# fabioiuri/DRecPy

Hardware: AMD Instinct MI355X
Metric: training samples/sec (user-item pairs) (higher is better)
Workload: dtype f32; 1 GPU; CDAE hidden_factors=128 sampled-output sparse-Adagrad on synth-10m-shaped synthetic (10000000 users x 1000000 items, 199573906 positives), corruption 0.2, neg_ratio 5; batch_per_gpu=65536, global_batch=65536, touch_list=prepared ahead on a side stream, batches=fresh device-sampled batch every step (sampler running ahead on the side stream)

## Files before the change

drecpy_amd/_lib.py:

```python
import ctypes as C
import os

_HERE = os.path.dirname(os.path.abspath(__file__))
LIB_PATH = os.path.join(_HERE, 'libdrx.so')

LOSS_BCE, LOSS_MSE = 0, 1
TARGETS_REFERENCE, TARGETS_PER_ROW = 0, 1
OPT_ADAM, OPT_ADAGRAD, OPT_ROWWISE_ADAGRAD = 0, 1, 2
DENSE_AUX_CLEAN = 0x100
KEY_NONE = 0xFFFFFFFF
SHARD_SELF_BYPASS = 1
BATCH_SHARE_USERS = 1


class DrxError(RuntimeError):
    pass


DRX_REC_SIGMOID_BIAS, DRX_REC_BIAS, DRX_REC_CLIP = 0, 1, 2

KNN_METRICS = {'cosine': 0, 'adjusted_cosine': 1, 'cosine_cf': 2, 'jaccard': 3, 'msd': 4, 'pearson': 5}
KNN_USER, KNN_ITEM = 0, 1
KNN_AGGREGATIONS = {'mean': 0, 'weighted_mean': 1}

# ... 116 lines not shown
    _fields_ = [(n, C.c_void_p) for n in ('K0u', 'm_u', 'v_u', 'K0i', 'm_i', 'v_i')] + [('n_items', C.c_int32), ('n_users', C.c_int32)] + \
               [(n, C.c_float) for n in ('alpha_u', 'alpha_i', 'l2_coef', 'beta1', 'beta2', 'eps')] + [('row_order', C.c_void_p), ('n_long', C.c_int32), ('opt_kind', C.c_int32)]


class Optim(C.Structure):
    _fields_ = [('kind', C.c_int32), ('lr', C.c_float), ('reg_rate', C.c_float), ('beta1', C.c_float),
                ('beta2', C.c_float), ('eps', C.c_float), ('alpha', C.c_float * 5),
                ('s1', C.c_void_p * 5), ('s2', C.c_void_p * 5)]


_lib = None

SIGNATURES = {
    'drx_version': (C.c_int, []),
    'drx_strerror': (C.c_char_p, [C.c_int]),
    'drx_hash_u32': (C.c_uint32, [C.c_uint64, C.c_uint32, C.c_uint32]),
    'drx_event_create': (C.c_void_p, []),
    'drx_event_destroy': (None, [C.c_void_p]),
    'drx_event_record': (C.c_int, [C.c_void_p, C.c_void_p]),
    'drx_stream_wait_event': (C.c_int, [C.c_void_p, C.c_void_p]),
    'drx_event_synchronize': (C.c_int, [C.c_void_p]),
    'drx_stream_create_cu_slice': (C.c_void_p, [C.c_int32]),
    'drx_stream_destroy': (None, [C.c_void_p]),
    'drx_cdae_forward': (C.c_int, [C.POINTER(CdaeParams), C.POINTER(History), C.POINTER(Batch), C.c_void_p,
                                   C.c_void_p, C.c_void_p]),
    'drx_cdae_scratch_bytes': (C.c_size_t, [C.POINTER(CdaeParams), C.c_int32, C.c_int32, C.c_int32]),
    'drx_cdae_step_dense': (C.c_int, [C.POINTER(CdaeParams), C.POINTER(Optim), C.POINTER(History), C.POINTER(Batch),
                                      C.c_int32, C.c_int32, C.c_void_p, C.c_size_t, C.c_void_p, C.c_void_p]),
    'drx_cdae_step_sparse': (C.c_int, [C.POINTER(CdaeParams), C.POINTER(Optim), C.POINTER(History), C.POINTER(Batch),
                                       C.c_int32, C.c_void_p, C.c_size_t, C.c_void_p, C.c_void_p]),
    'drx_cdae_step_sparse_timed': (C.c_int, [C.POINTER(CdaeParams), C.POINTER(Optim), C.POINTER(History),
                                             C.POINTER(Batch), C.c_int32, C.c_void_p, C.c_size_t, C.c_void_p,
                                             C.POINTER(C.c_void_p), C.c_void_p]),
    'drx_cdae_prep_bytes': (C.c_size_t, [C.POINTER(CdaeParams), C.c_int32, C.c_int32]),
    'drx_cdae_sparse_prepare': (C.c_int, [C.POINTER(CdaeParams), C.POINTER(History), C.POINTER(Batch), C.c_void_p,
                                          C.c_size_t, C.c_void_p]),
    'drx_cdae_step_sparse_prepared': (C.c_int, [C.POINTER(CdaeParams), C.POINTER(Optim), C.POINTER(History),
                                                C.POINTER(Batch), C.c_int32, C.c_void_p, C.c_size_t, C.c_void_p,
                                                C.c_size_t, C.c_void_p, C.POINTER(C.c_void_p), C.c_void_p]),
    'drx_cdae_prep_bytes_hot': (C.c_size_t, [C.POINTER(CdaeParams), C.c_int32, C.c_int32, C.c_int32]),
    'drx_cdae_scratch_bytes_hot': (C.c_size_t, [C.POINTER(CdaeParams), C.c_int32, C.c_int32, C.c_int32]),
    'drx_cdae_sparse_prepare_hot': (C.c_int, [C.POINTER(CdaeParams), C.POINTER(History), C.POINTER(Batch), C.POINTER(HotHead),
                                              C.c_void_p, C.c_size_t, C.c_void_p]),
    'drx_debug_prep_counts': (C.c_int, [C.POINTER(CdaeParams), C.POINTER(History), C.POINTER(Batch), C.POINTER(HotHead), C.c_void_p,
                                        C.c_int32, C.c_int32, C.c_int32, C.c_void_p, C.c_size_t, C.c_void_p, C.c_void_p, C.c_void_p,
                                        C.c_void_p, C.c_void_p, C.POINTER(C.c_int32), C.c_void_p]),
    'drx_debug_prep_result': (C.c_int, [C.POINTER(CdaeParams), C.c_int32, C.c_int32, C.c_int32, C.c_void_p, C.c_size_t, C.c_void_p,
                                        C.c_void_p, C.c_void_p, C.c_void_p, C.c_void_p, C.c_void_p]),
    'drx_debug_cdae_reduce': (C.c_int, [C.POINTER(CdaeParams), C.POINTER(Optim), C.POINTER(History), C.POINTER(Batch), C.POINTER(HotHead),
                                        C.c_void_p, C.c_size_t, C.c_void_p, C.c_void_p, C.c_void_p, C.c_int32, C.c_void_p, C.c_size_t,
                                        C.c_void_p]),
    'drx_debug_span_plan': (C.c_int, [C.POINTER(CdaeParams), C.c_int32, C.c_int32, C.c_int32, C.c_void_p, C.c_size_t, C.c_void_p,
                                      C.c_void_p, C.c_void_p, C.c_void_p]),
    'drx_cdae_step_sparse_hot': (C.c_int, [C.POINTER(CdaeParams), C.POINTER(Optim), C.POINTER(History), C.POINTER(Batch),
                                           C.POINTER(HotHead), C.c_int32, C.c_void_p, C.c_size_t, C.c_void_p, C.c_size_t,
                                           C.c_void_p, C.POINTER(C.c_void_p), C.c_void_p]),
    'drx_cdae_hot_rows_for': (C.c_int32, [C.POINTER(CdaeParams), C.c_int32, C.c_int32, C.c_int32, C.c_int32]),
    'drx_cdae_prep_forget': (None, [C.c_void_p]),
    'drx_point_sample_scratch_bytes': (C.c_size_t, [C.c_int32]),
    'drx_list_sample_device': (C.c_int, [C.POINTER(ListGroups), C.c_int32, C.c_int32, C.c_int32, C.c_int32, C.c_uint64, C.c_void_p, C.c_void_p,
                                         C.c_void_p, C.c_void_p]),
    'drx_point_sample': (C.c_int, [C.POINTER(History), C.c_int32, C.c_int32, C.c_int32, C.c_int32, C.c_uint64,
                                   C.c_void_p, C.c_void_p, C.c_void_p, C.c_void_p, C.c_void_p, C.c_size_t, C.c_void_p, C.c_uint32,
                                   C.c_void_p]),
    'drx_point_sample_recorded': (C.c_int, [C.POINTER(History), C.POINTER(History), C.c_int32, C.c_int32, C.c_int32, C.c_int32, C.c_uint64,
                                   C.c_void_p, C.c_void_p, C.c_void_p, C.c_void_p, C.c_void_p, C.c_size_t, C.c_void_p, C.c_uint32,
                                   C.c_void_p]),
    'drx_point_sample_by_user_scratch_bytes': (C.c_size_t, [C.c_int32, C.c_int32]),
    'drx_point_sample_by_user': (C.c_int, [C.POINTER(History), C.POINTER(History), C.c_int32, C.c_int32, C.c_int32, C.c_int32, C.c_uint64,
                                           C.c_void_p, C.c_void_p, C.c_void_p, C.c_void_p, C.c_void_p, C.c_size_t, C.c_void_p, C.c_uint32,
                                           C.c_void_p]),
    'drx_point_sample_valued': (C.c_int, [C.POINTER(History), C.POINTER(History), C.c_void_p, C.c_float, C.c_float, C.c_int32, C.c_int32,
                                          C.c_int32, C.c_int32, C.c_uint64, C.c_void_p, C.c_void_p, C.c_void_p, C.c_void_p]),
    'drx_dmf_distinct_scratch_bytes': (C.c_size_t, [C.c_int32, C.c_int32, C.c_int32]),
    'drx_dmf_batch_distinct_device': (C.c_int, [C.c_void_p, C.c_void_p, C.c_void_p, C.c_int32, C.c_int32, C.c_int32] + [C.c_void_p] * 10 +
                                      [C.c_void_p, C.c_size_t, C.c_void_p]),
    'drx_shard_prep_bytes': (C.c_size_t, [C.POINTER(CdaeParams), C.POINTER(Shard), C.c_int32, C.c_int32]),
    'drx_shard_work_bytes': (C.c_size_t, [C.POINTER(Shard)]),
    'drx_shard_prep_layout': (C.c_int, [C.POINTER(CdaeParams), C.POINTER(Shard), C.c_int32, C.c_int32, C.POINTER(C.c_size_t)]),
    'drx_shard_prepare': (C.c_int, [C.POINTER(CdaeParams), C.POINTER(Shard), C.POINTER(History), C.POINTER(Batch), C.c_void_p,
                                    C.c_size_t, C.c_void_p, C.c_size_t, C.c_void_p]),
    'drx_shard_owner_table_bytes': (C.c_size_t, [C.POINTER(Shard), C.c_int32]),
    'drx_shard_chunks': (C.c_int32, [C.POINTER(Shard)]),
    'drx_shard_unit_shift': (C.c_int32, [C.POINTER(Shard)]),
    'drx_shard_owner_index': (C.c_int, [C.POINTER(Shard), C.c_void_p, C.c_int32, C.POINTER(C.c_int32), C.c_int32, C.c_int32, C.c_void_p,
                                        C.c_size_t, C.c_void_p]),
    'drx_shard_gather_rows': (C.c_int, [C.POINTER(CdaeParams), C.POINTER(Shard), C.c_void_p, C.c_int32, C.POINTER(C.c_int32),
                                        C.c_int32, C.c_void_p, C.c_void_p]),
    'drx_shard_step_scratch_bytes': (C.c_size_t, [C.POINTER(CdaeParams), C.c_int32, C.c_int32]),
    'drx_shard_step_local': (C.c_int, [C.POINTER(CdaeParams), C.POINTER(Optim), C.POINTER(Shard), C.POINTER(History), C.POINTER(Batch),
                                       C.c_void_p, C.c_size_t, C.c_void_p, C.c_void_p, C.c_int32, C.c_int32, C.c_void_p, C.c_size_t,
                                       C.POINTER(C.c_void_p), C.c_void_p]),
    'drx_shard_apply': (C.c_int, [C.POINTER(CdaeParams), C.POINTER(Optim), C.POINTER(Shard), C.c_int32, C.c_void_p, C.c_void_p,
                                  C.c_int32, C.POINTER(C.c_int32), C.c_int32, C.c_int32, C.c_void_p, C.POINTER(C.c_void_p), C.POINTER(C.c_int64),
                                  C.c_void_p, C.c_void_p]),
    'drx_shard_exchange_sizes': (C.c_int, [C.POINTER(CdaeParams), C.POINTER(Shard), C.c_void_p, C.c_void_p, C.POINTER(C.c_int64)]),
    'drx_shard_phase_layout': (C.c_int, [C.POINTER(CdaeParams), C.POINTER(Shard), C.c_void_p, C.c_void_p, C.c_int32, C.POINTER(C.c_int64)]),
    'drx_shard_phase_keys': (C.c_int, [C.POINTER(Shard), C.c_void_p, C.POINTER(ShardExchange), C.c_void_p]),
    'drx_shard_phase_rows': (C.c_int, [C.POINTER(CdaeParams), C.POINTER(Shard), C.c_void_p, C.POINTER(ShardExchange), C.c_int32, C.c_void_p]),
    'drx_shard_phase_local': (C.c_int, [C.POINTER(CdaeParams), C.POINTER(Optim), C.POINTER(Shard), C.POINTER(History), C.POINTER(Batch),
                                        C.c_void_p, C.POINTER(ShardExchange), C.c_void_p, C.c_size_t, C.c_int32, C.c_int32, C.c_void_p,
                                        C.c_size_t, C.POINTER(C.c_void_p), C.c_void_p]),
    'drx_shard_phase_tail': (C.c_int, [C.POINTER(CdaeParams), C.POINTER(Optim), C.POINTER(Shard), C.c_void_p, C.POINTER(ShardExchange),
                                       C.POINTER(ShardExchange), C.c_int32, C.c_void_p, C.c_void_p]),
    'drx_copy_f4': (C.c_int, [C.c_void_p, C.c_void_p, C.c_size_t, C.c_void_p]),
    'drx_copy_f4_variant': (C.c_int, [C.c_void_p, C.c_void_p, C.c_size_t, C.c_int32, C.c_void_p]),
# ... 277 lines not shown
```

drecpy_amd/csrc/drx_cdae.hip:

```cpp
#include "drx_common.hpp"
#include "drx_rows.hpp"
#include "drx_segreduce.hpp"
#include <cstring>
#include "drx_scan.hpp"
#include "drx_prep.hpp"
#include "drx_segstream.hpp"
#include "drx_cdae_host.hpp"
#include <type_traits>
#include <mutex>
#include <unordered_map>

#ifdef DRX_STAMPS
static unsigned long long *h_stamps = nullptr;
extern "C" int drx_debug_set_stamps(unsigned long long *buf, unsigned int) { h_stamps = buf; return 0; }
#endif

namespace drx {

struct SparseBufs {
  float *dz1;
  float *g2;
  float *dz2;
  float *lossb;
  float *phead, *ptail;
  float *phs, *pts;
  float *pblock, *pbs;
  float *bpart;
  const uint8_t *solo_v, *solo_o;
  unsigned long long *stamps;
  const int32_t *order;
  const int32_t *usamp, *worder, *n_items;
  const WorkItem *witem;
  int T, n_chunks, n_bpart;
};

template <int G, int J, int KIND = -1>
__device__ __forceinline__ void sparse_apply(const DrxCdaeParams &P, const DrxOptim &opt, int B, uint32_t key, int lane,
                                             const float4 (&g)[J], float gs) {
  const uint32_t N = (uint32_t)P.n_items;
  float *const tW = P.W, *const tO = P.W2T, *const tV = P.V;
  float *const a0 = opt.s1[0], *const a1 = opt.s1[1], *const a2 = opt.s1[2];
  float *const c0 = opt.s2[0], *const c1 = opt.s2[1], *const c2 = opt.s2[2];
  const int var = key < N ? 0 : (key < 2 * N ? 1 : 2);
  const size_t row = key - (uint32_t)var * N;
  float *const tab = var == 0 ? tW : (var == 1 ? tO : tV);
  float *const s1 = var == 0 ? a0 : (var == 1 ? a1 : a2);
  float *const s2 = var == 0 ? c0 : (var == 1 ? c1 : c2);
  OptScalars o = opt_for(opt, 0, B);
  o.inv_k = 1.0f / (float)P.k;
  float4 w[J];
  load_row<G, J>(tab, row, P.ld, lane, w);
  row_update<G, J, KIND>(o, tab, s1, s2, row, P.ld, lane, w, g);
  if (var == 1 && lane == 0) {
    const int kind = KIND >= 0 ? KIND : o.kind;
    float pb = P.b2[row], m = opt.s1[4][row], v = kind == DRX_OPT_ADAM ? opt.s2[4][row] : 0.f;
    o.rb = 0.f;
    opt_update1<KIND>(o, gs, pb, m, v);
    P.b2[row] = pb; opt.s1[4][row] = m;
    if (kind == DRX_OPT_ADAM) opt.s2[4][row] = v;
  }
}

template <int G, int J>
// ... 283 lines not shown
  if (r != 0) return;
#pragma unroll
  for (int j = 0; j < J; ++j) acc[j] = f4_zero();
#pragma unroll 8
  for (int rr = 0; rr < R; ++rr) {
    float4 v[J];
    load_row<G, J>(lds, (size_t)rr, P.ld, lane, v);
#pragma unroll
    for (int j = 0; j < J; ++j) f4_add(acc[j], v[j]);
  }
  sampled_finish<G, J>(P, opt, H, bt, scale, qthr, loss_kind, S, b, lane, acc);
}

template <int KIND>
struct DirectPolicyT {
  DrxCdaeParams P;
  DrxOptim opt;
  int B;
  float scale;
  const float *dz1;
  long long g2_off;
  const float *dz2;
  template <int G, int J>
  __device__ __forceinline__ void load(uint32_t key, uint32_t bv, int lane, float4 (&row)[J], float &sc, float &coef) const {
    const uint32_t N = (uint32_t)P.n_items;
    const bool is_out = key >= N && key < 2 * N;
    const uint32_t b = bv & 0x7FFFFFFFu;
    load_row<G, J>(dz1 + (is_out ? g2_off : 0ll), (size_t)b, P.ld, lane, row);
    if (is_out) sc = dz2[b];
    coef = key < N ? ((bv >> 31) ? -scale : scale) : 1.0f;
  }
  template <int G, int J>
  __device__ __forceinline__ void finish(uint32_t key, int, int lane, const float4 (&g)[J], float gs) const {
    sparse_apply<G, J, KIND>(P, opt, B, key, lane, g, gs);
  }
  static constexpr bool kStreamParks = false;
  __device__ __forceinline__ StreamArrays stream_arrays() const {
    const uint32_t N = (uint32_t)P.n_items;
    return StreamArrays{{0u, N, 2u * N}, {dz1, dz1 + g2_off, dz1}, {P.W, P.W2T, P.V}, {opt.s1[0], opt.s1[1], opt.s1[2]},
                        {scale, 1.0f, 1.0f}, {nullptr, dz2, nullptr}, {nullptr, P.b2, nullptr}, {nullptr, opt.s1[4], nullptr}};
  }
  __device__ __forceinline__ float stream_decay() const { return opt.reg_rate / (float)B; }
  __device__ __forceinline__ void stream_update(float g, float &p, float &a) const {
    static_assert(KIND == DRX_OPT_ADAGRAD || KIND < 0, "one slot per element");
    OptScalars o = opt_for(opt, 0, B);
    float unused = 0.f;
    opt_update1<DRX_OPT_ADAGRAD>(o, g, p, a, unused);
  }
  __device__ __forceinline__ void stream_update_scalar(float g, float &p, float &a) const { stream_update(g, p, a); }
};
using DirectPolicy = DirectPolicyT<-1>;
using DirectPolicyAdagrad = DirectPolicyT<DRX_OPT_ADAGRAD>;

template <int G, int J, int NT>
__device__ __forceinline__ void bias_final_body(const DrxCdaeParams &P, const DrxOptim &opt, const BiasArgs &A,
                                                float *lds , float *red) {
  constexpr int R = NT / G;
  const int lane = threadIdx.x % G, r = threadIdx.x / G;
  float4 acc[J];
#pragma unroll
  for (int j = 0; j < J; ++j) acc[j] = f4_zero();
  constexpr int NB = J == 1 ? 8 : 2;
  for (int i = r; i < A.n_part; i += NB * R) {
    float4 v[NB][J];
#pragma unroll
    for (int q = 0; q < NB; ++q) {
#pragma unroll
      for (int j = 0; j < J; ++j) v[q][j] = f4_zero();
      if (i + q * R < A.n_part) load_row<G, J>(A.part, (size_t)(i + q * R), P.ld, lane, v[q]);
    }
#pragma unroll
    for (int q = 0; q < NB; ++q)
#pragma unroll
      for (int j = 0; j < J; ++j) f4_add(acc[j], v[q][j]);
  }
  store_row<G, J>(lds, (size_t)r, P.ld, lane, acc);
  __syncthreads();
  if (r == 0) {
    float4 g[J], w[J];
#pragma unroll
    for (int j = 0; j < J; ++j) g[j] = f4_zero();
#pragma unroll 8
    for (int rr = 0; rr < R; ++rr) {
      float4 v[J];
      load_row<G, J>(lds, (size_t)rr, P.ld, lane, v);
#pragma unroll
      for (int j = 0; j < J; ++j) f4_add(g[j], v[j]);
    }
    load_row<G, J>(P.b, 0, P.ld, lane, w);
    OptScalars o = opt_for(opt, 0, A.B);
    if (o.kind == DRX_OPT_ROWWISE_ADAGRAD) o.kind = DRX_OPT_ADAGRAD;
    o.rb = 0.f;
    row_update<G, J>(o, P.b, opt.s1[3], opt.s2[3], 0, P.ld, lane, w, g);
  }
  if (A.loss_out) {
    const float *lp = A.part + (size_t)A.n_part * P.ld;
    float a = 0.f;
    for (int b = threadIdx.x; b < A.n_part; b += NT) a += lp[b];
    float t = block_sum(a, red);
    if (threadIdx.x == 0) { A.loss_out[0] = t / (float)A.B; A.loss_out[1] = 0.f; }
  }
}

template <int G, int J>
struct BiasFinalExtra {
  DrxCdaeParams P;
  DrxOptim opt;
  BiasArgs A;
  __device__ __forceinline__ void operator()(float *lds) const {
    __shared__ float red[kFixBlock / 64];
    bias_final_body<G, J, kFixBlock>(P, opt, A, lds, red);
  }
};

constexpr int kHotSlice = 512;
constexpr int kHotGroup = 64;

struct HotArgs {
  const float *dz1;
  const uint32_t *mask;
  float *part;
  uint32_t *any;
  const int32_t *item;
  float scale;
  int B, H, Bw, S, first;
  float *bpart;
  const float *lossb;
};

static inline int hot_slices(int B) { return (B + kHotSlice - 1) / kHotSlice; }
static inline int hot_groups(int H) { return (H + kHotGroup - 1) / kHotGroup; }

typedef __bf16 hot_bf16x8 __attribute__((ext_vector_type(8)));
typedef float hot_f32x4 __attribute__((ext_vector_type(4)));
typedef uint32_t hot_u32x4 __attribute__((ext_vector_type(4)));

template <int LD, int NT>
struct HotPartialExtra {
  HotArgs A;
  __device__ __forceinline__ void operator()(float *) const {
    constexpr int CS = LD / 16, NW = NT / 64;
    const int lane = threadIdx.x & 63, wv = __builtin_amdgcn_readfirstlane((int)(threadIdx.x >> 6));
    const int ngr = (A.H + kHotGroup - 1) / kHotGroup;
    const int task = ((int)blockIdx.x - A.first) * NW + wv;
    if (task >= A.S * ngr * CS) return;
    const int cs = task % CS, rg = (task / CS) % ngr, s = task / (CS * ngr);
    const int c = lane & 15, kq = lane >> 4;
    const int nt = min(kHotGroup, A.H - rg * kHotGroup) / 16;
    const int b_begin = s * kHotSlice, b_end = min(A.B, b_begin + kHotSlice);
    const uint32_t *const mgrp = A.mask + (size_t)rg * kHotGroup * A.Bw;
    const float *const slice = A.dz1 + (size_t)b_begin * LD + cs * 16;
    const uint32_t mlane = (uint32_t)c * (uint32_t)A.Bw, xlane = (uint32_t)(8 * kq * LD + c);
    hot_f32x4 acc[4];
#pragma unroll
    for (int t = 0; t < 4; ++t) acc[t] = hot_f32x4{0.f, 0.f, 0.f, 0.f};
    uint32_t seen = 0u;
    float bsum = 0.f;
    for (int b0 = b_begin; b0 < b_end; b0 += 32) {
      float x[8];
      uint32_t w[4];
      {
        const float *const rows = slice + (size_t)(b0 - b_begin) * LD;
        const uint32_t *const words = mgrp + (b0 >> 5);
        const int left = A.B - b0 - 8 * kq;
// ... 18 lines not shown
          hv[e] = __float_as_uint(v) & 0xFFFF0000u;
          const float r1 = v - __uint_as_float(hv[e]);
          mv[e] = __float_as_uint(r1) & 0xFFFF0000u;
          lv[e] = __float_as_uint(r1 - __uint_as_float(mv[e])) & 0xFFFF0000u;
        }
        bh[i] = (hv[0] >> 16) | hv[1];
        bm[i] = (mv[0] >> 16) | mv[1];
        bl[i] = (lv[0] >> 16) | lv[1];
      }
#pragma unroll
      for (int t = 0; t < 4; ++t) {
        seen |= (w[t] != 0u ? 1u : 0u) << t;
        const uint32_t bits = (w[t] >> (8 * kq)) & 0xFFu;
        hot_u32x4 a;
#pragma unroll
        for (int i = 0; i < 4; ++i) a[i] = ((bits >> (2 * i)) & 1u) * 0x3F80u | ((bits >> (2 * i + 1)) & 1u) * 0x3F800000u;
        const hot_bf16x8 av = __builtin_bit_cast(hot_bf16x8, a);
        acc[t] = __builtin_amdgcn_mfma_f32_16x16x32_bf16(av, __builtin_bit_cast(hot_bf16x8, bh), acc[t], 0, 0, 0);
        acc[t] = __builtin_amdgcn_mfma_f32_16x16x32_bf16(av, __builtin_bit_cast(hot_bf16x8, bm), acc[t], 0, 0, 0);
        acc[t] = __builtin_amdgcn_mfma_f32_16x16x32_bf16(av, __builtin_bit_cast(hot_bf16x8, bl), acc[t], 0, 0, 0);
      }
    }
    float *const out = A.part + ((size_t)s * A.H + rg * kHotGroup) * LD + cs * 16 + c;
#pragma unroll
    for (int t = 0; t < 4; ++t)
      if (t < nt) {
#pragma unroll
        for (int i = 0; i < 4; ++i) out[(size_t)(16 * t + 4 * kq + i) * LD] = acc[t][i];
      }
    if (cs == 0) {
      uint32_t rows[4];
#pragma unroll
      for (int t = 0; t < 4; ++t) rows[t] = (uint32_t)__ballot((seen >> t) & 1u) & 0xFFFFu;
      if (lane == 0) {
        uint32_t *const any = A.any + (size_t)s * (A.H / 32) + rg * (kHotGroup / 32);
        any[0] = rows[0] | (rows[1] << 16);
        if (nt > 2) any[1] = rows[2] | (rows[3] << 16);
      }
    }
    if (rg == 0) {
      const float g1 = __shfl(bsum, c + 16, 64), g2 = __shfl(bsum, c + 32, 64), g3 = __shfl(bsum, c + 48, 64);
      if (kq == 0) A.bpart[(size_t)s * LD + cs * 16 + c] = ((bsum + g1) + g2) + g3;
      if (cs == 0 && A.lossb) {
        float l = 0.f;
        for (int b = b_begin + lane; b < b_end; b += 64) l += A.lossb[b];
#pragma unroll
        for (int o = 32; o > 0; o >>= 1) l += __shfl_xor(l, o, 64);
        if (lane == 0) A.bpart[(size_t)A.S * LD + s] = l;
      }
    }
  }
};

template <int LD, class Policy>
struct HotFinishExtra {
  HotArgs A;
  Policy pol;
  __device__ __forceinline__ void operator()(float *lds) const {
    constexpr int NT = kFixBlock, NQ = NT / LD;
    static_assert(NQ >= 1 && NT % LD == 0, "a row per workgroup");
    const int h = (int)blockIdx.x - A.first;
    if (h >= A.H) return;
    const uint32_t bit = 1u << (h & 31);
    bool touched = false;
    for (int s = (int)threadIdx.x; s < A.S; s += NT) touched |= (A.any[(size_t)s * (A.H / 32) + (h >> 5)] & bit) != 0u;
    if (!__syncthreads_or(touched)) return;
    const int c = (int)threadIdx.x % LD, q = (int)threadIdx.x / LD;
    const int per = (A.S + NQ - 1) / NQ, s0 = q * per, s1 = min(A.S, s0 + per);
    float sum = 0.f;
#pragma unroll 8
    for (int s = s0; s < s1; ++s) sum += A.part[((size_t)s * A.H + h) * LD + c];
    lds[q * LD + c] = sum;
    __syncthreads();
    if (q == 0) {
      float t = lds[c];
#pragma unroll
      for (int k = 1; k < NQ; ++k) t += lds[k * LD + c];
      const StreamArrays SA = pol.stream_arrays();
      const size_t off = (size_t)A.item[h] * LD + c;
      float pv = SA.table[0][off], av = SA.slot[0][off];
      pol.stream_update(fmaf(pol.stream_decay(), pv, A.scale * t), pv, av);
      SA.table[0][off] = pv;
      SA.slot[0][off] = av;
    }
  }
};

template <class E1, class E2>
struct ExtraPair {
  E1 e1;
  int n1;
  E2 e2;
  __device__ __forceinline__ void operator()(float *lds) const {
    if ((int)blockIdx.x < n1) e1(lds);
    else e2(lds);
  }
};

static SparseBufs sparse_layout(Carver &cv, const DrxCdaeParams &P, int B, int n_touch_slots) {
  SparseBufs S{};
  S.T = n_touch_slots + 2 * B;
  const int chunk = seg_chunk(long_segments(S.T, P));
  S.n_chunks = (S.T + chunk - 1) / chunk;
  S.n_bpart = 1024;
  S.dz1 = cv.take<float>((size_t)2 * B * P.ld);
  S.g2 = cv.take<float>((size_t)B * P.ld);
  S.dz2 = cv.take<float>(B);
  S.lossb = cv.take<float>(B);
  S.phead = cv.take<float>((size_t)S.n_chunks * P.ld);
  S.ptail = cv.take<float>((size_t)S.n_chunks * P.ld);
  S.phs = cv.take<float>(S.n_chunks);
  S.pts = cv.take<float>(S.n_chunks);
  {
    const int cpb = kSegBlock / pick_geom(P.ld).G;
    const int n_blocks = (S.n_chunks + cpb - 1) / cpb;
    S.pblock = cv.take<float>((size_t)n_blocks * P.ld);
    S.pbs = cv.take<float>(n_blocks);
  }
  S.bpart = cv.take<float>((size_t)S.n_bpart * (P.ld + 1));
  return S;
}

static std::mutex g_hot_mu;
static std::unordered_map<const void *, int> g_hot_of;
static void hot_record(const void *prepared, int H) {
  std::lock_guard<std::mutex> lk(g_hot_mu);
  if (H > 0) g_hot_of[prepared] = H;
  else g_hot_of.erase(prepared);
}
static int hot_recorded(const void *prepared) {
  std::lock_guard<std::mutex> lk(g_hot_mu);
  const auto it = g_hot_of.find(prepared);
  return it == g_hot_of.end() ? 0 : it->second;
}

struct HotBufs { float *part; uint32_t *any; float *bpart; };
static HotBufs hot_layout(Carver &cv, const DrxCdaeParams &P, int B, int H) {
  HotBufs HB{nullptr, nullptr, nullptr};
  if (H <= 0) return HB;
  HB.part = cv.take<float>((size_t)hot_slices(B) * H * P.ld);
  HB.any = cv.take<uint32_t>((size_t)hot_slices(B) * (H / 32));
  HB.bpart = cv.take<float>((size_t)hot_slices(B) * (P.ld + 1));
  return HB;
}

template <int G, int J>
static void launch_forward(ForwardForm form, const DrxCdaeParams &P, const DrxOptim &opt, const DrxHistory &hist, const DrxBatch &bt,
                           float scale, uint32_t qthr, int32_t loss_kind, const SparseBufs &S, const float *ks_h, const float *ks_dot,
                           hipStream_t st) {
  constexpr int gpb = kBlock / G;
  const dim3 groups((bt.B + gpb - 1) / gpb);
  const bool adagrad = opt.kind == DRX_OPT_ADAGRAD;
  switch (form) {
  case ForwardForm::ColumnShard:
    hipLaunchKernelGGL((k_kshard_rest<G, J>), groups, dim3(kBlock), 0, st, P, opt, hist, bt, scale, qthr, loss_kind, S, ks_h, ks_dot);
    break;
  case ForwardForm::SharedUsers:
    if constexpr (G >= 16 && J <= 2) {
      const long long wmax = (long long)(P.n_users < bt.B ? P.n_users : bt.B) + bt.B / share_item_triples(P.ld) + 1;
      hipLaunchKernelGGL((adagrad ? k_items_fwd_bwd<G, J, DRX_OPT_ADAGRAD> : k_items_fwd_bwd<G, J>), dim3((unsigned)(wmax < bt.B ? wmax : bt.B)),
                         dim3(kItemThreads), share_item_lds_bytes(P.ld), st, P, opt, hist, bt, scale, qthr, loss_kind, S);
    }
    break;
  case ForwardForm::PerWorkgroup:
    hipLaunchKernelGGL((k_sampled_fwd_bwd_wg<G, J>), dim3(bt.B), dim3(kBlock), (size_t)gpb * P.ld * 4, st, P, opt, hist, bt, scale, qthr,
                       loss_kind, S);
    break;
  case ForwardForm::PerGroup:
    hipLaunchKernelGGL((adagrad ? k_sampled_fwd_bwd<G, J, DRX_OPT_ADAGRAD> : k_sampled_fwd_bwd<G, J>), groups, dim3(kBlock), 0, st, P, opt, hist,
                       bt, scale, qthr, loss_kind, S);
    break;
  }
}

template <int G, int J, class Policy>
static int reduce_and_finish(ReduceForm form, const DrxCdaeParams &P, const DrxOptim &opt, const SparseBufs &S, const SegBufs &SB,
                             const PlanBufs &PB, const SpanPlan &plan, const BiasArgs &BA, const HotArgs &HA, void *const *events,
                             hipStream_t st) {
  const Policy pol{P, opt, BA.B, HA.scale, S.dz1, (long long)(S.g2 - S.dz1), S.dz2};
  const BiasFinalExtra<G, J> bias{P, opt, BA};
  int rc = DRX_EINVAL;
  if (HA.H == 0) rc = launch_reduce<G, J>(form, SB, PB, plan, pol, BA, st);
  else if constexpr (kHotBuilt<G, J, Policy>) {
    constexpr int NT = kStreamThreads<G>;
    HotArgs part = HA;
    part.first = 0;
    const int n_hot = (HA.S * hot_groups(HA.H) * (G / 4) + NT / 64 - 1) / (NT / 64);
    rc = launch_reduce_streamed<G, J>(SB, PB, plan, pol, n_hot, HotPartialExtra<4 * G, NT>{part}, st);
  }
  if (rc) return rc;
  DRX_HIP(phase_event(events, 3, st));
  rc = DRX_EINVAL;
  if (HA.H == 0) rc = launch_spans<G, J>(SB, PB, plan, pol, 1, bias, st);
  else if constexpr (kHotBuilt<G, J, Policy>) {
    HotArgs fin = HA;
    fin.first = kSpanBlocks + 1;
    using Finish = ExtraPair<BiasFinalExtra<G, J>, HotFinishExtra<4 * G, Policy>>;
    rc = launch_spans<G, J>(SB, PB, plan, pol, 1 + HA.H, Finish{bias, fin.first, {fin, pol}}, st);
  }
  if (rc) return rc;
  DRX_HIP(phase_event(events, 4, st));
  DRX_HIP(phase_event(events, 5, st));
  return DRX_OK;
}

}

using namespace drx;

extern "C" {

size_t drx_cdae_scratch_bytes(const DrxCdaeParams *p, int32_t B, int32_t n_touch_slots, int32_t dense_mode) {
  if (!p || B < 1 || n_touch_slots < 0) return 0;
  Carver c(nullptr, 0);
  if (dense_mode) {
    c.off = dense_layout_bytes(*p, B);
  } else {
    (void)sparse_layout(c, *p, B, n_touch_slots);
    (void)prep_layout(c, *p, B, n_touch_slots);
  }
  return align_up(c.off, 256) + 256;
}

struct GivenGradients { const float *dz1, *g2, *dz2; int32_t form; };

static int step_sparse_impl(const DrxCdaeParams *p, const DrxOptim *opt, const DrxHistory *hist, const DrxBatch *bt,
                            int32_t loss_kind, const void *prepared, size_t prepared_bytes, void *scratch, size_t scratch_bytes,
                            float *loss_out, void *const *events, void *stream, const float *ks_h = nullptr,
                            const float *ks_dot = nullptr, const DrxHotHead *hot = nullptr, const GivenGradients *given = nullptr) {
  int rc = check_params(p);
  if (rc) return rc;
  rc = check_batch(hist, bt);
  if (rc || !opt || !scratch || !bt->iid || (!bt->y && !given) || !bt->keep_off) return DRX_EINVAL;
  if (opt->kind != DRX_OPT_ADAM && opt->kind != DRX_OPT_ADAGRAD && opt->kind != DRX_OPT_ROWWISE_ADAGRAD) return DRX_EINVAL;
  for (int i = 0; i < 5; ++i)
    if (!opt->s1[i] || (opt->kind == DRX_OPT_ADAM && !opt->s2[i])) return DRX_EINVAL;
  if ((uint64_t)2 * p->n_items + p->n_users + 1 >= 0xFFFFFFFFull) return DRX_EINVAL;
  hipStream_t st = (hipStream_t)stream;
  const int H = hot ? hot->H : 0;
  if (prepared && hot_recorded(prepared) != H) return DRX_EINVAL;
  Carver cv(scratch, scratch_bytes);
  SparseBufs S = sparse_layout(cv, *p, bt->B, bt->n_touch_slots);
  const HotBufs HB = hot_layout(cv, *p, bt->B, H);
  PrepBufs R{};
  if (prepared) {
    Carver cp(const_cast<void *>(prepared), prepared_bytes);
    R = prep_layout(cp, *p, bt->B, bt->n_touch_slots, H);
    if (!cp.ok()) return DRX_ESCRATCH;
  } else {
    R = prep_layout(cv, *p, bt->B, bt->n_touch_slots, H);
  }
  if (!cv.ok()) return DRX_ESCRATCH;
  const float scale = 1.0f / (1.0f - bt->q);
  const uint32_t qthr = q_threshold(bt->q);
  const int rows_per_block = (bt->B + S.n_bpart - 1) / S.n_bpart;
  const int n_bpart = (bt->B + rows_per_block - 1) / rows_per_block;
  S.solo_v = prepared ? R.solo_v : nullptr;
  S.solo_o = prepared ? R.solo_o : nullptr;
  S.order = prepared ? R.order : nullptr;
  SegBufs SB{R.keys_s, R.vals_s, S.phead, S.ptail, S.phs, S.pts, nullptr, nullptr, nullptr, nullptr, S.T, S.n_chunks, p->ld, nullptr};
#ifdef DRX_STAMPS
  S.stamps = SB.stamps = h_stamps;
#endif
  PlanBufs PB{S.pblock, S.pbs};
  if (prepared && ks_h && share_users(p, hist, bt, R)) return DRX_EINVAL;
  const bool share = prepared && !ks_h && share_users(p, hist, bt, R);
  S.usamp = share ? R.usamp : nullptr;
  S.witem = share ? R.witem : nullptr;
  S.worder = share ? R.worder : nullptr;
  S.n_items = share ? R.n_du : nullptr;
  ReduceForm form = reduce_form(opt->kind, bt->B, S.T, *p);
  const ForwardForm fwd = forward_form(ks_h != nullptr, share, bt->B, bt->n_touch_slots);
  if (H > 0 && !hot_head_fits(form, p->ld, share, ks_h != nullptr)) return DRX_EINVAL;
  if (given) {
    if (share || (given->form == 1 && (H > 0 || form == ReduceForm::PlannedLong))) return DRX_EINVAL;
    if (given->form == 1) form = ReduceForm::PlannedShort;
  }
  const HotArgs HA{S.dz1, R.hmask, HB.part, HB.any, hot ? hot->item : nullptr, scale, bt->B, H, R.Bw, hot_slices(bt->B), 0, HB.bpart,
                   loss_out ? S.lossb : nullptr};
  const BiasArgs BA = H > 0 ? BiasArgs{S.dz1, HB.bpart, S.lossb, loss_out, bt->B, hot_slices(bt->B), kHotSlice}
                            : BiasArgs{S.dz1, S.bpart, S.lossb, loss_out, bt->B, n_bpart, rows_per_block};
  DRX_HIP(phase_event(events, 0, st));
  if (given) {
    const size_t row_bytes = (size_t)bt->B * p->ld * sizeof(float);
    DRX_HIP(hipMemcpyAsync(S.dz1, given->dz1, row_bytes, hipMemcpyDeviceToDevice, st));
    DRX_HIP(hipMemcpyAsync(S.g2, given->g2, row_bytes, hipMemcpyDeviceToDevice, st));
    DRX_HIP(hipMemcpyAsync(S.dz2, given->dz2, (size_t)bt->B * sizeof(float), hipMemcpyDeviceToDevice, st));
    DRX_HIP(hipMemsetAsync(S.lossb, 0, (size_t)bt->B * sizeof(float), st));
  } else {
    (void)dispatch_geom(p->ld, [&](auto g) -> int {
      launch_forward<decltype(g)::G, decltype(g)::J>(fwd, *p, *opt, *hist, *bt, scale, qthr, loss_kind, S, ks_h, ks_dot, st);
      return DRX_OK;
    });
  }
  DRX_HIP(phase_event(events, 1, st));
  if (!prepared) {
    rc = prepare_impl(p, hist, bt, R, st, false, TouchPresence{nullptr, WireGeo{1, 0, 1}}, hot ? hot->slot : nullptr,
                      hot ? hot->item : nullptr);
    if (rc) return rc;
  }
  DRX_HIP(phase_event(events, 2, st));
  rc = dispatch_geom(p->ld, [&](auto g) -> int {
    constexpr int G = decltype(g)::G, J = decltype(g)::J;
    return opt->kind == DRX_OPT_ADAGRAD
        ? reduce_and_finish<G, J, DirectPolicyAdagrad>(form, *p, *opt, S, SB, PB, R.plan, BA, HA, events, st)
        : reduce_and_finish<G, J, DirectPolicy>(form, *p, *opt, S, SB, PB, R.plan, BA, HA, events, st);
  });
  if (rc) return rc;
  DRX_LAUNCH_CHECK();
  return DRX_OK;
}

size_t drx_cdae_prep_bytes(const DrxCdaeParams *p, int32_t B, int32_t n_touch_slots) {
  if (!p || B < 1 || n_touch_slots < 0) return 0;
  Carver c(nullptr, 0);
  (void)prep_layout(c, *p, B, n_touch_slots);
  return align_up(c.off, 256) + 256;
}

int drx_cdae_sparse_prepare(const DrxCdaeParams *p, const DrxHistory *hist, const DrxBatch *bt, void *prepared,
                            size_t prepared_bytes, void *stream) {
  int rc = check_params(p);
  if (rc) return rc;
  rc = check_batch(hist, bt);
  if (rc || !prepared || !bt->iid || !bt->keep_off) return DRX_EINVAL;
  Carver cp(prepared, prepared_bytes);
  PrepBufs R = prep_layout(cp, *p, bt->B, bt->n_touch_slots);
  if (!cp.ok()) return DRX_ESCRATCH;
  hot_record(prepared, 0);
  rc = prepare_impl(p, hist, bt, R, (hipStream_t)stream, true);
  if (rc) return rc;
  if (p->ld <= 16) order_by_degree(bt, R, (hipStream_t)stream, true);
  DRX_LAUNCH_CHECK();
  return DRX_OK;
}

size_t drx_cdae_prep_result_bytes(const DrxCdaeParams *p, int32_t B, int32_t n_touch_slots) {
  if (!p || B < 1 || n_touch_slots < 0) return 0;
  Carver c(nullptr, 0);
  return prep_layout(c, *p, B, n_touch_slots).result_bytes;
}

int drx_cdae_step_sparse_prepared(const DrxCdaeParams *p, const DrxOptim *opt, const DrxHistory *hist, const DrxBatch *bt,
                                  int32_t loss_kind, const void *prepared, size_t prepared_bytes, void *scratch,
                                  size_t scratch_bytes, float *loss_out, void *const *events, void *stream) {
  if (!prepared) return DRX_EINVAL;
  return step_sparse_impl(p, opt, hist, bt, loss_kind, prepared, prepared_bytes, scratch, scratch_bytes, loss_out, events, stream);
}

int drx_cdae_kshard_forward(const DrxCdaeParams *p, const DrxHistory *hist, const DrxBatch *bt, float *h_out, float *dot_partial,
                            void *stream) {
  return drx_cdae_kshard_forward_prepared(p, hist, bt, nullptr, 0, h_out, dot_partial, stream);
}

int drx_cdae_kshard_forward_prepared(const DrxCdaeParams *p, const DrxHistory *hist, const DrxBatch *bt, const void *prepared,
                                     size_t prepared_bytes, float *h_out, float *dot_partial, void *stream) {
  int rc = check_params(p);
  if (rc) return rc;
  rc = check_batch(hist, bt);
  if (rc || !bt->iid || !bt->keep_off || !h_out || !dot_partial) return DRX_EINVAL;
  const int32_t *order = nullptr;
  if (prepared) {
    Carver cp(const_cast<void *>(prepared), prepared_bytes);
    const PrepBufs R = prep_layout(cp, *p, bt->B, bt->n_touch_slots);
    if (!cp.ok()) return DRX_ESCRATCH;
    order = R.order;
  }
  hipStream_t st = (hipStream_t)stream;
  const float scale = 1.0f / (1.0f - bt->q);
  const uint32_t qthr = q_threshold(bt->q);
  const bool per_wg = forward_per_workgroup(bt->B, bt->n_touch_slots);
  return dispatch_geom(p->ld, [&](auto g) -> int {
    constexpr int G = decltype(g)::G, J = decltype(g)::J;
    constexpr int gpb = kBlock / G;
    if (per_wg)
      hipLaunchKernelGGL((k_kshard_fwd_wg<G, J>), dim3(bt->B), dim3(kBlock), (size_t)gpb * p->ld * 4, st, *p, *hist, *bt, scale, qthr,
                         h_out, dot_partial);
    else
      hipLaunchKernelGGL((k_kshard_fwd<G, J>), dim3((bt->B + gpb - 1) / gpb), dim3(kBlock), 0, st, *p, *hist, *bt, scale, qthr, h_out,
                         dot_partial, order);
    DRX_LAUNCH_CHECK();
    return DRX_OK;
  });
// ... 5 lines not shown
  if (!h || !dot_total) return DRX_EINVAL;
  if (opt && opt->kind == DRX_OPT_ROWWISE_ADAGRAD) return DRX_EINVAL;
  return step_sparse_impl(p, opt, hist, bt, loss_kind, prepared, prepared_bytes, scratch, scratch_bytes, loss_out, events, stream,
                          h, dot_total);
}

int drx_cdae_step_sparse(const DrxCdaeParams *p, const DrxOptim *opt, const DrxHistory *hist, const DrxBatch *bt,
                         int32_t loss_kind, void *scratch, size_t scratch_bytes, float *loss_out, void *stream) {
  return step_sparse_impl(p, opt, hist, bt, loss_kind, nullptr, 0, scratch, scratch_bytes, loss_out, nullptr, stream);
}

int drx_cdae_step_sparse_timed(const DrxCdaeParams *p, const DrxOptim *opt, const DrxHistory *hist, const DrxBatch *bt,
                               int32_t loss_kind, void *scratch, size_t scratch_bytes, float *loss_out, void *const *events,
                               void *stream) {
  if (!events) return DRX_EINVAL;
  return step_sparse_impl(p, opt, hist, bt, loss_kind, nullptr, 0, scratch, scratch_bytes, loss_out, events, stream);
}

static int hot_rows(const DrxCdaeParams *p, int32_t H) {
  if (!p || H < 0 || H > DRX_MAX_HOT || H % 32 || H > p->n_items) return -1;
  return H;
}

static bool hot_ok(const DrxCdaeParams *p, const DrxHotHead *hot) {
  return hot && hot_rows(p, hot->H) >= 0 && (hot->H == 0 || (hot->slot && hot->item && p->ld <= 4 * kHotMaxG));
}

size_t drx_cdae_prep_bytes_hot(const DrxCdaeParams *p, int32_t B, int32_t n_touch_slots, int32_t H) {
  if (!p || B < 1 || n_touch_slots < 0 || hot_rows(p, H) < 0) return 0;
  Carver c(nullptr, 0);
  (void)prep_layout(c, *p, B, n_touch_slots, H);
  return align_up(c.off, 256) + 256;
}

size_t drx_cdae_scratch_bytes_hot(const DrxCdaeParams *p, int32_t B, int32_t n_touch_slots, int32_t H) {
  if (!p || B < 1 || n_touch_slots < 0 || hot_rows(p, H) < 0) return 0;
  Carver c(nullptr, 0);
  (void)sparse_layout(c, *p, B, n_touch_slots);
  (void)hot_layout(c, *p, B, H);
  (void)prep_layout(c, *p, B, n_touch_slots, H);
  return align_up(c.off, 256) + 256;
}

int drx_cdae_sparse_prepare_hot(const DrxCdaeParams *p, const DrxHistory *hist, const DrxBatch *bt, const DrxHotHead *hot,
                                void *prepared, size_t prepared_bytes, void *stream) {
  int rc = check_params(p);
  if (rc) return rc;
  rc = check_batch(hist, bt);
  if (rc || !prepared || !bt->iid || !bt->keep_off || !hot_ok(p, hot)) return DRX_EINVAL;
  Carver cp(prepared, prepared_bytes);
  PrepBufs R = prep_layout(cp, *p, bt->B, bt->n_touch_slots, hot->H);
  if (!cp.ok()) return DRX_ESCRATCH;
  hot_record(prepared, 0);
  rc = prepare_impl(p, hist, bt, R, (hipStream_t)stream, true, TouchPresence{nullptr, WireGeo{1, 0, 1}}, hot->slot, hot->item);
  if (rc) return rc;
  hot_record(prepared, hot->H);
  if (p->ld <= 16) order_by_degree(bt, R, (hipStream_t)stream, true);
  DRX_LAUNCH_CHECK();
  return DRX_OK;
}

int drx_debug_prep_counts(const DrxCdaeParams *p, const DrxHistory *hist, const DrxBatch *bt, const DrxHotHead *hot, uint8_t *present,
                          int32_t ipr, int32_t cshift, int32_t world, void *prepared, size_t prepared_bytes, uint32_t *hist_out,
                          uint32_t *buckets_out, uint32_t *keys_out, uint32_t *vals_out, uint32_t *mask_out, int32_t *info_out,
                          void *stream) {
  int rc = check_params(p);
  if (rc) return rc;
  rc = check_batch(hist, bt);
  if (rc || !prepared || !bt->iid || !bt->keep_off || !hist_out || !buckets_out || !keys_out || !vals_out || !info_out) return DRX_EINVAL;
  if ((uint64_t)2 * p->n_items + p->n_users + 1 >= 0xFFFFFFFFull) return DRX_EINVAL;
  if (hot && !hot_ok(p, hot)) return DRX_EINVAL;
  if (present && (ipr < 1 || cshift < 0 || cshift > 30 || world < 1)) return DRX_EINVAL;
  const int H = hot ? hot->H : 0;
  if (H > 0 && !mask_out) return DRX_EINVAL;
  Carver cp(prepared, prepared_bytes);
  const PrepBufs R = prep_layout(cp, *p, bt->B, bt->n_touch_slots, H);
  if (!cp.ok()) return DRX_ESCRATCH;
  if (H > 0 && !hot_list_fits(R.T, *p, present != nullptr)) return DRX_EINVAL;
  hipStream_t st = (hipStream_t)stream;
  hot_record(prepared, 0);
  launch_touches(p, hist, bt, R, st, TouchPresence{present, WireGeo{present ? ipr : 1, present ? cshift : 0, present ? world : 1}},
                 H > 0 ? hot->slot : nullptr, H > 0 ? hot->item : nullptr);
  const SortRider rider{bt->keep_off, bt->B, R.order_work, R.partials, R.partial_rows};
  const uint32_t *h = nullptr;
  rc = sort_first_counts(R.sort_temp, R.sort_bytes, R.keys, (size_t)R.T, R.bits, true, st, rider, &h);
  if (rc) return rc;
  const int dbits = sort_first_digit_bits(R.bits);
  DRX_HIP(hipMemcpyAsync(hist_out, h, sizeof(uint32_t) << dbits, hipMemcpyDeviceToDevice, st));
  DRX_HIP(hipMemcpyAsync(buckets_out, R.order_work, 256 * sizeof(uint32_t), hipMemcpyDeviceToDevice, st));
  DRX_HIP(hipMemcpyAsync(keys_out, R.keys, (size_t)R.T * sizeof(uint32_t), hipMemcpyDeviceToDevice, st));
  DRX_HIP(hipMemcpyAsync(vals_out, R.vals, (size_t)R.T * sizeof(uint32_t), hipMemcpyDeviceToDevice, st));
  if (H > 0) DRX_HIP(hipMemcpyAsync(mask_out, R.hmask, (size_t)H * R.Bw * sizeof(uint32_t), hipMemcpyDeviceToDevice, st));
  info_out[0] = dbits;
  info_out[1] = R.partials ? R.partial_rows : 0;
  info_out[2] = R.T;
  info_out[3] = DRX_PREP_ROUNDS ? touch_grid(bt->B) : (bt->B + 15) / 16;
  DRX_LAUNCH_CHECK();
  return DRX_OK;
}

int drx_debug_prep_result(const DrxCdaeParams *p, int32_t B, int32_t n_touch_slots, int32_t H, const void *prepared, size_t prepared_bytes,
                          uint32_t *keys_s_out, uint32_t *vals_s_out, uint8_t *solo_v_out, uint8_t *solo_o_out, int32_t *order_out,
                          void *stream) {
  int rc = check_params(p);
  if (rc) return rc;
  if (B < 1 || n_touch_slots < 0 || hot_rows(p, H) < 0 || !prepared || !keys_s_out || !vals_s_out || !solo_v_out || !solo_o_out || !order_out)
    return DRX_EINVAL;
  Carver cp(const_cast<void *>(prepared), prepared_bytes);
  const PrepBufs R = prep_layout(cp, *p, B, n_touch_slots, H);
  if (!cp.ok()) return DRX_ESCRATCH;
  hipStream_t st = (hipStream_t)stream;
  DRX_HIP(hipMemcpyAsync(keys_s_out, R.keys_s, (size_t)R.T * sizeof(uint32_t), hipMemcpyDeviceToDevice, st));
  DRX_HIP(hipMemcpyAsync(vals_s_out, R.vals_s, (size_t)R.T * sizeof(uint32_t), hipMemcpyDeviceToDevice, st));
  DRX_HIP(hipMemcpyAsync(solo_v_out, R.solo_v, (size_t)B, hipMemcpyDeviceToDevice, st));
  DRX_HIP(hipMemcpyAsync(solo_o_out, R.solo_o, (size_t)B, hipMemcpyDeviceToDevice, st));
  DRX_HIP(hipMemcpyAsync(order_out, R.order, (size_t)B * sizeof(int32_t), hipMemcpyDeviceToDevice, st));
  return DRX_OK;
}

int drx_debug_cdae_reduce(const DrxCdaeParams *p, const DrxOptim *opt, const DrxHistory *hist, const DrxBatch *bt, const DrxHotHead *hot,
                          const void *prepared, size_t prepared_bytes, const float *dz1_in, const float *g2_in, const float *dz2_in,
                          int32_t form, void *scratch, size_t scratch_bytes, void *stream) {
  if (!dz1_in || !g2_in || !dz2_in || (form != 0 && form != 1) || (hot && !hot_ok(p, hot))) return DRX_EINVAL;
  const GivenGradients given{dz1_in, g2_in, dz2_in, form};
  return step_sparse_impl(p, opt, hist, bt, DRX_LOSS_BCE, prepared, prepared_bytes, scratch, scratch_bytes, nullptr, nullptr, stream,
                          nullptr, nullptr, hot && hot->H > 0 ? hot : nullptr, &given);
}

int drx_debug_span_plan(const DrxCdaeParams *p, int32_t B, int32_t n_touch_slots, int32_t H, const void *prepared, size_t prepared_bytes,
                        uint8_t *ext_out, uint32_t *desc_out, uint32_t *cnt_out, void *stream) {
  int rc = check_params(p);
  if (rc) return rc;
  if (B < 1 || n_touch_slots < 0 || hot_rows(p, H) < 0 || !prepared || !ext_out || !desc_out || !cnt_out) return DRX_EINVAL;
  Carver cp(const_cast<void *>(prepared), prepared_bytes);
  const PrepBufs R = prep_layout(cp, *p, B, n_touch_slots, H);
  if (!cp.ok()) return DRX_ESCRATCH;
  hipStream_t st = (hipStream_t)stream;
  DRX_HIP(hipMemcpyAsync(ext_out, R.plan.ext, (size_t)R.n_chunks, hipMemcpyDeviceToDevice, st));
  DRX_HIP(hipMemcpyAsync(desc_out, R.plan.desc, (size_t)R.n_chunks * sizeof(uint2), hipMemcpyDeviceToDevice, st));
  DRX_HIP(hipMemcpyAsync(cnt_out, R.plan.cnt, 2 * sizeof(uint32_t), hipMemcpyDeviceToDevice, st));
  return DRX_OK;
}

int drx_cdae_step_sparse_hot(const DrxCdaeParams *p, const DrxOptim *opt, const DrxHistory *hist, const DrxBatch *bt,
                             const DrxHotHead *hot, int32_t loss_kind, const void *prepared, size_t prepared_bytes, void *scratch,
                             size_t scratch_bytes, float *loss_out, void *const *events, void *stream) {
  if (!hot_ok(p, hot)) return DRX_EINVAL;
  return step_sparse_impl(p, opt, hist, bt, loss_kind, prepared, prepared_bytes, scratch, scratch_bytes, loss_out, events, stream,
                          nullptr, nullptr, hot);
}

int32_t drx_cdae_hot_rows_for(const DrxCdaeParams *p, int32_t opt_kind, int32_t B, int32_t n_touch_slots, int32_t H) {
  if (B < 1 || n_touch_slots < 0 || hot_rows(p, H) <= 0) return 0;
  return hot_head_fits(reduce_form(opt_kind, B, n_touch_slots + 2 * B, *p), p->ld, false, false) ? H : 0;
}

void drx_cdae_prep_forget(const void *prepared) {
  if (prepared) hot_record(prepared, 0);
}

}
```

drecpy_amd/csrc/drx_common.hpp:

```cpp
#pragma once
#include <cstring>
#include <hip/hip_runtime.h>
#include <stdint.h>
#include "drx.h"

#define DRX_HIP(expr)                                  \
  do {                                                 \
    hipError_t e_ = (expr);                            \
    if (e_ != hipSuccess) return (int)e_;              \
  } while (0)

#define DRX_LAUNCH_CHECK()                             \
  do {                                                 \
    hipError_t e_ = hipGetLastError();                 \
    if (e_ != hipSuccess) return (int)e_;              \
  } while (0)

namespace drx {

constexpr int kWave = 64;
constexpr int kBlock = 256;

__host__ __device__ inline uint32_t hash_u32(uint64_t seed, uint32_t a, uint32_t b) {
  uint64_t x = seed + (uint64_t)a * 0x9E3779B97F4A7C15ull + (uint64_t)b * 0xD1B54A32D192ED03ull;
// ... 96 lines not shown
  bool ok() const { return off <= cap; }
};

size_t sort_pairs_temp_bytes(size_t n, int end_bit);
int sort_pairs(void *temp, size_t temp_bytes, const uint32_t *kin, uint32_t *kout, const uint32_t *vin,
               uint32_t *vout, size_t n, int end_bit, hipStream_t stream);
__device__ __forceinline__ int degree_bucket(const int32_t *keep_off, int b) {
  const int d = (keep_off[b + 1] - keep_off[b]) >> 2;
  return 255 - (d > 255 ? 255 : d);
}

__device__ __forceinline__ unsigned long long same_bucket_lanes(bool valid, int d) {
  unsigned long long m = __ballot(valid);
#pragma unroll
  for (int bit = 0; bit < 8; ++bit) {
    const bool one = (d >> bit) & 1;
    const unsigned long long bl = __ballot(one);
    m &= one ? bl : ~bl;
  }
  return m;
}

template <int NT>
__device__ __forceinline__ void degree_counts_body(const int32_t *__restrict__ keep_off, int B, unsigned int *__restrict__ work, int block_id,
                                                   unsigned int *cnt ) {
  for (int i = threadIdx.x; i < 256; i += NT) cnt[i] = 0;
  __syncthreads();
  const int b = block_id * NT + (int)threadIdx.x, lane = threadIdx.x & 63;
  const bool valid = b < B;
  const int d = valid ? degree_bucket(keep_off, b) : 0;
  const unsigned long long m = same_bucket_lanes(valid, d);
  if (valid && lane == __ffsll((long long)m) - 1) atomicAdd(&cnt[d], (unsigned int)__popcll(m));
  __syncthreads();
  for (int i = threadIdx.x; i < 256; i += NT)
    if (cnt[i]) atomicAdd(&work[i], cnt[i]);
}

struct SortRider {
  const int32_t *keep_off;
  int B;
  unsigned int *counts;
  const uint32_t *partials = nullptr;
  int partial_rows = 0;
};
constexpr int kPartialWords = 512;
int sort_first_digit_bits(int end_bit);

int sort_pairs_ex(void *temp, size_t temp_bytes, const uint32_t *kin, uint32_t *kout, const uint32_t *vin, uint32_t *vout, size_t n, int end_bit,
                  bool drop_none, hipStream_t stream, bool pre_zeroed = false, SortRider rider = SortRider{nullptr, 0, nullptr});
void sort_pairs_zero_region(void *temp, size_t n, int end_bit, uint32_t **words, size_t *n_words);
int sort_first_counts(void *temp, size_t temp_bytes, const uint32_t *kin, size_t n, int end_bit, bool drop_none, hipStream_t stream,
                      SortRider rider, const uint32_t **hist);

inline int bits_for(uint64_t max_key_exclusive) {
  int b = 1;
  while (b < 32 && (1ull << b) < max_key_exclusive) ++b;
  return b;
}

}
```

drecpy_amd/csrc/drx_prep.hpp:

```cpp
#pragma once
#include <algorithm>
#include "drx_common.hpp"
#include "drx_rows.hpp"
#include "drx_segreduce.hpp"
#include "drx_scan.hpp"

namespace drx {

struct WireGeo {
  int ipr, cshift, world;
  __host__ __device__ __forceinline__ uint32_t wire(int item, int is_out) const {
    const int o = item / ipr;
    const uint32_t l = 2u * (uint32_t)(item - o * ipr) + (uint32_t)(is_out ? 1 : 0);
    return (((l >> cshift) * (uint32_t)world + (uint32_t)o) << cshift) | (l & ((1u << cshift) - 1u));
  }
  __host__ __device__ __forceinline__ uint32_t local(uint32_t w) const {
    return (((w >> cshift) / (uint32_t)world) << cshift) | (w & ((1u << cshift) - 1u));
  }
  __host__ __device__ __forceinline__ uint32_t unit(uint32_t w) const { return w >> cshift; }
};

struct TouchPresence {
  uint8_t *present;
  WireGeo G;
  __device__ __forceinline__ uint32_t wire(int item, int is_out) const { return G.wire(item, is_out); }
};

#ifndef DRX_HOT_LDS_LOOKUP
#define DRX_HOT_LDS_LOOKUP 1
#endif
struct HotMark {
  const int16_t *slot;
  uint32_t *mask;
  int H, Bw;
  const int32_t *item;
  int tbits;
};
static inline int hot_table_bits(int H) {
  int b = 0;
  while ((1 << b) < 4 * H) ++b;
  return b;
}
static inline size_t hot_table_lds_bytes(int H) { return H > 0 && DRX_HOT_LDS_LOOKUP ? ((size_t)6 << hot_table_bits(H)) : 0; }
__device__ __forceinline__ uint32_t hot_table_home(int item, int tbits) { return ((uint32_t)item * 2654435761u) >> (32 - tbits); }

static __global__ __launch_bounds__(kBlock) void k_sparse_touches(int n_items, DrxHistory H, DrxBatch bt, uint32_t qthr, uint32_t *keys,
                                                           uint32_t *vals, int T, uint8_t *solo, uint32_t *zero_a,
                                                           int n_zero_a, uint32_t *zero_b, int n_zero_b, uint32_t *zero_c, int n_zero_c,
                                                           TouchPresence pres, HotMark hot) {
  constexpr int G = 16;
  const int lane = threadIdx.x % G;
  const int b = blockIdx.x * (kBlock / G) + threadIdx.x / G;
  for (int w = blockIdx.x * kBlock + threadIdx.x; w < n_zero_a; w += gridDim.x * kBlock) zero_a[w] = 0u;
  for (int w = blockIdx.x * kBlock + threadIdx.x; w < n_zero_b; w += gridDim.x * kBlock) zero_b[w] = 0u;
// ... 213 lines not shown
}

template <int NT>
__device__ __forceinline__ void degree_scatter_body(const int32_t *__restrict__ keep_off, int B, unsigned int *__restrict__ work,
                                                    int32_t *__restrict__ order, int block_id, unsigned int *lds ) {
  unsigned int *start = lds, *cnt = lds + 256, *base = lds + 512;
  for (int i = threadIdx.x; i < 256; i += NT) cnt[i] = 0;
  if (threadIdx.x < 64) {
    unsigned int c[4], sum = 0;
#pragma unroll
    for (int q = 0; q < 4; ++q) { c[q] = work[threadIdx.x * 4 + q]; sum += c[q]; }
    unsigned int inc = sum;
#pragma unroll
    for (int o = 1; o < 64; o <<= 1) { const unsigned int t = __shfl_up(inc, o); if ((int)threadIdx.x >= o) inc += t; }
    unsigned int run = inc - sum;
#pragma unroll
    for (int q = 0; q < 4; ++q) { start[threadIdx.x * 4 + q] = run; run += c[q]; }
  }
  __syncthreads();
  const int b = block_id * NT + (int)threadIdx.x, lane = threadIdx.x & 63;
  const bool valid = b < B;
  const int d = valid ? degree_bucket(keep_off, b) : 0;
  const unsigned long long m = same_bucket_lanes(valid, d);
  const int leader = valid ? __ffsll((long long)m) - 1 : lane;
  unsigned int at = 0;
  if (valid && lane == leader) at = atomicAdd(&cnt[d], (unsigned int)__popcll(m));
  at = __shfl(at, leader);
  __syncthreads();
  for (int i = threadIdx.x; i < 256; i += NT) base[i] = cnt[i] ? atomicAdd(&work[256 + i], cnt[i]) : 0u;
  __syncthreads();
  if (valid) order[start[d] + base[d] + at + __popcll(m & ((1ull << lane) - 1ull))] = b;
}

static __global__ __launch_bounds__(1024) void k_degree_scatter(const int32_t *__restrict__ keep_off, int B, unsigned int *__restrict__ work,
                                                         int32_t *__restrict__ order) {
  __shared__ unsigned int lds[768];
  degree_scatter_body<1024>(keep_off, B, work, order, (int)blockIdx.x, lds);
}

static __global__ void k_mark_solo(uint32_t *keys_s, const uint32_t *__restrict__ vals_s, int T, uint32_t n_items, int B, uint8_t *solo_v,
                            uint8_t *solo_o) {
  for (int j = blockIdx.x * blockDim.x + threadIdx.x; j < T; j += gridDim.x * blockDim.x) {
    const uint32_t k = keys_s[j];
    if (k == DRX_KEY_NONE || k < n_items) continue;
    const uint32_t prev = j > 0 ? keys_s[j - 1] : DRX_KEY_NONE, next = j + 1 < T ? keys_s[j + 1] : DRX_KEY_NONE;
    if (k == prev || k == next) continue;
    const uint32_t b = vals_s[j];
    if (k < 2 * n_items) solo_o[b] = 1;
    else solo_v[b] = 1;
    keys_s[j] = DRX_KEY_NONE;
  }
}

static __global__ __launch_bounds__(256) void k_plan_and_mark(uint32_t *keys_s, const uint32_t *__restrict__ vals_s, int T, int n_chunks, int cpb,
                                                       SpanPlan P, uint32_t n_items, int B, uint8_t *solo_v, uint8_t *solo_o,
                                                       int order_blocks, const int32_t *keep_off, unsigned int *order_work,
                                                       int32_t *order) {
  const int plan_blocks = (int)gridDim.x - order_blocks;
  if ((int)blockIdx.x >= plan_blocks) {
    __shared__ unsigned int lds[768];
    degree_scatter_body<256>(keep_off, B, order_work, order, (int)blockIdx.x - plan_blocks, lds);
    return;
  }
  const int tid = blockIdx.x * blockDim.x + threadIdx.x;
  const int real = P.xrank ? (int)P.cnt[20] : 0;
  if (tid < n_chunks && (real == 0 || (long long)tid * P.chunk < (long long)real)) plan_chunk(keys_s, T, n_chunks, cpb, P, tid);
  const int nb = (n_chunks + cpb - 1) / cpb;
  if (P.xrank && (tid & ~63) < nb) place_block(keys_s, vals_s, T, cpb, B, P, tid, tid < nb);
  const int j_lo = real != 0 ? max(0, real - 2 * B) : 0, j_hi = real != 0 ? min(T, real) : T;
  for (int j = j_lo + tid; j < j_hi; j += plan_blocks * blockDim.x) {
    const uint32_t k = keys_s[j];
    if (k == DRX_KEY_NONE || k < n_items) continue;
    const uint32_t prev = j > 0 ? keys_s[j - 1] : DRX_KEY_NONE, next = j + 1 < T ? keys_s[j + 1] : DRX_KEY_NONE;
    if (k == prev || k == next) continue;
    const uint32_t b = vals_s[j];
    if (k < 2 * n_items) solo_o[b] = 1;
    else solo_v[b] = 1;
    keys_s[j] = DRX_KEY_NONE;
  }
}

struct BiasArgs {
  const float *dz1;
  float *part;
  const float *lossb;
  float *loss_out;
  int B, n_part, rows_per_block;
};

template <int G, int J, int NT>
__device__ __forceinline__ void bias_partial_body(int ld, const BiasArgs &A, int block_id, float *lds , float *red) {
  constexpr int R = (NT < kSegBlock ? NT : kSegBlock) / G;
  const int lane = threadIdx.x % G, r = threadIdx.x / G;
  const int b0 = block_id * A.rows_per_block, b1 = r < R ? min(A.B, b0 + A.rows_per_block) : 0;
  float4 acc[J];
#pragma unroll
  for (int j = 0; j < J; ++j) acc[j] = f4_zero();
  constexpr int NB = J == 1 ? 8 : 2;
  for (int b = b0 + r; b < b1; b += NB * R) {
    float4 v[NB][J];
#pragma unroll
    for (int q = 0; q < NB; ++q) {
#pragma unroll
      for (int j = 0; j < J; ++j) v[q][j] = f4_zero();
      if (b + q * R < b1) load_row<G, J>(A.dz1, (size_t)(b + q * R), ld, lane, v[q]);
    }
#pragma unroll
    for (int q = 0; q < NB; ++q)
#pragma unroll
      for (int j = 0; j < J; ++j) f4_add(acc[j], v[q][j]);
  }
  if (r < R) store_row<G, J>(lds, (size_t)r, ld, lane, acc);
  __syncthreads();
  if (r == 0) {
    float4 t[J];
#pragma unroll
    for (int j = 0; j < J; ++j) t[j] = f4_zero();
#pragma unroll 8
    for (int rr = 0; rr < R; ++rr) {
      float4 v[J];
      load_row<G, J>(lds, (size_t)rr, ld, lane, v);
#pragma unroll
      for (int j = 0; j < J; ++j) f4_add(t[j], v[j]);
    }
    store_row<G, J>(A.part, (size_t)block_id, ld, lane, t);
  }
  if (A.loss_out) {
    const int b1 = min(A.B, b0 + A.rows_per_block);
    float a = 0.f;
    for (int b = b0 + (int)threadIdx.x; b < b1; b += NT) a += A.lossb[b];
    const float tl = block_sum(a, red);
// ... 18 lines not shown
struct PrepBufs {
  uint32_t *keys_s, *vals_s, *keys, *vals;
  void *sort_temp;
  size_t sort_bytes;
  uint8_t *solo_v, *solo_o;
  SpanPlan plan;
  int32_t *order;
  int32_t *usamp;
  int32_t *pitem;
  WorkItem *witem;
  int32_t *worder;
  int32_t *n_du;
  unsigned int *order_work;
  int n_chunks;
  size_t result_bytes;
  int T, bits;
  uint32_t *hmask;
  int H, Bw;
  uint32_t *partials;
  int partial_rows;
};

static inline bool long_segments(int T, const DrxCdaeParams &P) { return (int64_t)T > 8 * ((int64_t)2 * P.n_items + P.n_users); }

#ifndef DRX_STREAM_DEPTH
#define DRX_STREAM_DEPTH 4
#endif
constexpr int kStreamDepth = DRX_STREAM_DEPTH;
constexpr int kStreamIndexBits = 28;
constexpr int kHotMaxG = 32;

enum class ReduceForm { Streamed, PlannedLong, PlannedShort };

template <class Policy> struct PolicyKind;
template <template <int> class PolicyT, int KIND> struct PolicyKind<PolicyT<KIND>> { static constexpr int value = KIND; };
template <int G, int J, class Policy>
constexpr bool kStreamBuilt = kStreamDepth > 0 && J == 1 && G >= 16 && PolicyKind<Policy>::value == DRX_OPT_ADAGRAD;
template <int G, int J, class Policy>
constexpr bool kHotBuilt = kStreamBuilt<G, J, Policy> && G <= kHotMaxG;

static inline ReduceForm reduce_form(int opt_kind, int B, int T, const DrxCdaeParams &K) {
  if (long_segments(T, K)) return ReduceForm::PlannedLong;
  const Geom gm = pick_geom(K.ld);
  const bool streamed = kStreamDepth > 0 && gm.J == 1 && gm.G >= 16 && K.ld == 4 * gm.G && opt_kind == DRX_OPT_ADAGRAD &&
                        B < (1 << kStreamIndexBits) && K.n_items < (1 << kStreamIndexBits) && K.n_users < (1 << kStreamIndexBits);
  return streamed ? ReduceForm::Streamed : ReduceForm::PlannedShort;
}

static inline bool hot_list_fits(int T, const DrxCdaeParams &K, bool presence) { return !presence && !long_segments(T, K); }
static inline bool hot_head_fits(ReduceForm form, int ld, bool share, bool kshard) {
  return form == ReduceForm::Streamed && pick_geom(ld).G <= kHotMaxG && !share && !kshard;
}

static inline bool forward_per_workgroup(int B, int n_touch_slots) {
  const long long mean_hist = n_touch_slots / (long long)B;
  return mean_hist > 64 || (B <= 8192 && mean_hist > 16);
}
enum class ForwardForm { ColumnShard, SharedUsers, PerWorkgroup, PerGroup };
static inline ForwardForm forward_form(bool kshard, bool share, int B, int n_touch_slots) {
  if (kshard) return ForwardForm::ColumnShard;
  if (share) return ForwardForm::SharedUsers;
  return forward_per_workgroup(B, n_touch_slots) ? ForwardForm::PerWorkgroup : ForwardForm::PerGroup;
}

static inline hipError_t phase_event(void *const *events, int i, hipStream_t st) {
  return events ? hipEventRecord((hipEvent_t)events[i], st) : hipSuccess;
}

static PrepBufs prep_layout(Carver &cv, const DrxCdaeParams &P, int B, int n_touch_slots, int H = 0) {
  PrepBufs R{};
  R.T = n_touch_slots + 2 * B;
  R.bits = bits_for((uint64_t)2 * P.n_items + P.n_users + 1);
  R.keys_s = cv.take<uint32_t>(R.T);
  R.vals_s = cv.take<uint32_t>(R.T);
  R.solo_v = cv.take<uint8_t>((size_t)2 * B);
  R.solo_o = R.solo_v ? R.solo_v + B : nullptr;
  R.plan.chunk = seg_chunk(long_segments(R.T, P));
  R.n_chunks = (R.T + R.plan.chunk - 1) / R.plan.chunk;
  R.plan.desc = cv.take<uint2>(R.n_chunks);
  R.plan.cnt = cv.take<uint32_t>(128);
  R.plan.ext = cv.take<uint8_t>(R.n_chunks);
  {
    R.plan.xstride = (R.n_chunks + 1) / 2;
    const bool placed = long_segments(R.T, P);
    const bool placed_any = placed || DRX_STREAM_PLACED != 0;
    R.plan.xrank = placed_any ? cv.take<uint32_t>((size_t)R.plan.xstride) : nullptr;
    R.plan.xperm = placed_any ? cv.take<uint32_t>((size_t)R.plan.xstride) : nullptr;
    R.usamp = placed ? cv.take<int32_t>(B) : nullptr;
    R.pitem = placed ? cv.take<int32_t>(B) : nullptr;
    R.witem = placed ? cv.take<WorkItem>((size_t)B) : nullptr;
    R.worder = placed ? cv.take<int32_t>(B) : nullptr;
    R.n_du = placed ? cv.take<int32_t>(128) : nullptr;
  }
  R.order = cv.take<int32_t>(B);
  R.result_bytes = align_up(cv.off, 256);
  R.keys = cv.take<uint32_t>(R.T);
  R.vals = cv.take<uint32_t>(R.T);
  R.sort_bytes = sort_pairs_temp_bytes(R.T, R.bits);
  R.sort_temp = cv.take<char>(R.sort_bytes);
  R.order_work = cv.take<unsigned int>(512);
  R.H = H;
  R.Bw = (B + 31) / 32;
  R.hmask = H > 0 ? cv.take<uint32_t>((size_t)H * R.Bw) : nullptr;
  R.partial_rows = DRX_PREP_ROUNDS && sort_first_digit_bits(R.bits) == 8 ? touch_grid(B) : 0;
  R.partials = R.partial_rows > 0 ? cv.take<uint32_t>((size_t)R.partial_rows * kPartialWords) : nullptr;
  return R;
}

static int plan_zero_words(const PrepBufs &R) { return (int)(((const char *)R.plan.ext + R.n_chunks - (const char *)R.plan.cnt + 3) / 4); }

static int plan_spans(const DrxCdaeParams *p, const DrxBatch *bt, const PrepBufs &R0, hipStream_t st, bool cleared) {
  const PrepBufs &R = R0;
  if (!cleared) DRX_HIP(hipMemsetAsync(R.plan.cnt, 0, (size_t)plan_zero_words(R) * 4, st));
  hipLaunchKernelGGL(k_plan_spans<0>, dim3((R.n_chunks + 255) / 256), dim3(256), 0, st, R.keys_s, R.vals_s, R.T, R.n_chunks,
                     kSegBlock / pick_geom(p->ld).G, bt->B, R.plan);
  if (R.plan.xrank) hipLaunchKernelGGL(k_place_blocks, dim3(256), dim3(256), 0, st, R.plan, R.n_chunks);
  return DRX_OK;
}

static void order_by_degree(const DrxBatch *bt, const PrepBufs &R, hipStream_t st, bool cleared) {
  if (!cleared) (void)hipMemsetAsync(R.order_work, 0, 512 * sizeof(unsigned int), st);
  const int blocks = (bt->B + 1023) / 1024;
  hipLaunchKernelGGL(k_degree_counts, dim3(blocks), dim3(1024), 0, st, bt->keep_off, bt->B, R.order_work);
  hipLaunchKernelGGL(k_degree_scatter, dim3(blocks), dim3(1024), 0, st, bt->keep_off, bt->B, R.order_work, R.order);
}

constexpr int kTpFallback = 0x7fff0001;

static __global__ __launch_bounds__(256) void k_tp_begin(DrxBatch bt, int n_users, uint32_t *__restrict__ k2, uint32_t *__restrict__ v2,
                                                         int32_t *__restrict__ se, int n_se, uint8_t *solo, uint32_t *zero_a, int n_zero_a,
                                                         uint32_t *zero_b, int n_zero_b) {
  const int tid = blockIdx.x * blockDim.x + threadIdx.x, nt = gridDim.x * blockDim.x;
  for (int j = tid; j < 2 * bt.B; j += nt) {
    k2[j] = j < bt.B ? (uint32_t)bt.uid[j] : (uint32_t)n_users + (uint32_t)bt.iid[j - bt.B];
    v2[j] = (uint32_t)j;
  }
  for (int j = tid; j < n_se; j += nt) se[j] = 0;
  for (int j = tid; j < 2 * bt.B; j += nt) solo[j] = 0;
  for (int j = tid; j < n_zero_a; j += nt) zero_a[j] = 0u;
  for (int j = tid; j < n_zero_b; j += nt) zero_b[j] = 0u;
// ... 218 lines not shown
  const uint32_t qthr = q_threshold(bt->q);
  hipLaunchKernelGGL(k_tp_begin, dim3(512), dim3(256), 0, st, *bt, U, k2, v2, start, 2 * (U + N), R.solo_v, R.plan.cnt, plan_zero_words(R),
                     R.order_work, 512);
  int rc = sort_pairs(stemp, sb, k2, ks, v2, vs, (size_t)2 * B, bits2, st);
  if (rc) return rc;
  hipLaunchKernelGGL(k_tp_runs, dim3((2 * B + 255) / 256 < 1024 ? (2 * B + 255) / 256 : 1024), dim3(256), 0, st, ks, 2 * B, start, end);
  const int egrid = U < (1 << 20) ? U : (1 << 20);
  const int wgrid = (int)((nnz + 255) / 256 < 16384 ? (nnz + 255) / 256 : 16384);
  const int rt = share_item_triples(p->ld);
  if (share) {
    const int ig = (B + 255) / 256;
    hipLaunchKernelGGL(k_tp_item_flags, dim3(ig), dim3(256), 0, st, ks, B, rt, start, R.pitem, R.n_du);
    rc = scan_i32(sctemp2, scb2, R.pitem, R.pitem, (size_t)B, true, st);
    if (rc) return rc;
    hipLaunchKernelGGL(k_tp_item_finish, dim3(ig), dim3(256), 0, st, ks, vs, B, rt, start, end, hist->indptr, R.usamp, R.pitem, R.witem,
                       R.n_du, R.plan.cnt);
    hipLaunchKernelGGL(k_tp_item_order, dim3(ig), dim3(256), 0, st, ks, B, rt, start, hist->indptr, R.pitem, R.worder, R.n_du);
    hipLaunchKernelGGL((k_tp_count<true>), dim3(egrid), dim3(256), 0, st, *hist, *bt, qthr, U, start, end, vs, cnt, km, rt);
  } else
    hipLaunchKernelGGL((k_tp_count<false>), dim3(egrid), dim3(256), 0, st, *hist, *bt, qthr, U, start, end, vs, cnt, km, rt);
  int *cnt_last = (int *)R.vals;
  DRX_HIP(hipMemcpyAsync(cnt_last, cnt + (nnz - 1), sizeof(int), hipMemcpyDeviceToDevice, st));
  rc = scan_i32(sctemp, scb, cnt, cnt, (size_t)nnz, false, st);
  if (rc) return rc;
  if (share)
    hipLaunchKernelGGL((k_tp_write<true>), dim3(wgrid), dim3(256), 0, st, *hist, *bt, qthr, start, end, vs, cnt, km, R.keys_s, R.vals_s, R.pitem, rt, row_end);
  else
    hipLaunchKernelGGL((k_tp_write<false>), dim3(wgrid), dim3(256), 0, st, *hist, *bt, qthr, start, end, vs, cnt, km, R.keys_s, R.vals_s, R.pitem, rt, row_end);
  hipLaunchKernelGGL(k_tp_tail, dim3(2048), dim3(256), 0, st, ks, vs, B, U, N, cnt + (nnz - 1), cnt_last, R.T, R.keys_s, R.vals_s, R.plan.cnt);
  return DRX_OK;
}

static void launch_touches(const DrxCdaeParams *p, const DrxHistory *hist, const DrxBatch *bt, const PrepBufs &R, hipStream_t st,
                           TouchPresence pres, const int16_t *hot_slot, const int32_t *hot_item) {
  const int gpb = kBlock / 16;
  (void)gpb;
  uint32_t *sort_zero = nullptr;
  size_t sort_zero_words = 0;
  sort_pairs_zero_region(R.sort_temp, (size_t)R.T, R.bits, &sort_zero, &sort_zero_words);
  const HotMark hm{R.H > 0 ? hot_slot : nullptr, R.hmask, R.H, R.Bw, hot_item, hot_table_bits(R.H)};
#if DRX_PREP_ROUNDS
  hipLaunchKernelGGL(k_sparse_touches_rounds, dim3(touch_grid(bt->B)), dim3(kBlock), hot_table_lds_bytes(R.H), st, p->n_items, *hist, *bt,
                     q_threshold(bt->q), R.keys, R.vals, R.T, R.solo_v, R.plan.cnt, plan_zero_words(R), R.order_work, 512,
                     sort_zero, (int)sort_zero_words, pres, hm, R.partials);
#else
  hipLaunchKernelGGL(k_sparse_touches, dim3((bt->B + gpb - 1) / gpb), dim3(kBlock), hot_table_lds_bytes(R.H), st, p->n_items, *hist, *bt,
                     q_threshold(bt->q), R.keys, R.vals, R.T, R.solo_v, R.plan.cnt, plan_zero_words(R), R.order_work, 512,
                     sort_zero, (int)sort_zero_words, pres, hm);
#endif
}

static int prepare_impl(const DrxCdaeParams *p, const DrxHistory *hist, const DrxBatch *bt, const PrepBufs &R, hipStream_t st,
                        bool with_marks = false, TouchPresence pres = TouchPresence{nullptr, WireGeo{1, 0, 1}},
                        const int16_t *hot_slot = nullptr, const int32_t *hot_item = nullptr) {
  if (R.H > 0 && (!hot_slot || !hot_item || !hot_list_fits(R.T, *p, pres.present != nullptr))) return DRX_EINVAL;
  if (hist->t_rank && hist->t_users && hist->t_pos && hist->t_items && !pres.present && long_segments(R.T, *p)) {
    const int32_t *row_end = nullptr;
    const int rc = prepare_transposed(p, hist, bt, R, st, with_marks, &row_end);
    if (rc == DRX_OK) {
      PrepBufs Rb = R;
      Rb.plan.row_end = row_end;
      Rb.plan.row_end_keys = (uint32_t)p->n_items;
      if (with_marks && p->ld > 16) {
        if (!share_users(p, hist, bt, R)) order_by_degree(bt, R, st, true);
        const int blocks = std::max(2048, (R.n_chunks + 255) / 256);
        hipLaunchKernelGGL(k_plan_and_mark, dim3(blocks), dim3(256), 0, st, R.keys_s, R.vals_s, R.T, R.n_chunks,
                           kSegBlock / pick_geom(p->ld).G, Rb.plan, (uint32_t)p->n_items, bt->B, R.solo_v, R.solo_o, 0, bt->keep_off,
                           R.order_work, R.order);
        if (R.plan.xrank) hipLaunchKernelGGL(k_place_blocks, dim3(256), dim3(256), 0, st, Rb.plan, R.n_chunks);
        return DRX_OK;
      }
      return plan_spans(p, bt, Rb, st, true);
    }
    if (rc != kTpFallback) return rc;
  }
  launch_touches(p, hist, bt, R, st, pres, hot_slot, hot_item);
  const bool fused_order = with_marks && p->ld > 16;
  const SortRider rider{fused_order ? bt->keep_off : nullptr, bt->B, R.order_work, R.partials, R.partial_rows};
  const int rc = sort_pairs_ex(R.sort_temp, R.sort_bytes, R.keys, R.keys_s, R.vals, R.vals_s, (size_t)R.T, R.bits, true, st, true, rider);
  if (rc) return rc;
  if (with_marks && p->ld > 16) {
    const int blocks = std::max(2048, (R.n_chunks + 255) / 256);
    const int order_blocks = (bt->B + 255) / 256;
    hipLaunchKernelGGL(k_plan_and_mark, dim3(blocks + order_blocks), dim3(256), 0, st, R.keys_s, R.vals_s, R.T, R.n_chunks,
                       kSegBlock / pick_geom(p->ld).G, R.plan, (uint32_t)p->n_items, bt->B, R.solo_v, R.solo_o,
                       order_blocks, bt->keep_off, R.order_work, R.order);
    if (R.plan.xrank) hipLaunchKernelGGL(k_place_blocks, dim3(256), dim3(256), 0, st, R.plan, R.n_chunks);
    return DRX_OK;
  }
  return plan_spans(p, bt, R, st, true);
}

static int mark_solo(const DrxCdaeParams *p, const DrxBatch *bt, const PrepBufs &R, hipStream_t st, bool cleared) {
  if (!cleared) {
    DRX_HIP(hipMemsetAsync(R.solo_v, 0, (size_t)bt->B * 2, st));
  }
  if (p->ld <= 16) return DRX_OK;
  hipLaunchKernelGGL(k_mark_solo, dim3(2048), dim3(256), 0, st, R.keys_s, R.vals_s, R.T, (uint32_t)p->n_items, bt->B, R.solo_v,
                     R.solo_o);
  return DRX_OK;
}


}
```

drecpy_amd/csrc/drx_segreduce.hpp:

```cpp
#pragma once
#include "drx_rows.hpp"

namespace drx {

#ifndef DRX_CHUNK
#define DRX_CHUNK 32
#endif
constexpr int kChunk = DRX_CHUNK;
constexpr int kChunkLong = 64;
static inline int seg_chunk(bool long_segments) { return long_segments ? kChunkLong : kChunk; }
#ifdef DRX_SEG_WAVE_PER_CHUNK
#define SEG_GPB(G) (drx::kBlock / 64)
#else
#define SEG_GPB(G) (drx::kBlock / (G))
#endif
constexpr int kShortSpan = 64;
#ifndef DRX_SEG_BLOCK
#define DRX_SEG_BLOCK 128
#endif
constexpr int kSegBlock = DRX_SEG_BLOCK;
constexpr int kPlanShort = 16;
constexpr int kFixBlock = 512;

struct SegBufs {
// ... 67 lines not shown
    uint32_t k8[LB];
    float s8[LB], c8[LB];
    float4 rows[LB][J];
#pragma unroll
    for (int u = 0; u < LB; ++u) {
      const int t = t0 + u;
      k8[u] = t < n ? bcast(kreg, t) : DRX_KEY_NONE;
      const uint32_t b = bcast(vreg, t < n ? t : 0);
      s8[u] = 0.f;
      c8[u] = 1.f;
#pragma unroll
      for (int jx = 0; jx < J; ++jx) rows[u][jx] = f4_zero();
      if (k8[u] != DRX_KEY_NONE) pol.template load<G, J>(k8[u], b, lane, rows[u], s8[u], c8[u]);
    }
#pragma unroll
    for (int u = 0; u < LB; ++u) {
      const uint32_t key = k8[u];
      if (key != DRX_KEY_NONE) {
        if (key != cur) {
          flush(false);
          cur = key;
          cur_from_start = (t0 + u == 0);
#pragma unroll
          for (int jx = 0; jx < J; ++jx) acc[jx] = f4_zero();
          accs = 0.f;
        }
#pragma unroll
        for (int jx = 0; jx < J; ++jx) f4_fma(acc[jx], c8[u], rows[u][jx]);
        accs += s8[u];
        cur_pos = start + t0 + u;
      }
    }
  }
  const bool ran_to_end = n > 0 && bcast(kreg, n - 1) != DRX_KEY_NONE;
  flush(ran_to_end);
  if (lane == 0) {
    const uint32_t first = n > 0 ? S.keys_s[start] : DRX_KEY_NONE, last = n > 0 ? S.keys_s[end - 1] : DRX_KEY_NONE;
    const bool cont = first != DRX_KEY_NONE && first == prev_key;
    const bool middle = cont && last == first && next_key == first;
    S.cflag[g] = middle ? 2 : (cont ? 1 : 0);
  }
}

struct SpanPlan {
  uint2 *desc;
  uint32_t *cnt;
  uint8_t *ext;
  uint32_t *xrank;
  uint32_t *xperm;
  int xstride;
  int chunk;
  const int32_t *row_end;
  uint32_t row_end_keys;
};
#ifndef DRX_STREAM_PLACED
#define DRX_STREAM_PLACED 0
#endif
#ifndef DRX_XBINS
#define DRX_XBINS 8
#endif
constexpr int kXBase = 32, kXBins = DRX_XBINS;

__device__ __forceinline__ void place_block(const uint32_t *__restrict__ keys_s, const uint32_t *__restrict__ vals_s, int T, int cpb, int B,
                                            const SpanPlan &P, int blk, bool on) {
  int x = blk & (kXBins - 1);
  if (on && P.cnt[20] != 0u && (long long)blk * cpb * P.chunk >= (long long)P.cnt[20]) on = false;
  bool banded = true;
  if (on && P.chunk == kChunk) {
    const long long first = (long long)blk * cpb * P.chunk, last = first + (long long)cpb * P.chunk - 1;
    banded = first > 0 && last < T && keys_s[first] != DRX_KEY_NONE && keys_s[first - 1] == keys_s[first] && keys_s[last] == keys_s[first];
  }
  if (on && banded) {
    const int at = blk * cpb * P.chunk;
    if (at < T && keys_s[at] != DRX_KEY_NONE) {
      uint32_t b = vals_s[at];
      if (b & 0x80000000u) b &= 0x7FFFFFFFu;
      else if (b >= (uint32_t)B) b = (uint32_t)(((unsigned long long)(b - (uint32_t)B) * (unsigned long long)B) / (unsigned long long)max(1u, P.cnt[21]));
      x = (int)min((uint32_t)(kXBins - 1), (uint32_t)(((unsigned long long)b * (unsigned long long)kXBins) / (unsigned long long)(B > 0 ? B : 1)));
    }
  }
  const int lane = threadIdx.x & 63;
  unsigned long long mine = 0ull, of_lane = 0ull;
#pragma unroll
  for (int r = 0; r < kXBins; ++r) {
    const unsigned long long m = __ballot(on && x == r);
    if (x == r) mine = m;
    if (lane == r) of_lane = m;
  }
  uint32_t base = 0;
  if (lane < kXBins && of_lane) base = atomicAdd(&P.cnt[kXBase + lane], (uint32_t)__popcll(of_lane));
  base = (uint32_t)__shfl((int)base, x);
  if (on) P.xrank[blk] = ((uint32_t)x << 24) | (base + (uint32_t)__popcll(mine & ((1ull << lane) - 1ull)));
  if (on && blk == 0) { P.cnt[16] = 1u; P.cnt[17] = (uint32_t)cpb; }
}

static __global__ __launch_bounds__(256) void k_place_blocks(SpanPlan P, int n_chunks) {
  __shared__ uint32_t pre[kXBins];
  if (threadIdx.x < kXBins) {
    uint32_t run = 0;
    for (int t = 0; t < (int)threadIdx.x; ++t) run += P.cnt[kXBase + t];
    pre[threadIdx.x] = run;
  }
  __syncthreads();
  const int cpb = (int)P.cnt[17];
  const int nb = cpb > 0 ? (n_chunks + cpb - 1) / cpb : 0;
  for (int blk = blockIdx.x * blockDim.x + threadIdx.x; blk < nb; blk += gridDim.x * blockDim.x) {
    if (P.cnt[20] != 0u && (long long)blk * cpb * P.chunk >= (long long)P.cnt[20]) continue;
// ... 287 lines not shown
            for (int jx = 0; jx < J; ++jx) acc[jx] = f4_zero();
            accs = 0.f;
          }
#pragma unroll
          for (int jx = 0; jx < J; ++jx) f4_fma(acc[jx], cv, row[jx]);
          accs += sv;
          cur_pos = start + t0 + u;
        }
      }
    }
    flush(n > 0 && bcast(kreg, n - 1) != DRX_KEY_NONE);
  } else {
    seg_fold_short<G, J, CH, LB1>(S, pol, g, lane, start, n, prev_key, next_key, all_inner, acc, accs);
  }
  if (all_inner) {
    float *sc = seg_lds + (size_t)CPB * S.ld;
    store_row<G, J>(seg_lds, (size_t)r, S.ld, lane, acc);
    if (lane == 0) sc[r] = accs;
    __syncthreads();
    if (r == 0) {
      float4 t[J];
#pragma unroll
      for (int jx = 0; jx < J; ++jx) t[jx] = f4_zero();
      float ts = 0.f;
#pragma unroll 8
      for (int rr = 0; rr < CPB; ++rr) {
        float4 v[J];
        load_row<G, J>(seg_lds, (size_t)rr, S.ld, lane, v);
#pragma unroll
        for (int jx = 0; jx < J; ++jx) f4_add(t[jx], v[jx]);
        ts += sc[rr];
      }
      store_row<G, J>(PB.pblock, (size_t)blk, S.ld, lane, t);
      if (lane == 0) PB.pbs[blk] = ts;
    }
  }
}

template <int G, int J>
__device__ __forceinline__ void span_partial(const SegBufs &S, const PlanBufs &PB, const SpanShape &sh, int cpb, int i, int lane,
                                             float4 (&v)[J], float &sv) {
  if (i < sh.n_lead) {
    const int c = sh.first + i;
    load_row<G, J>(S.phead, (size_t)c, S.ld, lane, v); sv = S.phs[c];
  } else if (i < sh.n_lead + sh.n_blk) {
    const int bb = (sh.first + sh.n_lead) / cpb + (i - sh.n_lead);
    load_row<G, J>(PB.pblock, (size_t)bb, S.ld, lane, v); sv = PB.pbs[bb];
  } else {
    const int c = sh.first + sh.n_lead + sh.n_blk * cpb + (i - sh.n_lead - sh.n_blk);
    load_row<G, J>(S.phead, (size_t)c, S.ld, lane, v); sv = S.phs[c];
  }
}

template <int G, int J, class Policy, class Extra>
__global__ __launch_bounds__(kFixBlock) void k_span_planned(SegBufs S, PlanBufs PB, SpanPlan SP, Policy pol, int n_long_blocks,
                                                            int n_short_blocks, Extra extra) {
  extern __shared__ __align__(16) float span_lds[];
  constexpr int R = kFixBlock / G, CPB = kSegBlock / G;
  const int lane = threadIdx.x % G, r = threadIdx.x / G;
  constexpr int UL = J == 1 ? 8 : 2;
  if ((int)blockIdx.x >= n_long_blocks + n_short_blocks) { extra(span_lds); return; }
  if ((int)blockIdx.x >= n_long_blocks) {
    const uint32_t n_short = SP.cnt[0];
    for (uint32_t si = ((int)blockIdx.x - n_long_blocks) * R + r; si < n_short; si += (uint32_t)n_short_blocks * R) {
      const uint2 d = SP.desc[si];
      const SpanShape sh(d, CPB);
      const int g0 = (int)d.x, tot = sh.total();
      const int kpos = min(S.T, (g0 + 1) * SP.chunk) - 1;
      float4 t[J];
      load_row<G, J>(S.ptail, (size_t)g0, S.ld, lane, t);
      float ts = S.pts[g0];
      for (int i0 = 0; i0 < tot; i0 += UL) {
        float4 v[UL][J];
        float sv[UL];
#pragma unroll
        for (int u = 0; u < UL; ++u) {
          sv[u] = 0.f;
#pragma unroll
          for (int j = 0; j < J; ++j) v[u][j] = f4_zero();
          if (i0 + u < tot) span_partial<G, J>(S, PB, sh, CPB, i0 + u, lane, v[u], sv[u]);
        }
#pragma unroll
        for (int u = 0; u < UL; ++u) {
#pragma unroll
          for (int j = 0; j < J; ++j) f4_add(t[j], v[u][j]);
          ts += sv[u];
        }
      }
      pol.template finish<G, J>(S.keys_s[kpos], kpos, lane, t, ts);
    }
    return;
  }
  float *sc = span_lds + (size_t)R * S.ld;
  const uint32_t n_long = SP.cnt[1];
  for (uint32_t si = blockIdx.x; si < n_long; si += (uint32_t)n_long_blocks) {
    const uint2 d = SP.desc[S.n_chunks - 1 - (int)si];
    const SpanShape sh(d, CPB);
    const int g0 = (int)d.x, tot = sh.total();
    const int kpos = min(S.T, (g0 + 1) * SP.chunk) - 1;
    float4 acc[J];
#pragma unroll
    for (int j = 0; j < J; ++j) acc[j] = f4_zero();
    float accs = 0.f;
    const int per = (tot + R - 1) / R;
    const int i_lo = r * per, i_hi = min(tot, i_lo + per);
    for (int i0 = i_lo; i0 < i_hi; i0 += UL) {
      float4 v[UL][J];
      float sv[UL];
#pragma unroll
      for (int u = 0; u < UL; ++u) {
        sv[u] = 0.f;
#pragma unroll
        for (int j = 0; j < J; ++j) v[u][j] = f4_zero();
        if (i0 + u < i_hi) span_partial<G, J>(S, PB, sh, CPB, i0 + u, lane, v[u], sv[u]);
      }
#pragma unroll
      for (int u = 0; u < UL; ++u) {
#pragma unroll
        for (int j = 0; j < J; ++j) f4_add(acc[j], v[u][j]);
        accs += sv[u];
      }
    }
    __syncthreads();
    store_row<G, J>(span_lds, (size_t)r, S.ld, lane, acc);
    if (lane == 0) sc[r] = accs;
    __syncthreads();
    if (r == 0) {
      float4 t[J];
      load_row<G, J>(S.ptail, (size_t)g0, S.ld, lane, t);
      float ts = S.pts[g0];
#pragma unroll 8
      for (int rr = 0; rr < R; ++rr) {
        float4 v[J];
        load_row<G, J>(span_lds, (size_t)rr, S.ld, lane, v);
#pragma unroll
        for (int j = 0; j < J; ++j) f4_add(t[j], v[j]);
        ts += sc[rr];
      }
      pol.template finish<G, J>(S.keys_s[kpos], kpos, lane, t, ts);
    }
  }
}


template <int G, int J, class Policy>
__device__ __forceinline__ void span_short_body(const SegBufs &S, const Policy &pol, int block_id, int n_blocks) {
  const int lane = threadIdx.x % G;
  const int gshift = (threadIdx.x & 63) / G * G;
  const unsigned long long gmask = G == 64 ? ~0ull : ((1ull << G) - 1ull);
  const uint32_t n_span = S.n_span[0];
  const int gpb = kBlock / G;
  constexpr int UL = J == 1 ? 8 : 2;
  for (uint32_t si = block_id * gpb + threadIdx.x / G; si < n_span; si += n_blocks * gpb) {
    const int g0 = (int)S.span_list[si];
    const uint32_t key = S.keys_s[min(S.T, (g0 + 1) * kChunk) - 1];
    int m = 0;
    bool is_long = false;
    for (int base = g0 + 1;; base += G) {
      const int c = base + lane;
      const int fl = c < S.n_chunks ? (int)S.cflag[c] : 0;
      const unsigned long long mid = (__ballot(fl == 2) >> gshift) & gmask;
      const int run = mid == gmask ? G : __builtin_ctzll(~mid);
      m += run;
      if (run < G) {
        m += (__shfl(fl, run, G) == 1) ? 1 : 0;
        break;
      }
      if (m >= kShortSpan) { is_long = true; break; }
    }
    if (is_long || m > kShortSpan) {
      if (lane == 0) S.long_list[atomicAdd(&S.n_span[1], 1u)] = (uint32_t)g0;
      continue;
    }
    float4 t[J];
    load_row<G, J>(S.ptail, (size_t)g0, S.ld, lane, t);
    float ts = S.pts[g0];
    for (int c0 = g0 + 1; c0 <= g0 + m; c0 += UL) {
      float4 v[UL][J];
      float sv[UL];
#pragma unroll
      for (int u = 0; u < UL; ++u) {
        sv[u] = 0.f;
#pragma unroll
        for (int j = 0; j < J; ++j) v[u][j] = f4_zero();
        if (c0 + u <= g0 + m) { load_row<G, J>(S.phead, (size_t)(c0 + u), S.ld, lane, v[u]); sv[u] = S.phs[c0 + u]; }
      }
#pragma unroll
      for (int u = 0; u < UL; ++u) {
#pragma unroll
        for (int j = 0; j < J; ++j) f4_add(t[j], v[u][j]);
        ts += sv[u];
      }
    }
    pol.template finish<G, J>(key, min(S.T, (g0 + 1) * kChunk) - 1, lane, t, ts);
// ... 88 lines not shown
```

drecpy_amd/csrc/drx_segstream.hpp:

```cpp
#pragma once
#include "drx_segreduce.hpp"
#include "drx_prep.hpp"

namespace drx {

__device__ __forceinline__ void lds_dma16(const void *gsrc, uint32_t lds_dst) {
  uint32_t keep;
  asm volatile("s_mov_b32 %0, m0\n\ts_mov_b32 m0, %2\n\ts_nop 0\n\tglobal_load_lds_dwordx4 %1, off\n\ts_mov_b32 m0, %0"
               : "=&s"(keep) : "v"(gsrc), "s"(lds_dst) : "memory");
}
template <int N>
__device__ __forceinline__ void wait_vmcnt() { asm volatile("s_waitcnt vmcnt(%0)" :: "n"(N) : "memory"); }

template <int VL> struct LaneVec;
template <> struct LaneVec<1> { using T = float; };
template <> struct LaneVec<2> { typedef float T __attribute__((ext_vector_type(2))); };
template <> struct LaneVec<4> { typedef float T __attribute__((ext_vector_type(4))); };

#ifndef DRX_STREAM_SGPRS
#define DRX_STREAM_SGPRS 80
#endif
#define DRX_STREAM_SGPR_CAP __attribute__((amdgpu_num_sgpr(DRX_STREAM_SGPRS), amdgpu_waves_per_eu(8)))
constexpr int kStreamItems = 3 * (2 * kChunk - 1) + 3;
static inline size_t seg_stream_lds_bytes(int ld, int depth) {
  const int cpb = kSegBlock / (ld / 4);
  return (size_t)cpb * ((size_t)depth * 1024 + (size_t)kStreamItems * 4 + 128) + (size_t)cpb * (ld + 4) * 4;
}
struct StreamArrays {
  uint32_t first_key[3];
  const float *grad[3];
  float *table[3], *slot[3];
  float coef[3];
  const float *sgrad[3];
  float *sparam[3], *sslot[3];
};

enum : uint32_t { kItGrad = 0, kItGradHead = 1, kItGradTail = 2, kItParam = 3, kItSlot = 4 };

template <int LD, int D, class Policy, class Extra>
__global__ __launch_bounds__((kSegBlock / (LD / 4)) * 64) DRX_STREAM_SGPR_CAP void k_seg_reduce_stream(SegBufs S, PlanBufs PB, SpanPlan SP, Policy pol,
                                                                               int extra_blocks, Extra extra) {
  extern __shared__ __align__(16) float seg_lds[];
  constexpr int G = LD / 4;
  constexpr int CPB = kSegBlock / G;
  constexpr int VL = LD / 64;
  constexpr int IPI = 256 / LD;
  constexpr int LPI = 64 / IPI;
  constexpr int CH = kChunk;
  using V = typename LaneVec<VL>::T;
  using GV = V __attribute__((address_space(1)));
  static_assert(LD == 64 || LD == 128 || LD == 256, "one, two or four rows per KiB");
  static_assert(D >= 2 && D <= 32, "ring depth");
  static_assert(2 * CH <= 64 && 3 * CPB <= 64, "a window is one touch per lane; a block's border keys one per lane");
  if ((int)blockIdx.x < extra_blocks) { extra(seg_lds); return; }
  const int lane = threadIdx.x & 63, wv = __builtin_amdgcn_readfirstlane((int)(threadIdx.x >> 6));
  const uint32_t *__restrict__ const ks = S.keys_s, *__restrict__ const vs = S.vals_s;
  const uint8_t *__restrict__ const ext = SP.ext;
  char *const lds_b = reinterpret_cast<char *>(seg_lds);
  float *const ring = reinterpret_cast<float *>(lds_b + (size_t)wv * D * 1024);
  uint32_t *const tab = reinterpret_cast<uint32_t *>(lds_b + (size_t)CPB * D * 1024 + (size_t)wv * kStreamItems * 4);
  long long *const offs = reinterpret_cast<long long *>(lds_b + (size_t)CPB * (D * 1024 + kStreamItems * 4) + (size_t)wv * 128);
  float *const comb = reinterpret_cast<float *>(lds_b + (size_t)CPB * (D * 1024 + kStreamItems * 4 + 128));
  const uint32_t ring_lds = (uint32_t)__builtin_amdgcn_readfirstlane((int)(uint32_t)(uintptr_t)ring);
  const StreamArrays A = pol.stream_arrays();
  const char *const origin = reinterpret_cast<const char *>(A.grad[0]);
  if (lane < 15) {
    const int v = lane / 5, k = lane % 5;
    const uintptr_t g = (uintptr_t)(v == 0 ? A.grad[0] : (v == 1 ? A.grad[1] : A.grad[2]));
    const uintptr_t t = (uintptr_t)(v == 0 ? A.table[0] : (v == 1 ? A.table[1] : A.table[2]));
    const uintptr_t sl = (uintptr_t)(v == 0 ? A.slot[0] : (v == 1 ? A.slot[1] : A.slot[2]));
    offs[lane] = (long long)((k <= (int)kItGradTail ? g : (k == (int)kItParam ? t : sl)) - (uintptr_t)origin);
  }
  const float decay = pol.stream_decay();
  const int sub = lane / LPI, piece = lane % LPI;

  struct Meta { uint32_t key, val, bk, prevk; int e0, e1; } m;
#if DRX_STREAM_PLACED == 2
  const int pb_ = placed_block(SP, (int)blockIdx.x, extra_blocks, (int)gridDim.x - extra_blocks, CPB);
  const int blk = pb_ < -5 ? pb_ : (int)blockIdx.x - extra_blocks;
#else
  const int blk = DRX_STREAM_PLACED ? placed_block(SP, (int)blockIdx.x, extra_blocks, (int)gridDim.x - extra_blocks, CPB)
                                    : (int)blockIdx.x - extra_blocks;
#endif
  if (blk < 0) return;
  {
    const int g = blk * CPB + wv, base = g * CH, pos = base + lane;
    const bool have = g < S.n_chunks;
    m.key = have && pos < S.T ? ks[pos] : DRX_KEY_NONE;
    m.val = have && pos < S.T ? vs[pos] : 0u;
    m.prevk = have && g > 0 ? ks[base - 1] : DRX_KEY_NONE;
    m.e0 = have && g > 0 ? (int)ext[g - 1] : 0;
    m.e1 = have ? (int)ext[g] : 0;
    const int c = blk * CPB + lane % CPB, role = lane / CPB;
    const int p = role == 0 ? c * CH : (role == 1 ? (c + 1) * CH - 1 : c * CH - 1);
    m.bk = lane < 3 * CPB && c < S.n_chunks && (c + 1) * CH <= S.T && p >= 0 ? ks[p] : DRX_KEY_NONE;
  }
  wave_lds_sync();
  {
    const uint32_t bl = (uint32_t)__shfl((int)m.bk, lane + CPB, 64), bp = (uint32_t)__shfl((int)m.bk, lane + 2 * CPB, 64);
    const bool inner = lane < CPB && m.bk != DRX_KEY_NONE && m.bk == bp && bl == m.bk;
    const bool all_inner = (__ballot(inner) & ((1ull << CPB) - 1ull)) == ((1ull << CPB) - 1ull);
    const int g = blk * CPB + wv;
    V acc;
    float accs = 0.f;
    float *const accf = reinterpret_cast<float *>(&acc);
#pragma unroll
    for (int v = 0; v < VL; ++v) accf[v] = 0.f;
    if (g < S.n_chunks) {
      const int base = g * CH;
      const int e0 = __builtin_amdgcn_readfirstlane(m.e0), e1 = __builtin_amdgcn_readfirstlane(m.e1);
      const int end_off = min(CH + e1, S.T - base);
      const int n = max(0, end_off - e0);
      const uint32_t key = m.key, val = m.val;
      const bool valid = lane >= e0 && lane < end_off && key != DRX_KEY_NONE;
      const uint32_t prev_key = e0 > 0 ? (uint32_t)__builtin_amdgcn_readlane((int)key, e0 - 1) : (uint32_t)__builtin_amdgcn_readfirstlane((int)m.prevk);
      const uint32_t next_key = n > 0 ? (uint32_t)__builtin_amdgcn_readlane((int)key, end_off) : DRX_KEY_NONE;
      const uint32_t key_right = (uint32_t)__shfl_down((int)key, 1, 64);
      const uint32_t key0 = (uint32_t)__builtin_amdgcn_readlane((int)key, n > 0 ? e0 : 0);
      const bool seg_end = valid && (lane == end_off - 1 || key_right != key);
      const bool cont_left = key == key0 && prev_key == key;
      const bool cont_right = lane == end_off - 1 && next_key == key;
      const bool apply = seg_end && !cont_left && !cont_right;
      const uint32_t av = key < A.first_key[1] ? 0u : (key < A.first_key[2] ? 1u : 2u);
      const uint32_t row = key - (av == 0 ? A.first_key[0] : (av == 1 ? A.first_key[1] : A.first_key[2]));
      bool parked = false;
      if constexpr (Policy::kStreamParks) parked = apply && pol.stream_parked(av);
      const int w = valid ? (apply && !parked ? 3 : 1) : 0;
      int incl = w;
#pragma unroll
      for (int d = 1; d < 64; d <<= 1) {
        const int t = __shfl_up(incl, d, 64);
        if (lane >= d) incl += t;
      }
      const int pos = incl - w;
      const int M = __builtin_amdgcn_readlane(incl, 63);
      float sc = 0.f, sp = 0.f, ss = 0.f;
      uint32_t park_row = 0xFFFFFFFFu, park_scal = 0u;
      if (valid) {
        const uint32_t kind = 5u * av + (!seg_end || apply ? kItGrad : (cont_left ? kItGradHead : kItGradTail));
        tab[pos] = (val << 4) | kind;
        if (apply && !parked) { tab[pos + 1] = (row << 4) | (5u * av + kItParam); tab[pos + 2] = (row << 4) | (5u * av + kItSlot); }
        const float *const sg = av == 0 ? A.sgrad[0] : (av == 1 ? A.sgrad[1] : A.sgrad[2]);
        if (sg) {
          sc = sg[val];
          if (apply && !parked) {
            sp = (av == 0 ? A.sparam[0] : (av == 1 ? A.sparam[1] : A.sparam[2]))[row];
            ss = (av == 0 ? A.sslot[0] : (av == 1 ? A.sslot[1] : A.sslot[2]))[row];
          }
        }
        if constexpr (Policy::kStreamParks) {
// ... 72 lines not shown
                *reinterpret_cast<V *>(S.ptail + (size_t)g * LD + lane * VL) = acc;
                if (lane == 0) S.pts[g] = accs;
#pragma unroll
                for (int v = 0; v < VL; ++v) accf[v] = 0.f;
                accs = 0.f;
              }
            } else if (kind == kItParam) {
              prow = row;
            } else {
              V slotv = row;
              float *const sf = reinterpret_cast<float *>(&slotv);
#pragma unroll
              for (int v = 0; v < VL; ++v) pol.stream_update(fmaf(decay, pf[v], accf[v]), pf[v], sf[v]);
              const long long roff = (long long)idx * (LD * 4);
              ((GV *)(uintptr_t)(origin + offs[5u * av + kItParam] + roff))[lane] = prow;
              ((GV *)(uintptr_t)(origin + offs[5u * av + kItSlot] + roff))[lane] = slotv;
              float *const spar = av == 0 ? A.sparam[0] : (av == 1 ? A.sparam[1] : A.sparam[2]);
              if (spar) {
                float pb = __builtin_bit_cast(float, __builtin_amdgcn_readlane(__builtin_bit_cast(int, sp), at_lane));
                float ps = __builtin_bit_cast(float, __builtin_amdgcn_readlane(__builtin_bit_cast(int, ss), at_lane));
                pol.stream_update_scalar(accs, pb, ps);
                if (lane == 0) { spar[idx] = pb; (av == 0 ? A.sslot[0] : (av == 1 ? A.sslot[1] : A.sslot[2]))[idx] = ps; }
              }
#pragma unroll
              for (int v = 0; v < VL; ++v) accf[v] = 0.f;
              accs = 0.f;
            }
          }
        }
      }
      if (all_inner) *reinterpret_cast<V *>(comb + (size_t)wv * LD + lane * VL) = acc;
    }
    if (all_inner) {
      float *const sc = comb + (size_t)CPB * LD;
      if (lane == 0) sc[wv] = accs;
      __syncthreads();
      if (wv == 0) {
        V t;
        float *const tf = reinterpret_cast<float *>(&t);
#pragma unroll
        for (int v = 0; v < VL; ++v) tf[v] = 0.f;
        float ts = 0.f;
#pragma unroll
        for (int rr = 0; rr < CPB; ++rr) {
          const V x = *reinterpret_cast<const V *>(comb + (size_t)rr * LD + lane * VL);
          const float *const xf = reinterpret_cast<const float *>(&x);
#pragma unroll
          for (int v = 0; v < VL; ++v) tf[v] += xf[v];
          ts += sc[rr];
        }
        *reinterpret_cast<V *>(PB.pblock + (size_t)blk * LD + lane * VL) = t;
        if (lane == 0) PB.pbs[blk] = ts;
      }
    }
  }
}

template <int G> constexpr int kStreamThreads = (kSegBlock / G) * 64;

template <int G, int J, class Policy, class Front>
static int launch_reduce_streamed(const SegBufs &SB, const PlanBufs &PB, const SpanPlan &plan, const Policy &pol, int n_front,
                                  const Front &front, hipStream_t st) {
  if constexpr (kStreamBuilt<G, J, Policy>) {
    constexpr int cpb = kSegBlock / G;
    hipLaunchKernelGGL((k_seg_reduce_stream<4 * G, kStreamDepth, Policy, Front>), dim3(n_front + (SB.n_chunks + cpb - 1) / cpb),
                       dim3(kStreamThreads<G>), seg_stream_lds_bytes(SB.ld, kStreamDepth), st, SB, PB, plan, pol, n_front, front);
    return DRX_OK;
  }
  return DRX_EINVAL;
}

template <int G, int J, class Policy>
static int launch_reduce(ReduceForm form, const SegBufs &SB, const PlanBufs &PB, const SpanPlan &plan, const Policy &pol,
                         const BiasArgs &BA, hipStream_t st) {
  if (form == ReduceForm::Streamed)
    return launch_reduce_streamed<G, J>(SB, PB, plan, pol, BA.n_part, BiasPartialExtra<G, J, kStreamThreads<G>>{SB.ld, BA}, st);
  constexpr int cpb = kSegBlock / G;
  using Front = BiasPartialExtra<G, J>;
  const bool lng = form == ReduceForm::PlannedLong;
  const auto kernel = lng ? k_seg_reduce_planned<G, J, Policy, true, Front> : k_seg_reduce_planned<G, J, Policy, false, Front>;
  hipLaunchKernelGGL(kernel, dim3(BA.n_part + (SB.n_chunks + cpb - 1) / cpb), dim3(kSegBlock), seg_reduce_lds_bytes(cpb, SB.ld, lng), st,
                     SB, PB, plan, pol, BA.n_part, Front{SB.ld, BA});
  return DRX_OK;
}

constexpr int kSpanBlocks = kLongBlocks + kShortBlocks;
template <int G, int J, class Policy, class Extra>
static int launch_spans(const SegBufs &SB, const PlanBufs &PB, const SpanPlan &plan, const Policy &pol, int n_extra, const Extra &extra,
                        hipStream_t st) {
  const size_t lds = ((size_t)(kFixBlock / G) * (SB.ld + 1)) * 4;
  if (lds > 48 * 1024)
    DRX_HIP(hipFuncSetAttribute((const void *)k_span_planned<G, J, Policy, Extra>, hipFuncAttributeMaxDynamicSharedMemorySize, (int)lds));
  hipLaunchKernelGGL((k_span_planned<G, J, Policy, Extra>), dim3(kSpanBlocks + n_extra), dim3(kFixBlock), lds, st, SB, PB, plan, pol,
                     kLongBlocks, kShortBlocks, extra);
  return DRX_OK;
}

}
```

drecpy_amd/csrc/drx_sort.hip:

```cpp
#include <cstdlib>
#include <cstring>
#include <hip/hip_runtime.h>
#include "drx_common.hpp"

namespace drx {

#ifndef DRX_SORT_THREADS
#define DRX_SORT_THREADS 512
#endif
#ifndef DRX_SORT_IPT
#define DRX_SORT_IPT 16
#endif
constexpr int kSortThreads = DRX_SORT_THREADS;
constexpr int kSortWaves = kSortThreads / 64;
constexpr int kSortIPT = DRX_SORT_IPT;
constexpr int kSortTile = kSortThreads * kSortIPT;
constexpr int kMaxPasses = 4;
constexpr uint32_t kStAgg = 1u << 30, kStIncl = 2u << 30, kCountMask = (1u << 30) - 1;
constexpr int kDropNone = 1, kFirstPass = 2, kLastPass = 4;

struct SortPlan {
  int passes;
  int rbits[kMaxPasses];
  int shift[kMaxPasses];
// ... 268 lines not shown
    const uint32_t d = (k >> shift) & (RADIX - 1);
    const size_t o = (size_t)gbase[d] + (size_t)i;
    kout[o] = k;
    vout[o] = sval[i];
  }
  }
  if (next_hist) {
    for (int d = tid; d < RADIX; d += kSortThreads) {
      uint32_t c = 0;
#pragma unroll
      for (int r = 0; r < REP; ++r) c += nh[(d << REPB) + r];
      if (c) atomicAdd(&next_hist[d], c);
    }
  }
  if (drop && last)
    for (size_t i = n_valid + (size_t)blockIdx.x * kSortThreads + tid; i < n; i += (size_t)gridDim.x * kSortThreads) kout[i] = DRX_KEY_NONE;
}

#ifndef DRX_SORT_GRID
#define DRX_SORT_GRID 512
#endif
inline int sort_grid() { return DRX_SORT_GRID; }

constexpr size_t onesweep_lds_bytes(int r) { return ((size_t)(kSortWaves + 2) * ((size_t)1 << r) + 2 * (size_t)kSortTile + 2048) * 4; }
constexpr size_t kSortStaticLds = (2 + 2 * (size_t)kSortWaves) * 4;
constexpr size_t kSortLdsLimit = 160 * 1024;
static_assert(onesweep_lds_bytes(11) + kSortStaticLds <= kSortLdsLimit,
              "k_onesweep_pass<11>: tile (DRX_SORT_THREADS x DRX_SORT_IPT) + counters do not fit a workgroup's LDS");

template <int R>
static int launch_pass(const uint32_t *sk, const uint32_t *sv, uint32_t *dk, uint32_t *dv, size_t n, int shift, const uint32_t *gh, uint32_t *ticket,
                       uint32_t *desc, int tiles, int flags, uint32_t *next_hist, int next_shift, hipStream_t stream) {
  const size_t lds = onesweep_lds_bytes(R);
  if (lds > 48 * 1024) DRX_HIP(hipFuncSetAttribute((const void *)k_onesweep_pass<R>, hipFuncAttributeMaxDynamicSharedMemorySize, (int)lds));
  hipLaunchKernelGGL(k_onesweep_pass<R>, dim3(tiles < sort_grid() ? tiles : sort_grid()), dim3(kSortThreads), lds, stream, sk, sv, dk, dv, n, shift, gh,
                     ticket, desc, (uint32_t)tiles, flags, next_hist, next_shift);
  return 0;
}

size_t sort_pairs_temp_bytes(size_t n, int end_bit) {
  const SortPlan P = sort_plan(end_bit);
  return sort_layout(nullptr, n ? n : 1, P).total + 256;
}

void sort_pairs_zero_region(void *temp, size_t n, int end_bit, uint32_t **words, size_t *n_words) {
  const SortPlan P = sort_plan(end_bit);
  char *t = (char *)align_up((size_t)temp, 256);
  const SortLayout L = sort_layout(t, n ? n : 1, P);
  *words = (uint32_t *)(t + L.zero_begin);
  *n_words = L.zero_bytes / 4;
}

int sort_first_digit_bits(int end_bit) { return sort_plan(end_bit).rbits[0]; }

static int launch_first_counts(const SortPlan &P, const SortLayout &L, const uint32_t *kin, size_t n, bool drop_none, const SortRider &rider,
                               hipStream_t stream) {
  if (rider.partials) {
    if (P.rbits[0] != 8 || !drop_none || rider.partial_rows < 1) return DRX_EINVAL;
    const int cols = rider.keep_off ? kPartialWords : 256;
    hipLaunchKernelGGL(k_fold_counts, dim3(cols / kFoldCols), dim3(kFoldThreads), 0, stream, rider.partials, rider.partial_rows, L.hist,
                       rider.counts);
    return 0;
  }
  int hgrid = (int)((n + 8 * 512 - 1) / (8 * 512));
  if (hgrid > sort_grid()) hgrid = sort_grid();
  SortPlan P1 = P;
  P1.passes = 1;
  const int rider_blocks = rider.keep_off ? (rider.B + 511) / 512 : 0;
  hipLaunchKernelGGL(k_digit_histograms, dim3(hgrid + rider_blocks), dim3(512), 0, stream, kin, n, P1, L.hist, drop_none ? 1 : 0, rider,
                     rider_blocks);
  return 0;
}

int sort_first_counts(void *temp, size_t temp_bytes, const uint32_t *kin, size_t n, int end_bit, bool drop_none, hipStream_t stream,
                      SortRider rider, const uint32_t **hist) {
  if (n == 0 || n >= (1u << 30)) return DRX_EINVAL;
  const SortPlan P = sort_plan(end_bit);
  char *t = (char *)align_up((size_t)temp, 256);
  const SortLayout L = sort_layout(t, n, P);
  if ((size_t)(t - (char *)temp) + L.total > temp_bytes) return DRX_ESCRATCH;
  *hist = L.hist;
  const int rc = launch_first_counts(P, L, kin, n, drop_none, rider, stream);
  if (rc) return rc;
  DRX_LAUNCH_CHECK();
  return 0;
}

int sort_pairs_ex(void *temp, size_t temp_bytes, const uint32_t *kin, uint32_t *kout, const uint32_t *vin, uint32_t *vout, size_t n, int end_bit,
                  bool drop_none, hipStream_t stream, bool pre_zeroed, SortRider rider) {
  if (n == 0) return 0;
  if (n >= (1u << 30)) return DRX_EINVAL;
  const SortPlan P = sort_plan(end_bit);
  char *t = (char *)align_up((size_t)temp, 256);
  const SortLayout L = sort_layout(t, n, P);
  if ((size_t)(t - (char *)temp) + L.total > temp_bytes) return DRX_ESCRATCH;
  if (!pre_zeroed) DRX_HIP(hipMemsetAsync(t + L.zero_begin, 0, L.zero_bytes, stream));
  const int rc1 = launch_first_counts(P, L, kin, n, drop_none, rider, stream);
  if (rc1) return rc1;
  const uint32_t *src_k = kin, *src_v = vin;
  uint32_t *desc = L.desc;
  for (int p = 0; p < P.passes; ++p) {
    const bool to_out = ((P.passes - 1 - p) & 1) == 0;
    uint32_t *dk = to_out ? kout : L.tmp_k, *dv = to_out ? vout : L.tmp_v;
    const uint32_t *gh = L.hist + (size_t)p * 2048;
    const int flags = (drop_none ? kDropNone : 0) | (p == 0 ? kFirstPass : 0) | (p == P.passes - 1 ? kLastPass : 0);
    int rc;
// ... 45 lines not shown
```

drecpy_amd/engine.py:

```python
import ctypes as C
import math

import os
import time
import weakref

import numpy as np
import torch

from . import _lib
from ._lib import Batch, CdaeParams, History, Optim, check, lib, ptr, stream_ptr
from .engine_rows import ADAM_B1, ADAM_B2, ADAM_EPS, RowsRecommender, _round_up, pack_mask_bits

VAR_ORDER = ('W', 'W2T', 'V', 'b', 'b2')
ADAGRAD_INIT, ADAGRAD_EPS = 0.1, 1e-7


def _forget_prepared(addr):
    try:
        lib().drx_cdae_prep_forget(addr)
    except Exception:
        pass


# ... 352 lines not shown
            _lib.LOSS_BCE if loss == 'bce' else _lib.LOSS_MSE,
            (_lib.TARGETS_REFERENCE if targets == 'reference' else _lib.TARGETS_PER_ROW) | _lib.DENSE_AUX_CLEAN,
            ptr(sc), sc.numel(), ptr(self._loss) if want_loss else None, stream_ptr(self.device)),
            'drx_cdae_step_dense')
        self._dense_clean = self._dense_ent[1] = True
        return self._loss if want_loss else None

    _FIT_SLOTS = 16

    def fit_dense(self, drawahead, cursor, B, q, keep_capacity, first_step, n_steps, loss='bce', targets='reference'):
        L = lib()
        need = int(L.drx_cdae_fit_slot_bytes(B, int(keep_capacity)))
        slots = getattr(self, '_fit_slots', None)
        if slots is None or slots[0] < need:
            slots = self._fit_slots = (need, torch.empty(need * self._FIT_SLOTS, dtype=torch.uint8, pin_memory=True),
                                       torch.empty(2 * need, dtype=torch.uint8, device=self.device))
        o = self._optim([0.0] * 5)
        sc = self._ensure_dense_scratch(B)
        alphas = self._alpha_table(first_step, n_steps)
        self._dense_clean = self._dense_ent[1] = False
        check(L.drx_cdae_fit_dense(
            C.byref(self._params), C.byref(o), C.byref(self._hist), drawahead, cursor.ctypes.data, B, float(q), int(keep_capacity),
            _lib.LOSS_BCE if loss == 'bce' else _lib.LOSS_MSE, _lib.TARGETS_REFERENCE if targets == 'reference' else _lib.TARGETS_PER_ROW,
            n_steps, alphas.ctypes.data, slots[1].data_ptr(), slots[0], self._FIT_SLOTS, ptr(slots[2]), slots[2].numel(), ptr(sc),
            sc.numel(), stream_ptr(self.device)),
            'drx_cdae_fit_dense')
        self._dense_clean = self._dense_ent[1] = True

    def _retire(self, t):
        t.record_stream(torch.cuda.default_stream(self.device))
        t.record_stream(torch.cuda.current_stream(self.device))

    def prep_buffer(self, bt, out=None, hot=0):
        need = lib().drx_cdae_prep_bytes_hot(C.byref(self._params), bt.B, bt.n_touch_slots, hot) if hot else \
            lib().drx_cdae_prep_bytes(C.byref(self._params), bt.B, bt.n_touch_slots)
        if out is None or out.numel() < need:
            out = None
            out = torch.empty(int(need * 1.03) + 4096, dtype=torch.uint8, device=self.device)
        return out

    def prep_result_bytes(self, bt):
        return int(lib().drx_cdae_prep_result_bytes(C.byref(self._params), bt.B, bt.n_touch_slots))

    def prepare_sparse(self, bt, out=None, hot=False):
        H = self._hot_for(bt) if hot else 0
        out = self.prep_buffer(bt, out, H)
        if H:
            check(lib().drx_cdae_sparse_prepare_hot(C.byref(self._params), C.byref(self._hist), C.byref(bt), C.byref(self._hot_head(H)),
                                                    ptr(out), out.numel(), stream_ptr(self.device)), 'drx_cdae_sparse_prepare_hot')
        else:
            check(lib().drx_cdae_sparse_prepare(C.byref(self._params), C.byref(self._hist), C.byref(bt), ptr(out), out.numel(),
                                                stream_ptr(self.device)), 'drx_cdae_sparse_prepare')
        out._drx_hot = H
        if H and not getattr(out, '_drx_forget', None):
            out._drx_forget = weakref.finalize(out, _forget_prepared, out.data_ptr())
        return out

    def prepare_part(self, bt, part, parts, slot=None):
        P = C.byref(self._params)
        nb = int(lib().drx_cdae_prep_part_out_bytes(P, bt.B, bt.n_touch_slots, parts))
        if slot is None:
            out = torch.empty(nb, dtype=torch.uint8, device=self.device)
        else:
            bufs = self.__dict__.setdefault('_part_bufs', {})
            if slot not in bufs or bufs[slot].numel() < nb:
                if bufs.get(slot) is not None:
                    self._retire(bufs[slot])
                bufs[slot] = None
                bufs[slot] = torch.empty(int(nb * 1.05) + 4096, dtype=torch.uint8, device=self.device)
            out = bufs[slot][:nb]
        need = lib().drx_cdae_prep_part_bytes(P, bt.B, bt.n_touch_slots, parts)
        if getattr(self, '_pscratch', None) is None or self._pscratch.numel() < need:
            if getattr(self, '_pscratch', None) is not None:
                self._retire(self._pscratch)
            self._pscratch = None
            self._pscratch = torch.empty(int(need * 1.1) + 1024, dtype=torch.uint8, device=self.device)
        check(lib().drx_cdae_sparse_prepare_part(P, C.byref(self._hist), C.byref(bt), part, parts, ptr(out), out.numel(),
                                                 ptr(self._pscratch), self._pscratch.numel(), stream_ptr(self.device)),
              'drx_cdae_sparse_prepare_part')
        return out

    def prepare_assemble(self, bt, all_parts, parts, out=None, overflow=None):
        need = lib().drx_cdae_prep_bytes(C.byref(self._params), bt.B, bt.n_touch_slots)
        if out is None or out.numel() < need:
            out = torch.empty(int(need), dtype=torch.uint8, device=self.device)
        if overflow is None:
            overflow = torch.zeros(1, dtype=torch.int32, device=self.device)
        check(lib().drx_cdae_sparse_prepare_assemble(C.byref(self._params), C.byref(bt), ptr(all_parts), parts, ptr(out), out.numel(),
                                                     ptr(overflow), stream_ptr(self.device)), 'drx_cdae_sparse_prepare_assemble')
        return out, overflow

    def kshard_forward(self, bt, prepared=None):
        h = torch.empty(bt.B, self.ld, dtype=torch.float32, device=self.device)
        d = torch.empty(bt.B, dtype=torch.float32, device=self.device)
        check(lib().drx_cdae_kshard_forward_prepared(C.byref(self._params), C.byref(self._hist), C.byref(bt), ptr(prepared),
                                                     prepared.numel() if prepared is not None else 0, ptr(h), ptr(d),
                                                     stream_ptr(self.device)), 'drx_cdae_kshard_forward_prepared')
        return h, d

    def step_sparse(self, step, bt, loss='bce', want_loss=False, events=None, prepared=None, kshard=None, hot=False):
        a = self.adam_alpha(self.lr, step + 1, self.beta1, self.beta2)
        o = self._optim([a] * 5)
        H = int(getattr(prepared, '_drx_hot', 0)) if prepared is not None else (self._hot_for(bt) if hot else 0)
        sc = self._ensure_scratch(bt.B, bt.n_touch_slots, hot=H)
        lk = _lib.LOSS_BCE if loss == 'bce' else _lib.LOSS_MSE
        lo = ptr(self._loss) if want_loss else None
        arr = (C.c_void_p * len(events))(*[e.cuda_event for e in events]) if events is not None else None
# ... 358 lines not shown
```

include/drx.h:

```cpp
#ifndef DRX_H_
#define DRX_H_

#include <stddef.h>
#include <stdint.h>

#ifdef __cplusplus
extern "C" {
#endif

#define DRX_VERSION 100

enum {
  DRX_OK = 0,
  DRX_EINVAL = -1,
  DRX_ESCRATCH = -2,
  DRX_ENOTIMPL = -3,
  DRX_ERETRY = -4,
  DRX_ECOMM = -5
};

#define DRX_MAX_K 1024
#define DRX_KEY_NONE 0xFFFFFFFFu

enum { DRX_LOSS_BCE = 0, DRX_LOSS_MSE = 1 };
// ... 74 lines not shown
size_t drx_cdae_scratch_bytes(const DrxCdaeParams *p, int32_t B, int32_t n_touch_slots, int32_t dense_mode);

int drx_cdae_step_dense(const DrxCdaeParams *p, const DrxOptim *opt, const DrxHistory *hist,
                        const DrxBatch *bt, int32_t loss_kind, int32_t targets_kind,
                        void *scratch, size_t scratch_bytes, float *loss_out, void *stream);

int drx_cdae_step_sparse(const DrxCdaeParams *p, const DrxOptim *opt, const DrxHistory *hist,
                         const DrxBatch *bt, int32_t loss_kind,
                         void *scratch, size_t scratch_bytes, float *loss_out, void *stream);

#define DRX_SPARSE_PHASES 5
int drx_cdae_step_sparse_timed(const DrxCdaeParams *p, const DrxOptim *opt, const DrxHistory *hist,
                               const DrxBatch *bt, int32_t loss_kind, void *scratch, size_t scratch_bytes,
                               float *loss_out, void *const *events, void *stream);

size_t drx_cdae_prep_bytes(const DrxCdaeParams *p, int32_t B, int32_t n_touch_slots);
int drx_cdae_sparse_prepare(const DrxCdaeParams *p, const DrxHistory *hist, const DrxBatch *bt, void *prepared,
                            size_t prepared_bytes, void *stream);
int drx_cdae_step_sparse_prepared(const DrxCdaeParams *p, const DrxOptim *opt, const DrxHistory *hist, const DrxBatch *bt,
                                  int32_t loss_kind, const void *prepared, size_t prepared_bytes, void *scratch,
                                  size_t scratch_bytes, float *loss_out, void *const *events, void *stream);

typedef struct DrxHotHead {
  int32_t H;
  const int16_t *slot;
  const int32_t *item;
} DrxHotHead;
#define DRX_MAX_HOT 1024
size_t drx_cdae_prep_bytes_hot(const DrxCdaeParams *p, int32_t B, int32_t n_touch_slots, int32_t H);
size_t drx_cdae_scratch_bytes_hot(const DrxCdaeParams *p, int32_t B, int32_t n_touch_slots, int32_t H);
int drx_cdae_sparse_prepare_hot(const DrxCdaeParams *p, const DrxHistory *hist, const DrxBatch *bt, const DrxHotHead *hot,
                                void *prepared, size_t prepared_bytes, void *stream);
int drx_cdae_step_sparse_hot(const DrxCdaeParams *p, const DrxOptim *opt, const DrxHistory *hist, const DrxBatch *bt,
                             const DrxHotHead *hot, int32_t loss_kind, const void *prepared, size_t prepared_bytes, void *scratch,
                             size_t scratch_bytes, float *loss_out, void *const *events, void *stream);
int32_t drx_cdae_hot_rows_for(const DrxCdaeParams *p, int32_t opt_kind, int32_t B, int32_t n_touch_slots, int32_t H);
void drx_cdae_prep_forget(const void *prepared);

int drx_debug_prep_counts(const DrxCdaeParams *p, const DrxHistory *hist, const DrxBatch *bt, const DrxHotHead *hot, uint8_t *present,
                          int32_t ipr, int32_t cshift, int32_t world, void *prepared, size_t prepared_bytes, uint32_t *hist_out,
                          uint32_t *buckets_out, uint32_t *keys_out, uint32_t *vals_out, uint32_t *mask_out, int32_t *info_out,
                          void *stream);

int drx_debug_prep_result(const DrxCdaeParams *p, int32_t B, int32_t n_touch_slots, int32_t H, const void *prepared, size_t prepared_bytes,
                          uint32_t *keys_s_out, uint32_t *vals_s_out, uint8_t *solo_v_out, uint8_t *solo_o_out, int32_t *order_out,
                          void *stream);

int drx_debug_cdae_reduce(const DrxCdaeParams *p, const DrxOptim *opt, const DrxHistory *hist, const DrxBatch *bt, const DrxHotHead *hot,
                          const void *prepared, size_t prepared_bytes, const float *dz1_in, const float *g2_in, const float *dz2_in,
                          int32_t form, void *scratch, size_t scratch_bytes, void *stream);

int drx_debug_span_plan(const DrxCdaeParams *p, int32_t B, int32_t n_touch_slots, int32_t H, const void *prepared, size_t prepared_bytes,
                        uint8_t *ext_out, uint32_t *desc_out, uint32_t *cnt_out, void *stream);

int drx_batch_offsets(const int64_t *indptr, const int32_t *ids, int32_t B, int32_t *off, void *scratch, size_t scratch_bytes, void *stream);

size_t drx_point_sample_scratch_bytes(int32_t B);
int drx_point_sample(const DrxHistory *hist, int32_t n_users, int32_t n_items, int32_t B, int32_t neg_ratio,
                     uint64_t seed, int32_t *uid, int32_t *iid, float *y, int32_t *keep_off,
                     void *scratch, size_t scratch_bytes, uint64_t *host_mailbox, uint32_t tag, void *stream);
int drx_point_sample_recorded(const DrxHistory *hist, const DrxHistory *recorded, int32_t n_users, int32_t n_items, int32_t B,
                              int32_t neg_ratio, uint64_t seed, int32_t *uid, int32_t *iid, float *y, int32_t *keep_off,
                              void *scratch, size_t scratch_bytes, uint64_t *host_mailbox, uint32_t tag, void *stream);

size_t drx_point_sample_by_user_scratch_bytes(int32_t B, int32_t n_users);
int drx_point_sample_by_user(const DrxHistory *hist, const DrxHistory *recorded, int32_t n_users, int32_t n_items, int32_t B,
                             int32_t neg_ratio, uint64_t seed, int32_t *uid, int32_t *iid, float *y, int32_t *keep_off, void *scratch,
                             size_t scratch_bytes, uint64_t *host_mailbox, uint32_t tag, void *stream);

int drx_point_sample_valued(const DrxHistory *hist, const DrxHistory *recorded, const float *pos_values, float vmin, float vrange,
                            int32_t n_users, int32_t n_items, int32_t B, int32_t neg_ratio, uint64_t seed, int32_t *uid, int32_t *iid,
                            float *y, void *stream);

typedef struct DrxListGroups {
  const int64_t *indptr;
  const int32_t *seq_ids;
  const int64_t *held_indptr;
  const int32_t *held;
  const int32_t *group_value;
  const int32_t *eligible;
  int32_t n_groups, n_eligible, n_ids;
} DrxListGroups;
int drx_list_sample_device(const DrxListGroups *g, int32_t B, int32_t n_inputs, int32_t n_targets, int32_t neg_ratio, uint64_t seed,
                           int32_t *group_out, int32_t *before, int32_t *after, void *stream);

int drx_cdae_kshard_forward(const DrxCdaeParams *p, const DrxHistory *hist, const DrxBatch *bt, float *h_out ,
                            float *dot_partial , void *stream);
int drx_cdae_kshard_forward_prepared(const DrxCdaeParams *p, const DrxHistory *hist, const DrxBatch *bt, const void *prepared,
                                     size_t prepared_bytes, float *h_out , float *dot_partial , void *stream);
int drx_cdae_kshard_step(const DrxCdaeParams *p, const DrxOptim *opt, const DrxHistory *hist, const DrxBatch *bt, int32_t loss_kind,
                         const float *h, const float *dot_total, const void *prepared, size_t prepared_bytes, void *scratch,
                         size_t scratch_bytes, float *loss_out, void *const *events, void *stream);

size_t drx_cdae_prep_result_bytes(const DrxCdaeParams *p, int32_t B, int32_t n_touch_slots);

size_t drx_cdae_prep_part_out_bytes(const DrxCdaeParams *p, int32_t B, int32_t n_touch_slots, int32_t parts);
int drx_cdae_prep_part_layout(const DrxCdaeParams *p, int32_t B, int32_t n_touch_slots, int32_t parts, size_t *out4);
size_t drx_cdae_prep_part_bytes(const DrxCdaeParams *p, int32_t B, int32_t n_touch_slots, int32_t parts);
int drx_cdae_sparse_prepare_part(const DrxCdaeParams *p, const DrxHistory *hist, const DrxBatch *bt, int32_t part, int32_t parts,
                                 void *part_out, size_t part_out_bytes, void *scratch, size_t scratch_bytes, void *stream);
int drx_cdae_sparse_prepare_assemble(const DrxCdaeParams *p, const DrxBatch *bt, const void *all_parts, int32_t parts, void *prepared,
                                     size_t prepared_bytes, int32_t *overflow_out, void *stream);

#define DRX_MAX_WORLD 64
#define DRX_MAX_MICRO 4
#define DRX_MAX_CHUNKS 16
// ... 481 lines not shown
```

profiles/pmc_l2.py:

```python
import csv
import json
import sys
from collections import defaultdict


def main(path, out):
    acc = defaultdict(lambda: defaultdict(list))
    for r in csv.DictReader(open(path)):
        k = r['Kernel_Name'].split('(')[0].replace('void ', '')
        if 'drx::' in k:
            acc[k.split('<')[0]][r['Counter_Name']].append(float(r['Counter_Value']))
    med = lambda v: sorted(v)[len(v) // 2] if v else 0.0
    res = {}
    for k, c in sorted(acc.items()):
        h, m = med(c.get('TCC_HIT_sum', [])), med(c.get('TCC_MISS_sum', []))
        res[k] = {'TCC_HIT_sum': h, 'TCC_MISS_sum': m, 'l2_hit_rate': (h / (h + m)) if h + m else None}
        print(f"{k:40s} hit {h:14.0f} miss {m:14.0f} rate {res[k]['l2_hit_rate']}")
    json.dump(res, open(out, 'w'), indent=1)


if __name__ == '__main__':
    main(sys.argv[1], sys.argv[2])
```

profiles/pmc_summary.py:

```python
import csv
import json
import sys
from collections import defaultdict


def base_name(kernel):
    import re
    m = re.search(r'drx::(\w+)', kernel)
    return 'drx::' + m.group(1) if m else kernel.split('(')[0]


def per_kernel(path, counter):
    acc = defaultdict(list)
    for r in csv.DictReader(open(path)):
        if r['Counter_Name'] == counter:
            acc[base_name(r['Kernel_Name'])].append(float(r['Counter_Value']))
    return acc


def main(fetch_csv, write_csv, out):
    f = per_kernel(fetch_csv, 'FETCH_SIZE')
    w = per_kernel(write_csv, 'WRITE_SIZE')
    res = {}
    for k in sorted(set(f) | set(w)):
        if 'drx::' not in k and 'rocprim' not in k:
            continue
        fv, wv = f.get(k, []), w.get(k, [])
        med = lambda v: sorted(v)[len(v) // 2] if v else 0.0
        res[k] = {'launches': max(len(fv), len(wv)), 'fetch_bytes_corrected': 2.0 * med(fv) * 1024.0,
                  'write_bytes': med(wv) * 1024.0, 'fetch_raw_kib': med(fv), 'write_raw_kib': med(wv)}
        res[k]['hbm_bytes_per_launch'] = res[k]['fetch_bytes_corrected'] + res[k]['write_bytes']
    json.dump(res, open(out, 'w'), indent=1)
    for k, v in res.items():
        print(f"{k[:70]:70s} n={v['launches']:4d} fetch {v['fetch_bytes_corrected'] / 1e6:9.1f} MB  write {v['write_bytes'] / 1e6:9.1f} MB")


if __name__ == '__main__':
    main(*sys.argv[1:4])
```

Baseline: 219.6 million samples/s.

## Split streamed segment reduce into span and plain passes with predicted grid sizes

The streamed reduce now has a split mode. The first launch handles span-carrying blocks, and a second launch fuses the plain blocks with the long/short span finish, the bias final and the hot-row finish. Grid sizes come from block counts that the prepare step posts into pinned host memory, and blocks are walked in class-permuted order with a strided loop. The aim is to cut launch count and idle or oversized grids in the reduce and finish phases. The cost is extra host-device signalling and a dependence on predictions, with a fallback to full grids when no prediction is available.

```diff
diff --git a/drecpy_amd/_lib.py b/drecpy_amd/_lib.py
--- a/drecpy_amd/_lib.py
+++ b/drecpy_amd/_lib.py
@@ -192,6 +192,12 @@
                                         C.c_void_p]),
     'drx_debug_span_plan': (C.c_int, [C.POINTER(CdaeParams), C.c_int32, C.c_int32, C.c_int32, C.c_void_p, C.c_size_t, C.c_void_p,
                                       C.c_void_p, C.c_void_p, C.c_void_p]),
+    'drx_debug_block_classes': (C.c_int, [C.POINTER(CdaeParams), C.c_int32, C.c_int32, C.c_int32, C.c_void_p, C.c_size_t, C.c_void_p,
+                                          C.c_void_p, C.c_void_p]),
+    'drx_debug_block_classes_entries': (C.c_int32, [C.POINTER(CdaeParams), C.c_int32, C.c_int32]),
+    'drx_debug_split_prediction': (C.c_int, [C.c_void_p, C.POINTER(C.c_int32)]),
+    'drx_debug_split_grids': (None, [C.c_int32, C.c_int32, C.c_int32, C.c_int32]),
+    'drx_debug_split_reduce': (None, [C.c_int32]),
     'drx_cdae_step_sparse_hot': (C.c_int, [C.POINTER(CdaeParams), C.POINTER(Optim), C.POINTER(History), C.POINTER(Batch),
                                            C.POINTER(HotHead), C.c_int32, C.c_void_p, C.c_size_t, C.c_void_p, C.c_size_t,
                                            C.c_void_p, C.POINTER(C.c_void_p), C.c_void_p]),
diff --git a/drecpy_amd/csrc/drx_cdae.hip b/drecpy_amd/csrc/drx_cdae.hip
--- a/drecpy_amd/csrc/drx_cdae.hip
+++ b/drecpy_amd/csrc/drx_cdae.hip
@@ -9,6 +9,7 @@
 #include <type_traits>
 #include <mutex>
 #include <unordered_map>
+#include <vector>
 
 #ifdef DRX_STAMPS
 static unsigned long long *h_stamps = nullptr;
@@ -398,31 +399,35 @@
 using DirectPolicy = DirectPolicyT<-1>;
 using DirectPolicyAdagrad = DirectPolicyT<DRX_OPT_ADAGRAD>;
 
-template <int G, int J, int NT>
+template <int G, int J, int NT, int NB = (J == 1 ? 8 : 2)>
 __device__ __forceinline__ void bias_final_body(const DrxCdaeParams &P, const DrxOptim &opt, const BiasArgs &A,
                                                 float *lds , float *red) {
-  constexpr int R = NT / G;
-  const int lane = threadIdx.x % G, r = threadIdx.x / G;
-  float4 acc[J];
-#pragma unroll
-  for (int j = 0; j < J; ++j) acc[j] = f4_zero();
-  constexpr int NB = J == 1 ? 8 : 2;
-  for (int i = r; i < A.n_part; i += NB * R) {
-    float4 v[NB][J];
-#pragma unroll
-    for (int q = 0; q < NB; ++q) {
-#pragma unroll
-      for (int j = 0; j < J; ++j) v[q][j] = f4_zero();
-      if (i + q * R < A.n_part) load_row<G, J>(A.part, (size_t)(i + q * R), P.ld, lane, v[q]);
-    }
-#pragma unroll
-    for (int q = 0; q < NB; ++q)
-#pragma unroll
-      for (int j = 0; j < J; ++j) f4_add(acc[j], v[q][j]);
-  }
-  store_row<G, J>(lds, (size_t)r, P.ld, lane, acc);
+  static_assert(NT <= kFixBlock && kFixBlock % NT == 0 && NT % G == 0 && NT % 64 == 0, "whole logical groups and waves per turn");
+  constexpr int R = kFixBlock / G, RP = NT / G, TURNS = kFixBlock / NT;
+  const int lane = threadIdx.x % G, rp = threadIdx.x / G;
+#pragma unroll 1
+  for (int turn = 0; turn < TURNS; ++turn) {
+    const int r = turn * RP + rp;
+    float4 acc[J];
+#pragma unroll
+    for (int j = 0; j < J; ++j) acc[j] = f4_zero();
+    for (int i = r; i < A.n_part; i += NB * R) {
+      float4 v[NB][J];
+#pragma unroll
+      for (int q = 0; q < NB; ++q) {
+#pragma unroll
+        for (int j = 0; j < J; ++j) v[q][j] = f4_zero();
+        if (i + q * R < A.n_part) load_row<G, J>(A.part, (size_t)(i + q * R), P.ld, lane, v[q]);
+      }
+#pragma unroll
+      for (int q = 0; q < NB; ++q)
+#pragma unroll
+        for (int j = 0; j < J; ++j) f4_add(acc[j], v[q][j]);
+    }
+    store_row<G, J>(lds, (size_t)r, P.ld, lane, acc);
+  }
   __syncthreads();
-  if (r == 0) {
+  if (rp == 0) {
     float4 g[J], w[J];
 #pragma unroll
     for (int j = 0; j < J; ++j) g[j] = f4_zero();
@@ -441,21 +446,31 @@
   }
   if (A.loss_out) {
     const float *lp = A.part + (size_t)A.n_part * P.ld;
-    float a = 0.f;
-    for (int b = threadIdx.x; b < A.n_part; b += NT) a += lp[b];
-    float t = block_sum(a, red);
-    if (threadIdx.x == 0) { A.loss_out[0] = t / (float)A.B; A.loss_out[1] = 0.f; }
-  }
-}
-
-template <int G, int J>
+#pragma unroll 1
+    for (int turn = 0; turn < TURNS; ++turn) {
+      float a = 0.f;
+      for (int b = turn * NT + (int)threadIdx.x; b < A.n_part; b += kFixBlock) a += lp[b];
+      a = group_sum<64>(a);
+      if ((threadIdx.x & 63) == 0) red[turn * (NT / 64) + (int)(threadIdx.x >> 6)] = a;
+    }
+    __syncthreads();
+    if (threadIdx.x == 0) {
+      float t = 0.f;
+      for (int i = 0; i < kFixBlock / 64; ++i) t += red[i];
+      A.loss_out[0] = t / (float)A.B;
+      A.loss_out[1] = 0.f;
+    }
+  }
+}
+
+template <int G, int J, int NT = kFixBlock>
 struct BiasFinalExtra {
   DrxCdaeParams P;
   DrxOptim opt;
   BiasArgs A;
   __device__ __forceinline__ void operator()(float *lds) const {
     __shared__ float red[kFixBlock / 64];
-    bias_final_body<G, J, kFixBlock>(P, opt, A, lds, red);
+    bias_final_body<G, J, NT>(P, opt, A, lds, red);
   }
 };
 
@@ -580,37 +595,63 @@
   }
 };
 
+template <int LD, int NT, class Policy>
+__device__ __forceinline__ void hot_finish_body(const HotArgs &A, const Policy &pol, float *lds) {
+  constexpr int NQ = kFixBlock / LD, QP = NT / LD, TURNS = kFixBlock / NT;
+  static_assert(NQ >= 1 && kFixBlock % LD == 0 && NT % LD == 0 && NT <= kFixBlock && kFixBlock % NT == 0, "a row per workgroup");
+  const int h = (int)blockIdx.x - A.first;
+  if (h >= A.H) return;
+  const uint32_t bit = 1u << (h & 31);
+  bool touched = false;
+  for (int s = (int)threadIdx.x; s < A.S; s += NT) touched |= (A.any[(size_t)s * (A.H / 32) + (h >> 5)] & bit) != 0u;
+  if (!__syncthreads_or(touched)) return;
+  const int c = (int)threadIdx.x % LD, qp = (int)threadIdx.x / LD;
+  const int per = (A.S + NQ - 1) / NQ;
+#pragma unroll
+  for (int turn = 0; turn < TURNS; ++turn) {
+    const int q = turn * QP + qp, s0 = q * per, s1 = min(A.S, s0 + per);
+    float sum = 0.f;
+#pragma unroll 8
+    for (int s = s0; s < s1; ++s) sum += A.part[((size_t)s * A.H + h) * LD + c];
+    lds[q * LD + c] = sum;
+  }
+  __syncthreads();
+  if (qp == 0) {
+    float t = lds[c];
+#pragma unroll
+    for (int k = 1; k < NQ; ++k) t += lds[k * LD + c];
+    const StreamArrays SA = pol.stream_arrays();
+    const size_t off = (size_t)A.item[h] * LD + c;
+    float pv = SA.table[0][off], av = SA.slot[0][off];
+    pol.stream_update(fmaf(pol.stream_decay(), pv, A.scale * t), pv, av);
+    SA.table[0][off] = pv;
+    SA.slot[0][off] = av;
+  }
+}
 template <int LD, class Policy>
 struct HotFinishExtra {
   HotArgs A;
   Policy pol;
-  __device__ __forceinline__ void operator()(float *lds) const {
-    constexpr int NT = kFixBlock, NQ = NT / LD;
-    static_assert(NQ >= 1 && NT % LD == 0, "a row per workgroup");
-    const int h = (int)blockIdx.x - A.first;
-    if (h >= A.H) return;
-    const uint32_t bit = 1u << (h & 31);
-    bool touched = false;
-    for (int s = (int)threadIdx.x; s < A.S; s += NT) touched |= (A.any[(size_t)s * (A.H / 32) + (h >> 5)] & bit) != 0u;
-    if (!__syncthreads_or(touched)) return;
-    const int c = (int)threadIdx.x % LD, q = (int)threadIdx.x / LD;
-    const int per = (A.S + NQ - 1) / NQ, s0 = q * per, s1 = min(A.S, s0 + per);
-    float sum = 0.f;
-#pragma unroll 8
-    for (int s = s0; s < s1; ++s) sum += A.part[((size_t)s * A.H + h) * LD + c];
-    lds[q * LD + c] = sum;
-    __syncthreads();
-    if (q == 0) {
-      float t = lds[c];
-#pragma unroll
-      for (int k = 1; k < NQ; ++k) t += lds[k * LD + c];
-      const StreamArrays SA = pol.stream_arrays();
-      const size_t off = (size_t)A.item[h] * LD + c;
-      float pv = SA.table[0][off], av = SA.slot[0][off];
-      pol.stream_update(fmaf(pol.stream_decay(), pv, A.scale * t), pv, av);
-      SA.table[0][off] = pv;
-      SA.slot[0][off] = av;
-    }
+  __device__ __forceinline__ void operator()(float *lds) const { hot_finish_body<LD, kFixBlock>(A, pol, lds); }
+};
+
+#ifndef DRX_SPLIT_FRONT_ROWS
+#define DRX_SPLIT_FRONT_ROWS 4
+#endif
+template <int G, int J, class Policy, bool HOT>
+struct SplitFinishFront {
+  int n_long, n_short;
+  BiasArgs BA;
+  HotArgs HA;
+  __device__ __forceinline__ void operator()(float *lds, const SegBufs &S, const PlanBufs &PB, const SpanPlan &SP, const Policy &pol) const {
+    constexpr int NT = kStreamThreads<G>, kFrontRows = DRX_SPLIT_FRONT_ROWS;
+    const int b = (int)blockIdx.x;
+    if (b < n_long) span_long_planned_body<G, J, NT, kFrontRows>(S, PB, SP, pol, b, n_long, lds);
+    else if (b < n_long + n_short) span_short_planned_body<G, J, NT, kFrontRows>(S, PB, SP, pol, b - n_long, n_short);
+    else if (b == n_long + n_short) {
+      __shared__ float red[kFixBlock / 64];
+      bias_final_body<G, J, NT, kFrontRows>(pol.P, pol.opt, BA, lds, red);
+    } else if constexpr (HOT) hot_finish_body<4 * G, NT>(HA, pol, lds);
   }
 };
 
@@ -649,17 +690,49 @@
   return S;
 }
 
+struct PrepRecord { int H = 0; unsigned long long *post = nullptr; };
 static std::mutex g_hot_mu;
-static std::unordered_map<const void *, int> g_hot_of;
+static std::unordered_map<const void *, PrepRecord> g_hot_of;
+static std::vector<unsigned long long *> g_post_pool;
 static void hot_record(const void *prepared, int H) {
   std::lock_guard<std::mutex> lk(g_hot_mu);
-  if (H > 0) g_hot_of[prepared] = H;
-  else g_hot_of.erase(prepared);
+  g_hot_of[prepared].H = H;
 }
 static int hot_recorded(const void *prepared) {
   std::lock_guard<std::mutex> lk(g_hot_mu);
   const auto it = g_hot_of.find(prepared);
-  return it == g_hot_of.end() ? 0 : it->second;
+  return it == g_hot_of.end() ? 0 : it->second.H;
+}
+static unsigned long long *post_of(const void *prepared, bool create) {
+  std::lock_guard<std::mutex> lk(g_hot_mu);
+  if (!create) {
+    const auto it = g_hot_of.find(prepared);
+    return it == g_hot_of.end() ? nullptr : it->second.post;
+  }
+  PrepRecord &r = g_hot_of[prepared];
+  if (!r.post) {
+    if (!g_post_pool.empty()) { r.post = g_post_pool.back(); g_post_pool.pop_back(); }
+    else {
+      void *m = nullptr;
+      if (hipHostMalloc(&m, 2 * sizeof(unsigned long long), hipHostMallocPortable) != hipSuccess) { (void)hipGetLastError(); m = nullptr; }
+      r.post = (unsigned long long *)m;
+    }
+    if (r.post) { __atomic_store_n(r.post, 0ull, __ATOMIC_RELAXED); __atomic_store_n(r.post + 1, 0ull, __ATOMIC_RELAXED); }
+  }
+  return r.post;
+}
+static BlockCounts predicted_counts(const void *prepared) {
+  const unsigned long long *post = prepared ? post_of(prepared, false) : nullptr;
+  if (!post) return BlockCounts{0, 0, 0, 0, 0};
+  const unsigned long long w0 = __atomic_load_n(post, __ATOMIC_ACQUIRE), w1 = __atomic_load_n(post + 1, __ATOMIC_RELAXED);
+  return BlockCounts::unpack(w0, w1);
+}
+static void prep_forget(const void *prepared) {
+  std::lock_guard<std::mutex> lk(g_hot_mu);
+  const auto it = g_hot_of.find(prepared);
+  if (it == g_hot_of.end()) return;
+  if (it->second.post) g_post_pool.push_back(it->second.post);
+  g_hot_of.erase(it);
 }
 
 struct HotBufs { float *part; uint32_t *any; float *bpart; };
@@ -704,32 +777,70 @@
 template <int G, int J, class Policy>
 static int reduce_and_finish(ReduceForm form, const DrxCdaeParams &P, const DrxOptim &opt, const SparseBufs &S, const SegBufs &SB,
                              const PlanBufs &PB, const SpanPlan &plan, const BiasArgs &BA, const HotArgs &HA, void *const *events,
-                             hipStream_t st) {
+                             hipStream_t st, bool split, const BlockCounts &pred) {
   const Policy pol{P, opt, BA.B, HA.scale, S.dz1, (long long)(S.g2 - S.dz1), S.dz2};
   const BiasFinalExtra<G, J> bias{P, opt, BA};
   int rc = DRX_EINVAL;
-  if (HA.H == 0) rc = launch_reduce<G, J>(form, SB, PB, plan, pol, BA, st);
-  else if constexpr (kHotBuilt<G, J, Policy>) {
-    constexpr int NT = kStreamThreads<G>;
-    HotArgs part = HA;
+  if (form != ReduceForm::Streamed) {
+    if (HA.H != 0) return DRX_EINVAL;
+    rc = launch_reduce<G, J>(form, SB, PB, plan, pol, BA, st);
+    if (rc) return rc;
+    DRX_HIP(phase_event(events, 3, st));
+    rc = launch_spans<G, J>(SB, PB, plan, pol, 1, bias, st);
+    if (rc) return rc;
+    DRX_HIP(phase_event(events, 4, st));
+    DRX_HIP(phase_event(events, 5, st));
+    return DRX_OK;
+  }
+  if constexpr (kStreamBuilt<G, J, Policy>) {
+    constexpr int NT = kStreamThreads<G>, cpb = kSegBlock / G;
+    const int full = stream_full_grid<G>(SB);
+    const bool strided = split_reduce_mode() >= 0 && kStreamStrided<G>;
+    const bool have = strided && pred.cpb != 0, same = pred.cpb == cpb;
+    const long long real_p = !have ? -1 : (same ? pred.real_blocks : ((long long)pred.real_blocks * pred.cpb + cpb - 1) / cpb);
+    const long long span_p = !have ? -1 : (same ? pred.span_blocks : real_p), plain_p = !have ? -1 : (same ? real_p - span_p : 0);
+    const int span_groups = (split ? NT : kFixBlock) / G;
+    const int n_long = predicted_grid(have ? pred.n_long : -1, kLongBlocks, g_split_force[2]);
+    const int n_short = predicted_grid(have ? (pred.n_short + span_groups - 1) / span_groups : -1, kShortBlocks, g_split_force[3]);
+    HotArgs part = HA, fin = HA;
     part.first = 0;
+    fin.first = n_long + n_short + 1;
     const int n_hot = (HA.S * hot_groups(HA.H) * (G / 4) + NT / 64 - 1) / (NT / 64);
-    rc = launch_reduce_streamed<G, J>(SB, PB, plan, pol, n_hot, HotPartialExtra<4 * G, NT>{part}, st);
-  }
-  if (rc) return rc;
-  DRX_HIP(phase_event(events, 3, st));
-  rc = DRX_EINVAL;
-  if (HA.H == 0) rc = launch_spans<G, J>(SB, PB, plan, pol, 1, bias, st);
-  else if constexpr (kHotBuilt<G, J, Policy>) {
-    HotArgs fin = HA;
-    fin.first = kSpanBlocks + 1;
-    using Finish = ExtraPair<BiasFinalExtra<G, J>, HotFinishExtra<4 * G, Policy>>;
-    rc = launch_spans<G, J>(SB, PB, plan, pol, 1 + HA.H, Finish{bias, fin.first, {fin, pol}}, st);
-  }
-  if (rc) return rc;
-  DRX_HIP(phase_event(events, 4, st));
-  DRX_HIP(phase_event(events, 5, st));
-  return DRX_OK;
+    const int mode1 = split ? kStreamSpan : kStreamAll;
+    const int grid1 = predicted_grid(split ? span_p : real_p, full, g_split_force[0]);
+    if (HA.H == 0)
+      rc = launch_reduce_streamed<G, J>(SB, PB, plan, pol, BA.n_part, BiasPartialExtra<G, J, NT>{SB.ld, BA}, st, mode1, grid1, strided);
+    else if constexpr (kHotBuilt<G, J, Policy>)
+      rc = launch_reduce_streamed<G, J>(SB, PB, plan, pol, n_hot, HotPartialExtra<4 * G, NT>{part}, st, mode1, grid1, strided);
+    if (rc) return rc;
+    if (split) {
+      rc = DRX_EINVAL;
+      if constexpr (kSplitBuilt<G, J, Policy>) {
+        const int grid2 = predicted_grid(plain_p, full, g_split_force[1]);
+        if (HA.H == 0)
+          rc = launch_reduce_streamed<G, J>(SB, PB, plan, pol, n_long + n_short + 1, SplitFinishFront<G, J, Policy, false>{n_long, n_short, BA, fin},
+                                            st, kStreamPlain, grid2, true);
+        else if constexpr (kHotBuilt<G, J, Policy>)
+          rc = launch_reduce_streamed<G, J>(SB, PB, plan, pol, n_long + n_short + 1 + HA.H,
+                                            SplitFinishFront<G, J, Policy, true>{n_long, n_short, BA, fin}, st, kStreamPlain, grid2, true);
+      }
+      if (rc) return rc;
+      DRX_HIP(phase_event(events, 3, st));
+    } else {
+      DRX_HIP(phase_event(events, 3, st));
+      rc = DRX_EINVAL;
+      if (HA.H == 0) rc = launch_spans<G, J>(SB, PB, plan, pol, 1, bias, st, n_long, n_short);
+      else if constexpr (kHotBuilt<G, J, Policy>) {
+        using Finish = ExtraPair<BiasFinalExtra<G, J>, HotFinishExtra<4 * G, Policy>>;
+        rc = launch_spans<G, J>(SB, PB, plan, pol, 1 + HA.H, Finish{bias, fin.first, {fin, pol}}, st, n_long, n_short);
+      }
+      if (rc) return rc;
+    }
+    DRX_HIP(phase_event(events, 4, st));
+    DRX_HIP(phase_event(events, 5, st));
+    return DRX_OK;
+  }
+  return rc;
 }
 
 }
@@ -828,11 +939,13 @@
     if (rc) return rc;
   }
   DRX_HIP(phase_event(events, 2, st));
+  const bool split = split_reduce_applies(form, p->ld, prepared != nullptr, share, ks_h != nullptr);
+  const BlockCounts pred = form == ReduceForm::Streamed ? predicted_counts(prepared) : BlockCounts{0, 0, 0, 0, 0};
   rc = dispatch_geom(p->ld, [&](auto g) -> int {
     constexpr int G = decltype(g)::G, J = decltype(g)::J;
     return opt->kind == DRX_OPT_ADAGRAD
-        ? reduce_and_finish<G, J, DirectPolicyAdagrad>(form, *p, *opt, S, SB, PB, R.plan, BA, HA, events, st)
-        : reduce_and_finish<G, J, DirectPolicy>(form, *p, *opt, S, SB, PB, R.plan, BA, HA, events, st);
+        ? reduce_and_finish<G, J, DirectPolicyAdagrad>(form, *p, *opt, S, SB, PB, R.plan, BA, HA, events, st, split, pred)
+        : reduce_and_finish<G, J, DirectPolicy>(form, *p, *opt, S, SB, PB, R.plan, BA, HA, events, st, false, pred);
   });
   if (rc) return rc;
   DRX_LAUNCH_CHECK();
@@ -856,7 +969,8 @@
   PrepBufs R = prep_layout(cp, *p, bt->B, bt->n_touch_slots);
   if (!cp.ok()) return DRX_ESCRATCH;
   hot_record(prepared, 0);
-  rc = prepare_impl(p, hist, bt, R, (hipStream_t)stream, true);
+  rc = prepare_impl(p, hist, bt, R, (hipStream_t)stream, true, TouchPresence{nullptr, WireGeo{1, 0, 1}}, nullptr, nullptr,
+                    R.plan.bperm ? post_of(prepared, true) : nullptr);
   if (rc) return rc;
   if (p->ld <= 16) order_by_degree(bt, R, (hipStream_t)stream, true);
   DRX_LAUNCH_CHECK();
@@ -968,7 +1082,8 @@
   PrepBufs R = prep_layout(cp, *p, bt->B, bt->n_touch_slots, hot->H);
   if (!cp.ok()) return DRX_ESCRATCH;
   hot_record(prepared, 0);
-  rc = prepare_impl(p, hist, bt, R, (hipStream_t)stream, true, TouchPresence{nullptr, WireGeo{1, 0, 1}}, hot->slot, hot->item);
+  rc = prepare_impl(p, hist, bt, R, (hipStream_t)stream, true, TouchPresence{nullptr, WireGeo{1, 0, 1}}, hot->slot, hot->item,
+                    R.plan.bperm ? post_of(prepared, true) : nullptr);
   if (rc) return rc;
   hot_record(prepared, hot->H);
   if (p->ld <= 16) order_by_degree(bt, R, (hipStream_t)stream, true);
@@ -1072,7 +1187,46 @@
 }
 
 void drx_cdae_prep_forget(const void *prepared) {
-  if (prepared) hot_record(prepared, 0);
-}
-
-}
+  if (prepared) prep_forget(prepared);
+}
+
+int drx_debug_block_classes(const DrxCdaeParams *p, int32_t B, int32_t n_touch_slots, int32_t H, const void *prepared, size_t prepared_bytes,
+                            uint32_t *perm_out, uint32_t *info_out, void *stream) {
+  int rc = check_params(p);
+  if (rc) return rc;
+  if (B < 1 || n_touch_slots < 0 || hot_rows(p, H) < 0 || !prepared || !perm_out || !info_out) return DRX_EINVAL;
+  Carver cp(const_cast<void *>(prepared), prepared_bytes);
+  const PrepBufs R = prep_layout(cp, *p, B, n_touch_slots, H);
+  if (!cp.ok()) return DRX_ESCRATCH;
+  if (!R.plan.bperm) return DRX_EINVAL;
+  hipStream_t st = (hipStream_t)stream;
+  DRX_HIP(hipMemsetAsync(info_out, 0, 8 * sizeof(uint32_t), st));
+  DRX_HIP(hipMemcpyAsync(perm_out, R.plan.bperm, (size_t)R.plan.xstride * sizeof(uint32_t), hipMemcpyDeviceToDevice, st));
+  DRX_HIP(hipMemcpyAsync(info_out, R.plan.cnt + kSplitSpan, 2 * sizeof(uint32_t), hipMemcpyDeviceToDevice, st));
+  DRX_HIP(hipMemcpyAsync(info_out + 2, R.plan.cnt, 2 * sizeof(uint32_t), hipMemcpyDeviceToDevice, st));
+  DRX_HIP(hipMemcpyAsync(info_out + 4, R.plan.cnt + kSplitReal, sizeof(uint32_t), hipMemcpyDeviceToDevice, st));
+  DRX_HIP(hipMemcpyAsync(info_out + 5, R.plan.cnt + kSplitCpb, sizeof(uint32_t), hipMemcpyDeviceToDevice, st));
+  return DRX_OK;
+}
+
+int32_t drx_debug_block_classes_entries(const DrxCdaeParams *p, int32_t B, int32_t n_touch_slots) {
+  if (!p || B < 1 || n_touch_slots < 0) return 0;
+  Carver c(nullptr, 0);
+  const PrepBufs R = prep_layout(c, *p, B, n_touch_slots);
+  return long_segments(R.T, *p) ? 0 : R.plan.xstride;
+}
+
+int drx_debug_split_prediction(const void *prepared, int32_t *out) {
+  if (!prepared || !out) return DRX_EINVAL;
+  const BlockCounts c = predicted_counts(prepared);
+  out[0] = c.cpb; out[1] = c.real_blocks; out[2] = c.span_blocks; out[3] = c.n_short; out[4] = c.n_long;
+  return DRX_OK;
+}
+
+void drx_debug_split_grids(int32_t first, int32_t second, int32_t n_long, int32_t n_short) {
+  g_split_force[0] = first; g_split_force[1] = second; g_split_force[2] = n_long; g_split_force[3] = n_short;
+}
+
+void drx_debug_split_reduce(int32_t on) { g_split_override = on; }
+
+}
diff --git a/drecpy_amd/csrc/drx_common.hpp b/drecpy_amd/csrc/drx_common.hpp
--- a/drecpy_amd/csrc/drx_common.hpp
+++ b/drecpy_amd/csrc/drx_common.hpp
@@ -172,6 +172,8 @@
 int sort_first_counts(void *temp, size_t temp_bytes, const uint32_t *kin, size_t n, int end_bit, bool drop_none, hipStream_t stream,
                       SortRider rider, const uint32_t **hist);
 
+void sort_first_hist(void *temp, size_t n, int end_bit, const uint32_t **hist, int *n_digits);
+
 inline int bits_for(uint64_t max_key_exclusive) {
   int b = 1;
   while (b < 32 && (1ull << b) < max_key_exclusive) ++b;
diff --git a/drecpy_amd/csrc/drx_prep.hpp b/drecpy_amd/csrc/drx_prep.hpp
--- a/drecpy_amd/csrc/drx_prep.hpp
+++ b/drecpy_amd/csrc/drx_prep.hpp
@@ -1,5 +1,6 @@
 #pragma once
 #include <algorithm>
+#include <cstdlib>
 #include "drx_common.hpp"
 #include "drx_rows.hpp"
 #include "drx_segreduce.hpp"
@@ -319,10 +320,27 @@
   }
 }
 
+struct BlockCounts {
+  int cpb, real_blocks, span_blocks, n_short, n_long;
+  __host__ __device__ static unsigned long long pack(int cpb, uint32_t real_blocks, uint32_t span_blocks) {
+    return (1ull << 63) | ((unsigned long long)(cpb & 127) << 56) | ((unsigned long long)(real_blocks & 0xFFFFFFFu) << 28) |
+           (unsigned long long)(span_blocks & 0xFFFFFFFu);
+  }
+  static BlockCounts unpack(unsigned long long w0, unsigned long long w1) {
+    if (!(w0 >> 63)) return BlockCounts{0, 0, 0, 0, 0};
+    return BlockCounts{(int)((w0 >> 56) & 127), (int)((w0 >> 28) & 0xFFFFFFFu), (int)(w0 & 0xFFFFFFFu), (int)(w1 >> 32), (int)(w1 & 0xFFFFFFFFu)};
+  }
+};
+struct BlockClassArgs {
+  const uint32_t *digit_hist;
+  int n_digits;
+  unsigned long long *post;
+};
+
 static __global__ __launch_bounds__(256) void k_plan_and_mark(uint32_t *keys_s, const uint32_t *__restrict__ vals_s, int T, int n_chunks, int cpb,
                                                        SpanPlan P, uint32_t n_items, int B, uint8_t *solo_v, uint8_t *solo_o,
                                                        int order_blocks, const int32_t *keep_off, unsigned int *order_work,
-                                                       int32_t *order) {
+                                                       int32_t *order, BlockClassArgs bc) {
   const int plan_blocks = (int)gridDim.x - order_blocks;
   if ((int)blockIdx.x >= plan_blocks) {
     __shared__ unsigned int lds[768];
@@ -330,6 +348,34 @@
     return;
   }
   const int tid = blockIdx.x * blockDim.x + threadIdx.x;
+  if (bc.digit_hist) {
+    __shared__ unsigned int s_real;
+    if (threadIdx.x == 0) s_real = 0u;
+    __syncthreads();
+    unsigned int part = 0u;
+    for (int i = (int)threadIdx.x; i < bc.n_digits; i += (int)blockDim.x) part += bc.digit_hist[i];
+#pragma unroll
+    for (int o = 32; o > 0; o >>= 1) part += (unsigned int)__shfl_xor((int)part, o, 64);
+    if ((threadIdx.x & 63) == 0 && part) atomicAdd(&s_real, part);
+    __syncthreads();
+    const long long real = min((long long)s_real, (long long)T), block_touches = (long long)cpb * P.chunk;
+    const int nb_real = (int)((real + block_touches - 1) / block_touches);
+    if ((tid & ~63) < nb_real) {
+      const bool on = tid < nb_real;
+      bool bears = false;
+      if (on)
+        for (int c = tid * cpb; c < (tid + 1) * cpb && (long long)c * P.chunk < real; ++c) bears |= chunk_bears_span(keys_s, T, P.chunk, c);
+      const unsigned long long m_span = __ballot(on && bears), m_plain = __ballot(on && !bears);
+      const int lane = threadIdx.x & 63;
+      uint32_t base = 0u;
+      if (lane == 0 && m_span) base = atomicAdd(&P.cnt[kSplitSpan], (uint32_t)__popcll(m_span));
+      if (lane == 1 && m_plain) base = atomicAdd(&P.cnt[kSplitPlain], (uint32_t)__popcll(m_plain));
+      base = (uint32_t)__shfl((int)base, bears ? 0 : 1, 64);
+      const uint32_t rank = base + (uint32_t)__popcll((bears ? m_span : m_plain) & ((1ull << lane) - 1ull));
+      if (on) P.bperm[bears ? rank : (uint32_t)P.xstride - 1u - rank] = (uint32_t)tid;
+    }
+    if (tid == 0) { P.cnt[kSplitCpb] = (uint32_t)cpb; P.cnt[kSplitReal] = (uint32_t)real; }
+  }
   const int real = P.xrank ? (int)P.cnt[20] : 0;
   if (tid < n_chunks && (real == 0 || (long long)tid * P.chunk < (long long)real)) plan_chunk(keys_s, T, n_chunks, cpb, P, tid);
   const int nb = (n_chunks + cpb - 1) / cpb;
@@ -344,6 +390,18 @@
     if (k < 2 * n_items) solo_o[b] = 1;
     else solo_v[b] = 1;
     keys_s[j] = DRX_KEY_NONE;
+  }
+  if (bc.digit_hist && bc.post) {
+    __syncthreads();
+    if (threadIdx.x == 0) {
+      if (atomicAdd(&P.cnt[kSplitTicket], 1u) == (uint32_t)plan_blocks - 1u) {
+        const uint32_t n_span = atomicAdd(&P.cnt[kSplitSpan], 0u), n_plain = atomicAdd(&P.cnt[kSplitPlain], 0u);
+        const uint32_t n_short = atomicAdd(&P.cnt[0], 0u), n_long = atomicAdd(&P.cnt[1], 0u);
+        __hip_atomic_store(bc.post + 1, ((unsigned long long)n_short << 32) | (unsigned long long)n_long, __ATOMIC_RELAXED,
+                           __HIP_MEMORY_SCOPE_SYSTEM);
+        __hip_atomic_store(bc.post, BlockCounts::pack(cpb, n_span + n_plain, n_span), __ATOMIC_RELAXED, __HIP_MEMORY_SCOPE_SYSTEM);
+      }
+    }
   }
 }
 
@@ -468,6 +526,28 @@
   return form == ReduceForm::Streamed && pick_geom(ld).G <= kHotMaxG && !share && !kshard;
 }
 
+template <int G, int J, class Policy>
+constexpr bool kSplitBuilt = kStreamBuilt<G, J, Policy> && G <= kHotMaxG && DRX_STREAM_PLACED == 0;
+[[maybe_unused]] static int g_split_override = -1;
+static inline int split_reduce_mode() {
+  static const int env = [] { const char *e = getenv("DRX_SPLIT_REDUCE"); return !e || !e[0] ? -1 : (e[0] == '0' ? 0 : 1); }();
+  return g_split_override >= 0 ? (g_split_override != 0 ? 1 : 0) : env;
+}
+static inline bool split_reduce_wanted() { return split_reduce_mode() == 1; }
+static inline bool split_reduce_applies(ReduceForm form, int ld, bool prepared, bool share, bool kshard) {
+  return form == ReduceForm::Streamed && pick_geom(ld).G <= kHotMaxG && DRX_STREAM_PLACED == 0 && prepared && !share && !kshard &&
+         split_reduce_wanted();
+}
+constexpr int kGridMarginNum = 9, kGridMarginDen = 8;
+struct SplitGrids { int first, second, n_long, n_short; };
+[[maybe_unused]] static int g_split_force[4] = {-1, -1, -1, -1};
+static inline int predicted_grid(long long predicted, int full, int forced) {
+  if (forced >= 0) return forced < 1 ? 1 : (forced < full ? forced : full);
+  if (predicted < 0) return full;
+  const long long g = (predicted * kGridMarginNum + kGridMarginDen - 1) / kGridMarginDen + 8;
+  return (int)(g < full ? g : full);
+}
+
 static inline bool forward_per_workgroup(int B, int n_touch_slots) {
   const long long mean_hist = n_touch_slots / (long long)B;
   return mean_hist > 64 || (B <= 8192 && mean_hist > 16);
@@ -502,6 +582,7 @@
     const bool placed_any = placed || DRX_STREAM_PLACED != 0;
     R.plan.xrank = placed_any ? cv.take<uint32_t>((size_t)R.plan.xstride) : nullptr;
     R.plan.xperm = placed_any ? cv.take<uint32_t>((size_t)R.plan.xstride) : nullptr;
+    R.plan.bperm = placed ? nullptr : cv.take<uint32_t>((size_t)R.plan.xstride);
     R.usamp = placed ? cv.take<int32_t>(B) : nullptr;
     R.pitem = placed ? cv.take<int32_t>(B) : nullptr;
     R.witem = placed ? cv.take<WorkItem>((size_t)B) : nullptr;
@@ -826,7 +907,7 @@
 
 static int prepare_impl(const DrxCdaeParams *p, const DrxHistory *hist, const DrxBatch *bt, const PrepBufs &R, hipStream_t st,
                         bool with_marks = false, TouchPresence pres = TouchPresence{nullptr, WireGeo{1, 0, 1}},
-                        const int16_t *hot_slot = nullptr, const int32_t *hot_item = nullptr) {
+                        const int16_t *hot_slot = nullptr, const int32_t *hot_item = nullptr, unsigned long long *post = nullptr) {
   if (R.H > 0 && (!hot_slot || !hot_item || !hot_list_fits(R.T, *p, pres.present != nullptr))) return DRX_EINVAL;
   if (hist->t_rank && hist->t_users && hist->t_pos && hist->t_items && !pres.present && long_segments(R.T, *p)) {
     const int32_t *row_end = nullptr;
@@ -840,7 +921,7 @@
         const int blocks = std::max(2048, (R.n_chunks + 255) / 256);
         hipLaunchKernelGGL(k_plan_and_mark, dim3(blocks), dim3(256), 0, st, R.keys_s, R.vals_s, R.T, R.n_chunks,
                            kSegBlock / pick_geom(p->ld).G, Rb.plan, (uint32_t)p->n_items, bt->B, R.solo_v, R.solo_o, 0, bt->keep_off,
-                           R.order_work, R.order);
+                           R.order_work, R.order, BlockClassArgs{nullptr, 0, nullptr});
         if (R.plan.xrank) hipLaunchKernelGGL(k_place_blocks, dim3(256), dim3(256), 0, st, Rb.plan, R.n_chunks);
         return DRX_OK;
       }
@@ -856,9 +937,11 @@
   if (with_marks && p->ld > 16) {
     const int blocks = std::max(2048, (R.n_chunks + 255) / 256);
     const int order_blocks = (bt->B + 255) / 256;
+    BlockClassArgs bc{nullptr, 0, post};
+    if (R.plan.bperm && split_reduce_mode() >= 0) sort_first_hist(R.sort_temp, (size_t)R.T, R.bits, &bc.digit_hist, &bc.n_digits);
     hipLaunchKernelGGL(k_plan_and_mark, dim3(blocks + order_blocks), dim3(256), 0, st, R.keys_s, R.vals_s, R.T, R.n_chunks,
                        kSegBlock / pick_geom(p->ld).G, R.plan, (uint32_t)p->n_items, bt->B, R.solo_v, R.solo_o,
-                       order_blocks, bt->keep_off, R.order_work, R.order);
+                       order_blocks, bt->keep_off, R.order_work, R.order, bc);
     if (R.plan.xrank) hipLaunchKernelGGL(k_place_blocks, dim3(256), dim3(256), 0, st, R.plan, R.n_chunks);
     return DRX_OK;
   }
diff --git a/drecpy_amd/csrc/drx_segreduce.hpp b/drecpy_amd/csrc/drx_segreduce.hpp
--- a/drecpy_amd/csrc/drx_segreduce.hpp
+++ b/drecpy_amd/csrc/drx_segreduce.hpp
@@ -143,7 +143,18 @@
   int chunk;
   const int32_t *row_end;
   uint32_t row_end_keys;
+  uint32_t *bperm;
 };
+constexpr int kSplitSpan = 100, kSplitPlain = 101, kSplitCpb = 102, kSplitReal = 103, kSplitTicket = 104;
+
+__device__ __forceinline__ bool chunk_bears_span(const uint32_t *__restrict__ keys_s, int T, int CH, int c) {
+  const long long s = (long long)c * CH;
+  const uint32_t first = keys_s[s];
+  const uint32_t last = s + CH <= T ? keys_s[s + CH - 1] : DRX_KEY_NONE;
+  if (last != DRX_KEY_NONE && s + 2 * CH <= T && keys_s[s + 2 * CH - 1] == last) return true;
+  if (first == DRX_KEY_NONE || c == 0 || keys_s[s - 1] != first) return false;
+  return last == first || (c >= 2 && keys_s[s - CH - 1] == first);
+}
 #ifndef DRX_STREAM_PLACED
 #define DRX_STREAM_PLACED 0
 #endif
@@ -537,94 +548,114 @@
   }
 }
 
+template <int J> constexpr int kSpanRows = J == 1 ? 8 : 2;
+template <int G, int J, int NT, int UL, class Policy>
+__device__ __forceinline__ void span_short_planned_body(const SegBufs &S, const PlanBufs &PB, const SpanPlan &SP, const Policy &pol, int wg,
+                                                        int n_wgs) {
+  constexpr int R = NT / G, CPB = kSegBlock / G;
+  const int lane = threadIdx.x % G, r = threadIdx.x / G;
+  const uint32_t n_short = SP.cnt[0];
+  for (uint32_t si = (uint32_t)wg * R + r; si < n_short; si += (uint32_t)n_wgs * R) {
+    const uint2 d = SP.desc[si];
+    const SpanShape sh(d, CPB);
+    const int g0 = (int)d.x, tot = sh.total();
+    const int kpos = min(S.T, (g0 + 1) * SP.chunk) - 1;
+    float4 t[J];
+    load_row<G, J>(S.ptail, (size_t)g0, S.ld, lane, t);
+    float ts = S.pts[g0];
+    for (int i0 = 0; i0 < tot; i0 += UL) {
+      float4 v[UL][J];
+      float sv[UL];
+#pragma unroll
+      for (int u = 0; u < UL; ++u) {
+        sv[u] = 0.f;
+#pragma unroll
+        for (int j = 0; j < J; ++j) v[u][j] = f4_zero();
+        if (i0 + u < tot) span_partial<G, J>(S, PB, sh, CPB, i0 + u, lane, v[u], sv[u]);
+      }
+#pragma unroll
+      for (int u = 0; u < UL; ++u) {
+#pragma unroll
+        for (int j = 0; j < J; ++j) f4_add(t[j], v[u][j]);
+        ts += sv[u];
+      }
+    }
+    pol.template finish<G, J>(S.keys_s[kpos], kpos, lane, t, ts);
+  }
+}
+
+template <int G, int J, int NT, int UL, class Policy>
+__device__ __forceinline__ void span_long_planned_body(const SegBufs &S, const PlanBufs &PB, const SpanPlan &SP, const Policy &pol, int wg,
+                                                       int n_wgs, float *lds) {
+  static_assert(NT <= kFixBlock && kFixBlock % NT == 0 && NT % G == 0, "whole slices per group");
+  constexpr int RL = kFixBlock / G, RP = NT / G, TURNS = kFixBlock / NT, CPB = kSegBlock / G;
+  const int lane = threadIdx.x % G, rp = threadIdx.x / G;
+  float *sc = lds + (size_t)RL * S.ld;
+  const uint32_t n_long = SP.cnt[1];
+  for (uint32_t si = (uint32_t)wg; si < n_long; si += (uint32_t)n_wgs) {
+    const uint2 d = SP.desc[S.n_chunks - 1 - (int)si];
+    const SpanShape sh(d, CPB);
+    const int g0 = (int)d.x, tot = sh.total();
+    const int kpos = min(S.T, (g0 + 1) * SP.chunk) - 1;
+    const int per = (tot + RL - 1) / RL;
+    if (TURNS > 1) __syncthreads();
+#pragma unroll 1
+    for (int turn = 0; turn < TURNS; ++turn) {
+      const int r = turn * RP + rp;
+      float4 acc[J];
+#pragma unroll
+      for (int j = 0; j < J; ++j) acc[j] = f4_zero();
+      float accs = 0.f;
+      const int i_lo = r * per, i_hi = min(tot, i_lo + per);
+      for (int i0 = i_lo; i0 < i_hi; i0 += UL) {
+        float4 v[UL][J];
+        float sv[UL];
+#pragma unroll
+        for (int u = 0; u < UL; ++u) {
+          sv[u] = 0.f;
+#pragma unroll
+          for (int j = 0; j < J; ++j) v[u][j] = f4_zero();
+          if (i0 + u < i_hi) span_partial<G, J>(S, PB, sh, CPB, i0 + u, lane, v[u], sv[u]);
+        }
+#pragma unroll
+        for (int u = 0; u < UL; ++u) {
+#pragma unroll
+          for (int j = 0; j < J; ++j) f4_add(acc[j], v[u][j]);
+          accs += sv[u];
+        }
+      }
+      if (TURNS == 1) __syncthreads();
+      store_row<G, J>(lds, (size_t)r, S.ld, lane, acc);
+      if (lane == 0) sc[r] = accs;
+    }
+    __syncthreads();
+    if (rp == 0) {
+      float4 t[J];
+      load_row<G, J>(S.ptail, (size_t)g0, S.ld, lane, t);
+      float ts = S.pts[g0];
+#pragma unroll(kSpanRows<J> == UL ? 8 : UL)
+      for (int rr = 0; rr < RL; ++rr) {
+        float4 v[J];
+        load_row<G, J>(lds, (size_t)rr, S.ld, lane, v);
+#pragma unroll
+        for (int j = 0; j < J; ++j) f4_add(t[j], v[j]);
+        ts += sc[rr];
+      }
+      pol.template finish<G, J>(S.keys_s[kpos], kpos, lane, t, ts);
+    }
+  }
+}
+
 template <int G, int J, class Policy, class Extra>
 __global__ __launch_bounds__(kFixBlock) void k_span_planned(SegBufs S, PlanBufs PB, SpanPlan SP, Policy pol, int n_long_blocks,
                                                             int n_short_blocks, Extra extra) {
   extern __shared__ __align__(16) float span_lds[];
-  constexpr int R = kFixBlock / G, CPB = kSegBlock / G;
-  const int lane = threadIdx.x % G, r = threadIdx.x / G;
-  constexpr int UL = J == 1 ? 8 : 2;
   if ((int)blockIdx.x >= n_long_blocks + n_short_blocks) { extra(span_lds); return; }
   if ((int)blockIdx.x >= n_long_blocks) {
-    const uint32_t n_short = SP.cnt[0];
-    for (uint32_t si = ((int)blockIdx.x - n_long_blocks) * R + r; si < n_short; si += (uint32_t)n_short_blocks * R) {
-      const uint2 d = SP.desc[si];
-      const SpanShape sh(d, CPB);
-      const int g0 = (int)d.x, tot = sh.total();
-      const int kpos = min(S.T, (g0 + 1) * SP.chunk) - 1;
-      float4 t[J];
-      load_row<G, J>(S.ptail, (size_t)g0, S.ld, lane, t);
-      float ts = S.pts[g0];
-      for (int i0 = 0; i0 < tot; i0 += UL) {
-        float4 v[UL][J];
-        float sv[UL];
-#pragma unroll
-        for (int u = 0; u < UL; ++u) {
-          sv[u] = 0.f;
-#pragma unroll
-          for (int j = 0; j < J; ++j) v[u][j] = f4_zero();
-          if (i0 + u < tot) span_partial<G, J>(S, PB, sh, CPB, i0 + u, lane, v[u], sv[u]);
-        }
-#pragma unroll
-        for (int u = 0; u < UL; ++u) {
-#pragma unroll
-          for (int j = 0; j < J; ++j) f4_add(t[j], v[u][j]);
-          ts += sv[u];
-        }
-      }
-      pol.template finish<G, J>(S.keys_s[kpos], kpos, lane, t, ts);
-    }
+    span_short_planned_body<G, J, kFixBlock, kSpanRows<J>>(S, PB, SP, pol, (int)blockIdx.x - n_long_blocks, n_short_blocks);
     return;
   }
-  float *sc = span_lds + (size_t)R * S.ld;
-  const uint32_t n_long = SP.cnt[1];
-  for (uint32_t si = blockIdx.x; si < n_long; si += (uint32_t)n_long_blocks) {
-    const uint2 d = SP.desc[S.n_chunks - 1 - (int)si];
-    const SpanShape sh(d, CPB);
-    const int g0 = (int)d.x, tot = sh.total();
-    const int kpos = min(S.T, (g0 + 1) * SP.chunk) - 1;
-    float4 acc[J];
-#pragma unroll
-    for (int j = 0; j < J; ++j) acc[j] = f4_zero();
-    float accs = 0.f;
-    const int per = (tot + R - 1) / R;
-    const int i_lo = r * per, i_hi = min(tot, i_lo + per);
-    for (int i0 = i_lo; i0 < i_hi; i0 += UL) {
-      float4 v[UL][J];
-      float sv[UL];
-#pragma unroll
-      for (int u = 0; u < UL; ++u) {
-        sv[u] = 0.f;
-#pragma unroll
-        for (int j = 0; j < J; ++j) v[u][j] = f4_zero();
-        if (i0 + u < i_hi) span_partial<G, J>(S, PB, sh, CPB, i0 + u, lane, v[u], sv[u]);
-      }
-#pragma unroll
-      for (int u = 0; u < UL; ++u) {
-#pragma unroll
-        for (int j = 0; j < J; ++j) f4_add(acc[j], v[u][j]);
-        accs += sv[u];
-      }
-    }
-    __syncthreads();
-    store_row<G, J>(span_lds, (size_t)r, S.ld, lane, acc);
-    if (lane == 0) sc[r] = accs;
-    __syncthreads();
-    if (r == 0) {
-      float4 t[J];
-      load_row<G, J>(S.ptail, (size_t)g0, S.ld, lane, t);
-      float ts = S.pts[g0];
-#pragma unroll 8
-      for (int rr = 0; rr < R; ++rr) {
-        float4 v[J];
-        load_row<G, J>(span_lds, (size_t)rr, S.ld, lane, v);
-#pragma unroll
-        for (int j = 0; j < J; ++j) f4_add(t[j], v[j]);
-        ts += sc[rr];
-      }
-      pol.template finish<G, J>(S.keys_s[kpos], kpos, lane, t, ts);
-    }
-  }
+  span_long_planned_body<G, J, kFixBlock, kSpanRows<J>>(S, PB, SP, pol, (int)blockIdx.x, n_long_blocks, span_lds);
 }
 
 
diff --git a/drecpy_amd/csrc/drx_segstream.hpp b/drecpy_amd/csrc/drx_segstream.hpp
--- a/drecpy_amd/csrc/drx_segstream.hpp
+++ b/drecpy_amd/csrc/drx_segstream.hpp
@@ -37,9 +37,18 @@
 
 enum : uint32_t { kItGrad = 0, kItGradHead = 1, kItGradTail = 2, kItParam = 3, kItSlot = 4 };
 
-template <int LD, int D, class Policy, class Extra>
+template <class E, class Policy>
+__device__ __forceinline__ auto run_front(const E &e, float *lds, const SegBufs &S, const PlanBufs &PB, const SpanPlan &SP, const Policy &pol, int)
+    -> decltype(e(lds, S, PB, SP, pol)) { return e(lds, S, PB, SP, pol); }
+template <class E, class Policy>
+__device__ __forceinline__ void run_front(const E &e, float *lds, const SegBufs &, const PlanBufs &, const SpanPlan &, const Policy &, long) { e(lds); }
+
+enum : int { kStreamAll = 0, kStreamSpan = 1, kStreamPlain = 2 };
+template <int G> constexpr bool kStreamStrided = G <= 32;
+
+template <int LD, int D, class Policy, class Extra, bool STRIDED = false>
 __global__ __launch_bounds__((kSegBlock / (LD / 4)) * 64) DRX_STREAM_SGPR_CAP void k_seg_reduce_stream(SegBufs S, PlanBufs PB, SpanPlan SP, Policy pol,
-                                                                               int extra_blocks, Extra extra) {
+                                                                               int extra_blocks, Extra extra, int mode) {
   extern __shared__ __align__(16) float seg_lds[];
   constexpr int G = LD / 4;
   constexpr int CPB = kSegBlock / G;
@@ -52,7 +61,7 @@
   static_assert(LD == 64 || LD == 128 || LD == 256, "one, two or four rows per KiB");
   static_assert(D >= 2 && D <= 32, "ring depth");
   static_assert(2 * CH <= 64 && 3 * CPB <= 64, "a window is one touch per lane; a block's border keys one per lane");
-  if ((int)blockIdx.x < extra_blocks) { extra(seg_lds); return; }
+  if ((int)blockIdx.x < extra_blocks) { run_front(extra, seg_lds, S, PB, SP, pol, 0); return; }
   const int lane = threadIdx.x & 63, wv = __builtin_amdgcn_readfirstlane((int)(threadIdx.x >> 6));
   const uint32_t *__restrict__ const ks = S.keys_s, *__restrict__ const vs = S.vals_s;
   const uint8_t *__restrict__ const ext = SP.ext;
@@ -74,13 +83,36 @@
   const float decay = pol.stream_decay();
   const int sub = lane / LPI, piece = lane % LPI;
 
+  const int n_wg = (int)gridDim.x - extra_blocks, slot0 = (int)blockIdx.x - extra_blocks;
+#if DRX_STREAM_PLACED
+  const int count = slot0 + 1;
+  constexpr bool classed = false;
+#else
+  const int last_entry = SP.xstride - 1;
+  uint32_t perm0 = 0u;
+  bool classed = false;
+  int count = slot0 + 1;
+  if constexpr (STRIDED) {
+    const bool perm = mode != kStreamAll && SP.bperm != nullptr;
+    if (perm) perm0 = SP.bperm[mode == kStreamPlain ? max(0, last_entry - slot0) : min(slot0, last_entry)];
+    const uint32_t made = SP.cnt[kSplitCpb], real = SP.cnt[kSplitReal];
+    const uint32_t of_class = SP.cnt[mode == kStreamPlain ? kSplitPlain : kSplitSpan];
+    classed = perm && made == (uint32_t)CPB;
+    count = (S.n_chunks + CPB - 1) / CPB;
+    if (made != 0u) count = min(count, (int)(((long long)real + CPB * CH - 1) / (CPB * CH)));
+    if (classed) count = (int)of_class;
+    else if (mode == kStreamPlain) count = 0;
+  }
+#endif
+  for (int slot = slot0; slot < count; slot = STRIDED ? slot + n_wg : count) {
   struct Meta { uint32_t key, val, bk, prevk; int e0, e1; } m;
 #if DRX_STREAM_PLACED == 2
   const int pb_ = placed_block(SP, (int)blockIdx.x, extra_blocks, (int)gridDim.x - extra_blocks, CPB);
   const int blk = pb_ < -5 ? pb_ : (int)blockIdx.x - extra_blocks;
+#elif DRX_STREAM_PLACED
+  const int blk = placed_block(SP, (int)blockIdx.x, extra_blocks, (int)gridDim.x - extra_blocks, CPB);
 #else
-  const int blk = DRX_STREAM_PLACED ? placed_block(SP, (int)blockIdx.x, extra_blocks, (int)gridDim.x - extra_blocks, CPB)
-                                    : (int)blockIdx.x - extra_blocks;
+  const int blk = !classed ? slot : (int)(slot == slot0 ? perm0 : SP.bperm[mode == kStreamPlain ? last_entry - slot : slot]);
 #endif
   if (blk < 0) return;
   {
@@ -95,7 +127,7 @@
     const int p = role == 0 ? c * CH : (role == 1 ? (c + 1) * CH - 1 : c * CH - 1);
     m.bk = lane < 3 * CPB && c < S.n_chunks && (c + 1) * CH <= S.T && p >= 0 ? ks[p] : DRX_KEY_NONE;
   }
-  wave_lds_sync();
+  if (slot == slot0) wave_lds_sync();
   {
     const uint32_t bl = (uint32_t)__shfl((int)m.bk, lane + CPB, 64), bp = (uint32_t)__shfl((int)m.bk, lane + 2 * CPB, 64);
     const bool inner = lane < CPB && m.bk != DRX_KEY_NONE && m.bk == bp && bl == m.bk;
@@ -274,19 +306,35 @@
         *reinterpret_cast<V *>(PB.pblock + (size_t)blk * LD + lane * VL) = t;
         if (lane == 0) PB.pbs[blk] = ts;
       }
+      if (STRIDED && slot + n_wg < count) __syncthreads();
     }
   }
+  }
 }
 
 template <int G> constexpr int kStreamThreads = (kSegBlock / G) * 64;
+
+template <int G> static inline int stream_full_grid(const SegBufs &SB) { return (SB.n_chunks + kSegBlock / G - 1) / (kSegBlock / G); }
 
 template <int G, int J, class Policy, class Front>
 static int launch_reduce_streamed(const SegBufs &SB, const PlanBufs &PB, const SpanPlan &plan, const Policy &pol, int n_front,
-                                  const Front &front, hipStream_t st) {
+                                  const Front &front, hipStream_t st, int mode = kStreamAll, int n_wgs = 0, bool strided = false) {
   if constexpr (kStreamBuilt<G, J, Policy>) {
-    constexpr int cpb = kSegBlock / G;
-    hipLaunchKernelGGL((k_seg_reduce_stream<4 * G, kStreamDepth, Policy, Front>), dim3(n_front + (SB.n_chunks + cpb - 1) / cpb),
-                       dim3(kStreamThreads<G>), seg_stream_lds_bytes(SB.ld, kStreamDepth), st, SB, PB, plan, pol, n_front, front);
+    const int full = stream_full_grid<G>(SB);
+    if (!kStreamStrided<G>) strided = false;
+    if (n_wgs < 1 || n_wgs > full || !strided) n_wgs = full;
+    if (!strided && mode != kStreamAll) return DRX_EINVAL;
+    const size_t lds = seg_stream_lds_bytes(SB.ld, kStreamDepth);
+    if (mode == kStreamPlain && (size_t)(kFixBlock / G) * (SB.ld + 1) * 4 > lds) return DRX_EINVAL;
+    if constexpr (kStreamStrided<G>) {
+      if (strided) {
+        hipLaunchKernelGGL((k_seg_reduce_stream<4 * G, kStreamDepth, Policy, Front, true>), dim3(n_front + n_wgs), dim3(kStreamThreads<G>), lds,
+                           st, SB, PB, plan, pol, n_front, front, mode);
+        return DRX_OK;
+      }
+    }
+    hipLaunchKernelGGL((k_seg_reduce_stream<4 * G, kStreamDepth, Policy, Front, false>), dim3(n_front + n_wgs), dim3(kStreamThreads<G>), lds, st,
+                       SB, PB, plan, pol, n_front, front, mode);
     return DRX_OK;
   }
   return DRX_EINVAL;
@@ -309,12 +357,12 @@
 constexpr int kSpanBlocks = kLongBlocks + kShortBlocks;
 template <int G, int J, class Policy, class Extra>
 static int launch_spans(const SegBufs &SB, const PlanBufs &PB, const SpanPlan &plan, const Policy &pol, int n_extra, const Extra &extra,
-                        hipStream_t st) {
+                        hipStream_t st, int n_long_blocks = kLongBlocks, int n_short_blocks = kShortBlocks) {
   const size_t lds = ((size_t)(kFixBlock / G) * (SB.ld + 1)) * 4;
   if (lds > 48 * 1024)
     DRX_HIP(hipFuncSetAttribute((const void *)k_span_planned<G, J, Policy, Extra>, hipFuncAttributeMaxDynamicSharedMemorySize, (int)lds));
-  hipLaunchKernelGGL((k_span_planned<G, J, Policy, Extra>), dim3(kSpanBlocks + n_extra), dim3(kFixBlock), lds, st, SB, PB, plan, pol,
-                     kLongBlocks, kShortBlocks, extra);
+  hipLaunchKernelGGL((k_span_planned<G, J, Policy, Extra>), dim3(n_long_blocks + n_short_blocks + n_extra), dim3(kFixBlock), lds, st, SB, PB,
+                     plan, pol, n_long_blocks, n_short_blocks, extra);
   return DRX_OK;
 }
 
diff --git a/drecpy_amd/csrc/drx_sort.hip b/drecpy_amd/csrc/drx_sort.hip
--- a/drecpy_amd/csrc/drx_sort.hip
+++ b/drecpy_amd/csrc/drx_sort.hip
@@ -344,6 +344,13 @@
 }
 
 int sort_first_digit_bits(int end_bit) { return sort_plan(end_bit).rbits[0]; }
+
+void sort_first_hist(void *temp, size_t n, int end_bit, const uint32_t **hist, int *n_digits) {
+  const SortPlan P = sort_plan(end_bit);
+  char *t = (char *)align_up((size_t)temp, 256);
+  *hist = sort_layout(t, n ? n : 1, P).hist;
+  *n_digits = 1 << P.rbits[0];
+}
 
 static int launch_first_counts(const SortPlan &P, const SortLayout &L, const uint32_t *kin, size_t n, bool drop_none, const SortRider &rider,
                                hipStream_t stream) {
diff --git a/drecpy_amd/engine.py b/drecpy_amd/engine.py
--- a/drecpy_amd/engine.py
+++ b/drecpy_amd/engine.py
@@ -428,7 +428,7 @@
             check(lib().drx_cdae_sparse_prepare(C.byref(self._params), C.byref(self._hist), C.byref(bt), ptr(out), out.numel(),
                                                 stream_ptr(self.device)), 'drx_cdae_sparse_prepare')
         out._drx_hot = H
-        if H and not getattr(out, '_drx_forget', None):
+        if not getattr(out, '_drx_forget', None):
             out._drx_forget = weakref.finalize(out, _forget_prepared, out.data_ptr())
         return out
 
diff --git a/include/drx.h b/include/drx.h
--- a/include/drx.h
+++ b/include/drx.h
@@ -150,6 +150,13 @@
 
 int drx_debug_span_plan(const DrxCdaeParams *p, int32_t B, int32_t n_touch_slots, int32_t H, const void *prepared, size_t prepared_bytes,
                         uint8_t *ext_out, uint32_t *desc_out, uint32_t *cnt_out, void *stream);
+
+int drx_debug_block_classes(const DrxCdaeParams *p, int32_t B, int32_t n_touch_slots, int32_t H, const void *prepared, size_t prepared_bytes,
+                            uint32_t *perm_out, uint32_t *info_out, void *stream);
+int32_t drx_debug_block_classes_entries(const DrxCdaeParams *p, int32_t B, int32_t n_touch_slots);
+int drx_debug_split_prediction(const void *prepared, int32_t *out);
+void drx_debug_split_grids(int32_t first, int32_t second, int32_t n_long, int32_t n_short);
+void drx_debug_split_reduce(int32_t on);
 
 int drx_batch_offsets(const int64_t *indptr, const int32_t *ids, int32_t B, int32_t *off, void *scratch, size_t scratch_bytes, void *stream);
 
diff --git a/profiles/pmc_l2.py b/profiles/pmc_l2.py
--- a/profiles/pmc_l2.py
+++ b/profiles/pmc_l2.py
@@ -5,11 +5,19 @@
 
 
 def main(path, out):
-    acc = defaultdict(lambda: defaultdict(list))
+    import os
+    sys.path.insert(0, os.path.dirname(os.path.abspath(__file__)))
+    from pmc_summary import per_step
+    rows = defaultdict(lambda: defaultdict(list))
     for r in csv.DictReader(open(path)):
         k = r['Kernel_Name'].split('(')[0].replace('void ', '')
         if 'drx::' in k:
-            acc[k.split('<')[0]][r['Counter_Name']].append(float(r['Counter_Value']))
+            rows[k.split('<')[0]][r['Counter_Name']].append((int(r.get('Dispatch_Id') or 0), r['Kernel_Name'], float(r['Counter_Value'])))
+    acc = defaultdict(dict)
+    for k, c in rows.items():
+        for name, v in c.items():
+            v.sort(key=lambda t: t[0])
+            acc[k][name] = per_step([t[1] for t in v], [t[2] for t in v])
     med = lambda v: sorted(v)[len(v) // 2] if v else 0.0
     res = {}
     for k, c in sorted(acc.items()):
diff --git a/profiles/pmc_summary.py b/profiles/pmc_summary.py
--- a/profiles/pmc_summary.py
+++ b/profiles/pmc_summary.py
@@ -10,11 +10,24 @@
     return 'drx::' + m.group(1) if m else kernel.split('(')[0]
 
 
+def per_step(full_names, values):
+    first = full_names[0] if full_names else None
+    m = full_names.index(first, 1) if full_names.count(first) > 1 else len(full_names)
+    cyc = full_names[:m]
+    if m < 2 or len(set(cyc)) != m or len(full_names) % m or any(n != cyc[i % m] for i, n in enumerate(full_names)):
+        return list(values)
+    return [sum(values[i:i + m]) for i in range(0, len(values), m)]
+
+
 def per_kernel(path, counter):
-    acc = defaultdict(list)
+    rows = defaultdict(list)
     for r in csv.DictReader(open(path)):
         if r['Counter_Name'] == counter:
-            acc[base_name(r['Kernel_Name'])].append(float(r['Counter_Value']))
+            rows[base_name(r['Kernel_Name'])].append((int(r.get('Dispatch_Id') or len(rows)), r['Kernel_Name'], float(r['Counter_Value'])))
+    acc = {}
+    for k, v in rows.items():
+        v.sort(key=lambda t: t[0])
+        acc[k] = per_step([t[1] for t in v], [t[2] for t in v])
     return acc
 
 
```

Result: slower. 217.1 million samples/s (-1.1%).
